# mochell/PiCLES

Measured on AMD Instinct MI355X. Metric: particle_steps_per_sec, higher is better.
Workload: dtype f64

## Files before the change

### include/picles_hip.h

```cpp
#ifndef PICLES_HIP_H
#define PICLES_HIP_H

#include <stdint.h>
#include <stddef.h>

#ifdef __cplusplus
extern "C" {
#endif

#define PICLES_ABI_VERSION 8

typedef struct picles_grid {
    int32_t Nx, Ny;
    double  dx, dy;
    int32_t periodic_x;
    int32_t periodic_y;
    const int8_t *mask;
    int32_t j_begin, j_end;
} picles_grid;

typedef struct picles_phys {
    double r_g, C_alpha, C_phi, C_e, g;
    double gamma, q;
    double c_beta, c_D, c_e, c_alpha;
    int32_t propagation, input, dissipation, peak_shift, direction;
    int32_t _pad0;
    double  dir_deadband;
} picles_phys;

typedef struct picles_ode {
    double  abstol, reltol;
    double  dt0;
    double  dtmin;
    int32_t force_dtmin;
    int32_t solver;
    int64_t maxiters;
    double  log_energy_minimum, log_energy_maximum, wind_min_squared;
    double  timestep;
} picles_ode;

typedef struct picles_model {
    int32_t periodic_boundary;
    int32_t init_type;
    double  default_particle[3];
    double  minimal_state[2];
} picles_model;

#define PICLES_STEP_ZERO_FIRST   1
#define PICLES_STEP_MOVIE        2
#define PICLES_STEP_ATOMIC       4

#define PICLES_ST_STEPPED        1
#define PICLES_ST_MAXITERS       2
#define PICLES_ST_RESEED_NAN     4
#define PICLES_ST_RESEED_INF     8
#define PICLES_ST_CLAMPED       16
#define PICLES_ST_SWITCHED_ON   32
#define PICLES_ST_DTMIN         64
#define PICLES_ST_NONFINITE    128

typedef struct picles_counters {
    uint64_t rhs_evals;
    uint64_t steps_accepted;
    uint64_t steps_rejected;
    uint64_t reseeds;
    uint64_t clamps;
    uint64_t maxiters_hits;
    uint64_t particles_advanced;
    uint64_t halo_overflow;
    int32_t  max_reach;
    int32_t  max_reach_seen;
    uint64_t dropped_nonfinite;
    uint64_t wave_attempt_slots;
} picles_counters;

typedef struct picles_timing {
    double advance_ms, scatter_ms, remesh_ms, other_ms;
    uint64_t advance_launches, scatter_launches, remesh_launches;
} picles_timing;

typedef struct picles_ctx picles_ctx;

int32_t picles_create(const picles_grid *g, const picles_phys *p, const picles_ode *o,
                      const picles_model *m, int32_t device_id, int32_t halo_rows,
                      picles_ctx **out);
int32_t picles_destroy(picles_ctx *ctx);
const char *picles_last_error(const picles_ctx *ctx);
int32_t picles_abi_version(void);

int32_t picles_set_winds(picles_ctx *ctx, const double *u0, const double *v0, double t0,
                         const double *u1, const double *v1, double t1);
int32_t picles_set_winds3(picles_ctx *ctx, const double *u0, const double *v0, double t0,
                          const double *um, const double *vm,
                          const double *u1, const double *v1, double t1);
int32_t picles_set_winds_knot(picles_ctx *ctx, const double *u0, const double *v0, double t0,
                              const double *uk, const double *vk, double tk,
                              const double *u1, const double *v1, double t1);
#define PICLES_MAX_KNOTS 8
int32_t picles_set_winds_polyline(picles_ctx *ctx, int32_t nlev, const double *const *u, const double *const *v, const double *times);

int32_t picles_set_metric(picles_ctx *ctx, const double *m11, const double *m22, const double *pc);

int32_t picles_set_wind_grid(picles_ctx *ctx, int32_t nx, int32_t ny, int32_t nt,
                             double x0, double dx, double y0, double dy, double t0, double dt,
                             const double *u, const double *v, double mesh_x0, double mesh_y0);
#define PICLES_LATTICE_LINEAR  0
#define PICLES_LATTICE_SMOOTH3 1
int32_t picles_set_wind_grid_mode(picles_ctx *ctx, int32_t mode);
int32_t picles_lattice_knots(double lat_t0, double lat_dt, double t, double dt, double *tk);
int32_t picles_lattice_knot_times(double lat_t0, double lat_dt, double t, double dt, double *tks, int32_t cap);
int32_t picles_get_winds(picles_ctx *ctx, double *u0, double *v0, double *u1, double *v1);
int32_t picles_get_winds_mid(picles_ctx *ctx, double *um, double *vm);

int32_t picles_seed(picles_ctx *ctx, double t0);

int32_t picles_time_step(picles_ctx *ctx, double dt, int32_t flags);
int32_t picles_run_steps(picles_ctx *ctx, double dt, int32_t n_steps);
int32_t picles_advance(picles_ctx *ctx, double dt, int32_t flags);
int32_t picles_remesh(picles_ctx *ctx, double dt);
int32_t picles_tick(picles_ctx *ctx, double dt);
int32_t picles_zero_state(picles_ctx *ctx);
double  picles_clock(const picles_ctx *ctx);

int32_t picles_get_state(picles_ctx *ctx, double *state);
int32_t picles_set_state(picles_ctx *ctx, const double *state);
int32_t picles_get_movie_state(picles_ctx *ctx, double *state);

int32_t picles_store_init(picles_ctx *ctx, int32_t n_slots);
int32_t picles_store_push(picles_ctx *ctx);
int32_t picles_store_pop(picles_ctx *ctx, double *state, double *time);
int32_t picles_store_pending(const picles_ctx *ctx);

#define PICLES_DIAG_HS    1
#define PICLES_DIAG_TP    2
#define PICLES_DIAG_CG_X  4
#define PICLES_DIAG_CG_Y  8
#define PICLES_DIAG_E    16
#define PICLES_DIAG_MX   32
#define PICLES_DIAG_MY   64
#define PICLES_DIAG_ALL 127
#define PICLES_DIAG_TILE 256
int32_t picles_diag_init(picles_ctx *ctx, int32_t cx, int32_t cy, int32_t field_mask, int32_t n_slots);
int32_t picles_diag_shape(const picles_ctx *ctx, int32_t *nxc, int32_t *nyc_loc, int32_t *n_fields, int32_t *n_partials, size_t *bytes);
int32_t picles_diag_push(picles_ctx *ctx);
int32_t picles_diag_pop(picles_ctx *ctx, void *fields, double *partials, double *time);
int32_t picles_diag_pending(const picles_ctx *ctx);

#define PICLES_PROBE_E_FULL -30
int32_t picles_probe_init(picles_ctx *ctx, int32_t n, const int32_t *ij, int32_t every, int32_t first, int32_t capacity);
int32_t picles_probe_sample(picles_ctx *ctx, void *stream);
int32_t picles_probe_pop(picles_ctx *ctx, int32_t max_samples, double *values, double *times, int64_t *steps, int32_t *n_out);
int32_t picles_probe_pending(const picles_ctx *ctx);
int32_t picles_probe_shape(const picles_ctx *ctx, int32_t *n, int32_t *every, int32_t *capacity);
int32_t picles_probe_free(picles_ctx *ctx);

#define PICLES_STAT_PEAK   1
#define PICLES_STAT_MEAN   2
#define PICLES_STAT_EXCEED 4
#define PICLES_STAT_ALL    7
int32_t picles_stat_init(picles_ctx *ctx, int32_t group_mask, int32_t n_thresholds, const double *thresholds, int32_t every, int32_t first);
int32_t picles_stat_shape(const picles_ctx *ctx, int32_t *group_mask, int32_t *n_thresholds, double *thresholds, int32_t *every, int32_t *n_planes, size_t *bytes);
int32_t picles_stat_update(picles_ctx *ctx, void *stream);
int32_t picles_stat_get(picles_ctx *ctx, int32_t group_mask, void *planes, int64_t *n_samples, double *t_first, double *t_last);
int32_t picles_stat_set(picles_ctx *ctx, int32_t group_mask, const void *planes, int64_t n_samples, double t_first, double t_last);
int32_t picles_stat_reset(picles_ctx *ctx);
int32_t picles_stat_free(picles_ctx *ctx);

int32_t picles_get_particles(picles_ctx *ctx, double *z, uint8_t *on, uint8_t *boundary,
                             int32_t *status);
int32_t picles_set_particles(picles_ctx *ctx, const double *z, const uint8_t *on);

int32_t picles_get_counters(picles_ctx *ctx, picles_counters *c);
int32_t picles_reset_counters(picles_ctx *ctx);
int32_t picles_enable_timing(picles_ctx *ctx, int32_t on);
int32_t picles_get_timing(picles_ctx *ctx, picles_timing *t);
int32_t picles_get_timing_samples(picles_ctx *ctx, int32_t kind, double *out_ms, int32_t cap);
int32_t picles_get_dispatch_order(picles_ctx *ctx, int32_t *out, int32_t cap);
int32_t picles_sync(picles_ctx *ctx);

#define PICLES_ROWS_ALL      0
#define PICLES_ROWS_EDGE     1
#define PICLES_ROWS_INTERIOR 2
int32_t picles_begin_step(picles_ctx *ctx, double dt, int32_t flags);
int32_t picles_advance_rows(picles_ctx *ctx, int32_t which, void *stream);
int32_t picles_scatter_remesh(picles_ctx *ctx, void *stream);
int32_t picles_begin_fused_step(picles_ctx *ctx, double dt);
int32_t picles_step_rows(picles_ctx *ctx, int32_t which, void *stream);
int32_t picles_end_fused_step(picles_ctx *ctx);
int32_t picles_halo_send_dev(picles_ctx *ctx, int32_t side, void **ptr, size_t *bytes);
int32_t picles_halo_recv_dev(picles_ctx *ctx, int32_t side, void **ptr, size_t *bytes);
int32_t picles_halo_rows(const picles_ctx *ctx);
int32_t picles_set_halo_rows(picles_ctx *ctx, int32_t halo_rows);
int32_t picles_set_slab_mode(picles_ctx *ctx, int32_t on);

#define PICLES_SLAB_ID_BYTES 128
int32_t picles_slab_unique_id(void *id128);
int32_t picles_slab_comm_init(picles_ctx *ctx, const void *id128, int32_t rank, int32_t world);
int32_t picles_slab_run_steps(picles_ctx *ctx, double dt, int32_t n_steps, int32_t flags);
int32_t picles_slab_exchange(picles_ctx *ctx);
int32_t picles_slab_streams(picles_ctx *ctx, void **edge_stream, void **interior_stream);
int32_t picles_slab_comm_destroy(picles_ctx *ctx);
typedef struct picles_slab_phases {
    uint64_t steps;
    uint64_t exchange_hidden;
    double   edge_ms;
    double   exchange_ms;
    double   interior_ms;
    double   slack_ms;
    double   span_ms;
} picles_slab_phases;
int32_t picles_slab_get_phases(picles_ctx *ctx, picles_slab_phases *out);

#define PICLES_CKPT_E_SHORT    -20
#define PICLES_CKPT_E_MAGIC    -21
#define PICLES_CKPT_E_VERSION  -22
#define PICLES_CKPT_E_CONFIG   -23
#define PICLES_CKPT_E_CHECKSUM -24
#define PICLES_CKPT_E_BUSY     -25
int32_t picles_checkpoint_size(picles_ctx *ctx, size_t *bytes);
int32_t picles_checkpoint_begin(picles_ctx *ctx);
int32_t picles_checkpoint_end(picles_ctx *ctx, void *buf, size_t bytes);
int32_t picles_checkpoint_load(picles_ctx *ctx, const void *buf, size_t bytes);

int32_t picles_scatter_particles(picles_ctx *ctx, int64_t n, const int32_t *ij,
                                 const double *xy, const double *charge);

#ifdef __cplusplus
}
#endif
#endif
```

### picles_amd/_capi.py

```python
from __future__ import annotations

import ctypes as C
import os
from pathlib import Path

HERE = Path(__file__).resolve().parent
LIB_PATH = HERE / "csrc" / "libpicles_hip.so"

c_double_p = C.POINTER(C.c_double)
c_int8_p = C.POINTER(C.c_int8)
c_uint8_p = C.POINTER(C.c_uint8)
c_int32_p = C.POINTER(C.c_int32)


class PiclesGrid(C.Structure):
    _fields_ = [
        ("Nx", C.c_int32), ("Ny", C.c_int32),
        ("dx", C.c_double), ("dy", C.c_double),
        ("periodic_x", C.c_int32), ("periodic_y", C.c_int32),
        ("mask", c_int8_p),
        ("j_begin", C.c_int32), ("j_end", C.c_int32),
    ]


class PiclesPhys(C.Structure):
    _fields_ = [
        ("r_g", C.c_double), ("C_alpha", C.c_double), ("C_phi", C.c_double),
        ("C_e", C.c_double), ("g", C.c_double),
        ("gamma", C.c_double), ("q", C.c_double),
        ("c_beta", C.c_double), ("c_D", C.c_double), ("c_e", C.c_double), ("c_alpha", C.c_double),
        ("propagation", C.c_int32), ("input", C.c_int32), ("dissipation", C.c_int32),
        ("peak_shift", C.c_int32), ("direction", C.c_int32), ("_pad0", C.c_int32),
        ("dir_deadband", C.c_double),
    ]


class PiclesOde(C.Structure):
    _fields_ = [
        ("abstol", C.c_double), ("reltol", C.c_double),
        ("dt0", C.c_double), ("dtmin", C.c_double),
        ("force_dtmin", C.c_int32), ("solver", C.c_int32),
        ("maxiters", C.c_int64),
        ("log_energy_minimum", C.c_double), ("log_energy_maximum", C.c_double),
        ("wind_min_squared", C.c_double), ("timestep", C.c_double),
    ]


class PiclesModel(C.Structure):
    _fields_ = [
        ("periodic_boundary", C.c_int32), ("init_type", C.c_int32),
        ("default_particle", C.c_double * 3),
        ("minimal_state", C.c_double * 2),
    ]


class PiclesCounters(C.Structure):
    _fields_ = [
        ("rhs_evals", C.c_uint64), ("steps_accepted", C.c_uint64), ("steps_rejected", C.c_uint64),
        ("reseeds", C.c_uint64), ("clamps", C.c_uint64), ("maxiters_hits", C.c_uint64),
        ("particles_advanced", C.c_uint64), ("halo_overflow", C.c_uint64),
        ("max_reach", C.c_int32), ("max_reach_seen", C.c_int32),
        ("dropped_nonfinite", C.c_uint64), ("wave_attempt_slots", C.c_uint64),
    ]

    def as_dict(self):
        return {k: getattr(self, k) for k, _ in self._fields_ if not k.startswith("_")}


class PiclesTiming(C.Structure):
    _fields_ = [
        ("advance_ms", C.c_double), ("scatter_ms", C.c_double), ("remesh_ms", C.c_double),
        ("other_ms", C.c_double),
        ("advance_launches", C.c_uint64), ("scatter_launches", C.c_uint64),
        ("remesh_launches", C.c_uint64),
    ]

    def as_dict(self):
        return {k: getattr(self, k) for k, _ in self._fields_}


class PiclesSlabPhases(C.Structure):
    _fields_ = [
        ("steps", C.c_uint64), ("exchange_hidden", C.c_uint64),
        ("edge_ms", C.c_double), ("exchange_ms", C.c_double), ("interior_ms", C.c_double),
        ("slack_ms", C.c_double), ("span_ms", C.c_double),
    ]

    def as_dict(self):
        return {k: getattr(self, k) for k, _ in self._fields_}


LATTICE_LINEAR, LATTICE_SMOOTH3 = 0, 1
STEP_ZERO_FIRST = 1
STEP_MOVIE = 2
STEP_ATOMIC = 4
ABI_VERSION = 8
SLAB_ID_BYTES = 128
PROBE_E_FULL = -30

STAT_PEAK, STAT_MEAN, STAT_EXCEED, STAT_ALL = 1, 2, 4, 7

ROWS_ALL, ROWS_EDGE, ROWS_INTERIOR = 0, 1, 2

CKPT_E_SHORT, CKPT_E_MAGIC, CKPT_E_VERSION, CKPT_E_CONFIG, CKPT_E_CHECKSUM, CKPT_E_BUSY = -20, -21, -22, -23, -24, -25
CKPT_MAGIC = 0x31544b4353454c43
CKPT_HEADER_BYTES = 256
CKPT_SEGMENTS = ("state", "z", "qold", "dtn", "asw", "status", "on", "pflags", "counters", "reach_maps")

DIAG_FIELDS = ("hs", "tp", "cg_x", "cg_y", "e", "m_x", "m_y")
DIAG_BITS = {name: 1 << k for k, name in enumerate(DIAG_FIELDS)}
DIAG_TILE = 256
DIAG_PARTIAL = ("sum_e", "sum_mx", "sum_my", "n_wet", "max_e", "max_mx", "max_my")

ST_STEPPED, ST_MAXITERS, ST_RESEED_NAN, ST_RESEED_INF = 1, 2, 4, 8
ST_CLAMPED, ST_SWITCHED_ON, ST_DTMIN, ST_NONFINITE = 16, 32, 64, 128

_VP = C.c_void_p
SYMBOLS = {
    "picles_create": (C.c_int32, [C.POINTER(PiclesGrid), C.POINTER(PiclesPhys), C.POINTER(PiclesOde),
                                  C.POINTER(PiclesModel), C.c_int32, C.c_int32, C.POINTER(_VP)]),
    "picles_destroy": (C.c_int32, [_VP]),
    "picles_last_error": (C.c_char_p, [_VP]),
    "picles_abi_version": (C.c_int32, []),
    "picles_set_winds": (C.c_int32, [_VP, c_double_p, c_double_p, C.c_double, c_double_p, c_double_p, C.c_double]),
    "picles_set_winds3": (C.c_int32, [_VP, c_double_p, c_double_p, C.c_double, c_double_p, c_double_p, c_double_p, c_double_p, C.c_double]),
    "picles_set_winds_knot": (C.c_int32, [_VP, c_double_p, c_double_p, C.c_double, c_double_p, c_double_p, C.c_double,
                                          c_double_p, c_double_p, C.c_double]),
    "picles_set_winds_polyline": (C.c_int32, [_VP, C.c_int32, C.POINTER(c_double_p), C.POINTER(c_double_p), c_double_p]),
    "picles_get_winds_mid": (C.c_int32, [_VP, c_double_p, c_double_p]),
    "picles_set_metric": (C.c_int32, [_VP, c_double_p, c_double_p, c_double_p]),
    "picles_set_wind_grid": (C.c_int32, [_VP, C.c_int32, C.c_int32, C.c_int32, C.c_double, C.c_double, C.c_double,
                                         C.c_double, C.c_double, C.c_double, c_double_p, c_double_p, C.c_double, C.c_double]),
    "picles_set_wind_grid_mode": (C.c_int32, [_VP, C.c_int32]),
    "picles_lattice_knots": (C.c_int32, [C.c_double, C.c_double, C.c_double, C.c_double, c_double_p]),
    "picles_lattice_knot_times": (C.c_int32, [C.c_double, C.c_double, C.c_double, C.c_double, c_double_p, C.c_int32]),
    "picles_get_winds": (C.c_int32, [_VP, c_double_p, c_double_p, c_double_p, c_double_p]),
    "picles_seed": (C.c_int32, [_VP, C.c_double]),
    "picles_time_step": (C.c_int32, [_VP, C.c_double, C.c_int32]),
    "picles_run_steps": (C.c_int32, [_VP, C.c_double, C.c_int32]),
    "picles_advance": (C.c_int32, [_VP, C.c_double, C.c_int32]),
    "picles_remesh": (C.c_int32, [_VP, C.c_double]),
    "picles_tick": (C.c_int32, [_VP, C.c_double]),
    "picles_zero_state": (C.c_int32, [_VP]),
    "picles_clock": (C.c_double, [_VP]),
    "picles_get_state": (C.c_int32, [_VP, c_double_p]),
    "picles_set_state": (C.c_int32, [_VP, c_double_p]),
    "picles_get_movie_state": (C.c_int32, [_VP, c_double_p]),
    "picles_store_init": (C.c_int32, [_VP, C.c_int32]),
    "picles_store_push": (C.c_int32, [_VP]),
    "picles_store_pop": (C.c_int32, [_VP, c_double_p, c_double_p]),
    "picles_store_pending": (C.c_int32, [_VP]),
    "picles_diag_init": (C.c_int32, [_VP, C.c_int32, C.c_int32, C.c_int32, C.c_int32]),
    "picles_diag_shape": (C.c_int32, [_VP, c_int32_p, c_int32_p, c_int32_p, c_int32_p, C.POINTER(C.c_size_t)]),
    "picles_diag_push": (C.c_int32, [_VP]),
    "picles_diag_pop": (C.c_int32, [_VP, _VP, c_double_p, c_double_p]),
    "picles_diag_pending": (C.c_int32, [_VP]),
    "picles_probe_init": (C.c_int32, [_VP, C.c_int32, c_int32_p, C.c_int32, C.c_int32, C.c_int32]),
    "picles_probe_sample": (C.c_int32, [_VP, _VP]),
    "picles_probe_pop": (C.c_int32, [_VP, C.c_int32, c_double_p, c_double_p, C.POINTER(C.c_int64), c_int32_p]),
    "picles_probe_pending": (C.c_int32, [_VP]),
    "picles_probe_shape": (C.c_int32, [_VP, c_int32_p, c_int32_p, c_int32_p]),
    "picles_probe_free": (C.c_int32, [_VP]),
    "picles_stat_init": (C.c_int32, [_VP, C.c_int32, C.c_int32, c_double_p, C.c_int32, C.c_int32]),
    "picles_stat_shape": (C.c_int32, [_VP, c_int32_p, c_int32_p, c_double_p, c_int32_p, c_int32_p, C.POINTER(C.c_size_t)]),
    "picles_stat_update": (C.c_int32, [_VP, _VP]),
    "picles_stat_get": (C.c_int32, [_VP, C.c_int32, _VP, C.POINTER(C.c_int64), c_double_p, c_double_p]),
    "picles_stat_set": (C.c_int32, [_VP, C.c_int32, _VP, C.c_int64, C.c_double, C.c_double]),
    "picles_stat_reset": (C.c_int32, [_VP]),
    "picles_stat_free": (C.c_int32, [_VP]),
    "picles_get_particles": (C.c_int32, [_VP, c_double_p, c_uint8_p, c_uint8_p, c_int32_p]),
    "picles_set_particles": (C.c_int32, [_VP, c_double_p, c_uint8_p]),
    "picles_get_counters": (C.c_int32, [_VP, C.POINTER(PiclesCounters)]),
    "picles_reset_counters": (C.c_int32, [_VP]),
    "picles_enable_timing": (C.c_int32, [_VP, C.c_int32]),
    "picles_get_timing": (C.c_int32, [_VP, C.POINTER(PiclesTiming)]),
    "picles_get_timing_samples": (C.c_int32, [_VP, C.c_int32, c_double_p, C.c_int32]),
    "picles_get_dispatch_order": (C.c_int32, [_VP, C.POINTER(C.c_int32), C.c_int32]),
    "picles_sync": (C.c_int32, [_VP]),
    "picles_begin_step": (C.c_int32, [_VP, C.c_double, C.c_int32]),
    "picles_advance_rows": (C.c_int32, [_VP, C.c_int32, _VP]),
    "picles_scatter_remesh": (C.c_int32, [_VP, _VP]),
    "picles_begin_fused_step": (C.c_int32, [_VP, C.c_double]),
    "picles_step_rows": (C.c_int32, [_VP, C.c_int32, _VP]),
    "picles_end_fused_step": (C.c_int32, [_VP]),
    "picles_halo_send_dev": (C.c_int32, [_VP, C.c_int32, C.POINTER(_VP), C.POINTER(C.c_size_t)]),
    "picles_halo_recv_dev": (C.c_int32, [_VP, C.c_int32, C.POINTER(_VP), C.POINTER(C.c_size_t)]),
    "picles_halo_rows": (C.c_int32, [_VP]),
    "picles_set_halo_rows": (C.c_int32, [_VP, C.c_int32]),
    "picles_set_slab_mode": (C.c_int32, [_VP, C.c_int32]),
    "picles_slab_unique_id": (C.c_int32, [_VP]),
    "picles_slab_comm_init": (C.c_int32, [_VP, _VP, C.c_int32, C.c_int32]),
    "picles_slab_run_steps": (C.c_int32, [_VP, C.c_double, C.c_int32, C.c_int32]),
    "picles_slab_exchange": (C.c_int32, [_VP]),
    "picles_slab_streams": (C.c_int32, [_VP, C.POINTER(_VP), C.POINTER(_VP)]),
    "picles_slab_comm_destroy": (C.c_int32, [_VP]),
    "picles_slab_get_phases": (C.c_int32, [_VP, C.POINTER(PiclesSlabPhases)]),
    "picles_scatter_particles": (C.c_int32, [_VP, C.c_int64, c_int32_p, c_double_p, c_double_p]),
    "picles_checkpoint_size": (C.c_int32, [_VP, C.POINTER(C.c_size_t)]),
    "picles_checkpoint_begin": (C.c_int32, [_VP]),
    "picles_checkpoint_end": (C.c_int32, [_VP, _VP, C.c_size_t]),
    "picles_checkpoint_load": (C.c_int32, [_VP, _VP, C.c_size_t]),
}

_lib = None


class PiclesError(RuntimeError):
    pass


class CheckpointError(PiclesError):

    def __init__(self, code, msg):
        super().__init__(msg)
        self.code = code


def _settle_rocm_runtime():
    import sys
    if "torch" in sys.modules or os.environ.get("PICLES_NO_TORCH_PRELOAD"):
        return
    try:
        import torch
    except Exception:
        pass


def load(path: os.PathLike | None = None) -> C.CDLL:
    global _lib
    if _lib is not None and path is None:
        return _lib
    p = Path(path) if path else Path(os.environ.get("PICLES_HIP_LIB", LIB_PATH))
    if not p.exists():
        raise PiclesError(
            f"{p} not found: build the HIP extension first "
            "(python -c 'import __graft_entry__ as g; g.build()' or make -C picles_amd/csrc)")
    _settle_rocm_runtime()
    lib = C.CDLL(str(p))
    for name, (res, args) in SYMBOLS.items():
        fn = getattr(lib, name)
        fn.restype = res
        fn.argtypes = args
    if lib.picles_abi_version() != ABI_VERSION:
        raise PiclesError(f"{p}: ABI version {lib.picles_abi_version()}, this binding expects {ABI_VERSION} — rebuild the library")
    if path is None:
        _lib = lib
    return lib


def dptr(a):
    if a is None:
        return None
    return a.ctypes.data_as(c_double_p)
```

### picles_amd/csrc/k_step.inc

```
#ifndef K_STEP_NAME
#define K_STEP_NAME k_step
#define K_STEP_WROW false
#include "k_step.inc"
#undef K_STEP_NAME
#undef K_STEP_WROW
#define K_STEP_NAME k_step_waverow
#define K_STEP_WROW true
#include "k_step.inc"
#undef K_STEP_NAME
#undef K_STEP_WROW
#else
template <bool FAST, bool TSIT, bool STATIC, bool METRIC, bool AUTO>
__global__ void __launch_bounds__(256, (FAST && !AUTO) ? 4 : (FAST ? 3 : 2)) K_STEP_NAME(KParams P, GridP G, Arrays A, double t_prev, double DT_prev,
                                                double t_start, double DT, int r0, int n0, int r1, int n1)
{
    constexpr bool WROW = K_STEP_WROW;
    static_assert(!WROW || (FAST && !METRIC), "k_step_waverow: specialised physics, Cartesian");
#ifdef PICLES_PHASE_CLOCK
    const unsigned long long pc0_ = __builtin_readcyclecounter();
    unsigned long long pc1_ = pc0_, pc2_ = pc0_, pc3_ = pc0_;
#endif
#ifdef PICLES_WAVE_LOG
    const unsigned long long wl0_ = __builtin_amdgcn_s_memrealtime();
    unsigned long long wl1_ = 0;
#endif
    dp_device_init(TSIT ? 1 : 0);
    order_sign_init();
    const long long ord_counts = order_counts(A);
    const int ord_entry = order_entry(A);
    const int mr_early = pull_reach_early(A);
    pm_device_init();
    long long t = 0;
    const unsigned int lblock = ordered_block(A, ord_counts, ord_entry);
    WaveRow wr = {0, 0, 0};
    const unsigned int lane = threadIdx.x & 63u;
    bool active;
    if constexpr (WROW) { active = rows_index_waverow(G, r0, n0, lblock, wr); t = wr.t0 + lane; }
    else active = rows_index(G, r0, n0, r1, n1, t, lblock);
    StepStats S = {{0u, 0u, 0u, 0}, 0u, 0u, 0u, 0u, 0u, 0u, 0};
    int rtile = -1;
    if (active) {
        int i, jl;
        if constexpr (WROW) { i = wr.i0 + (int)lane; jl = wr.jl; }
        else { i = (int)(t % G.Nx); jl = (int)(t / G.Nx); }
        double s0 = 0.0, s1 = 0.0, s2 = 0.0;
        if constexpr (WROW) rmap_clear_ahead_waverow(A, wr, lane);
        else rmap_clear_ahead(A, t);
        const Arrays Av = WROW ? arrays_at(A, wr.t0) : A;
        const long long tx = WROW ? (long long)lane : t;
        constexpr bool PREFETCH = AUTO;
        unsigned char pf_pre = 0;
        Wind w_pre = {0.0, 0.0, 0.0, 0.0, 0.0, 0.0};
        double qold_pre = 0.0, uP_pre = 0.0, vP_pre = 0.0;
        int asw_pre = 0;
        if constexpr (PREFETCH) {
            pf_pre = Av.pflags[tx];
            w_pre = load_wind(P, Av, tx);
            if constexpr (WROW) w_pre.xi = (unsigned int)t;
            qold_pre = Av.qold[tx];
            asw_pre = Av.asw[tx];
            if (!STATIC) { uP_pre = Av.uP[tx]; vP_pre = Av.vP[tx]; }
        }
        if constexpr (WROW) pull_waverow(G, A, wr, lane, pull_reach_local_waverow(G, A, wr, lane, pull_reach(G, A, jl, mr_early)), s0, s1, s2);
        else pull_any(G, A, i, jl, pull_reach_local(G, A, i, jl, pull_reach(G, A, jl, mr_early)), s0, s1, s2);
#ifdef PICLES_PHASE_CLOCK
        __asm__ volatile("" : "+v"(s0), "+v"(s1), "+v"(s2));
        pc1_ = __builtin_readcyclecounter();
#endif
#ifdef PICLES_WAVE_LOG
        __asm__ volatile("" : "+v"(s0), "+v"(s1), "+v"(s2));
        wl1_ = __builtin_amdgcn_s_memrealtime();
#endif
        unsigned char pf = PREFETCH ? pf_pre : Av.pflags[tx];
        __shared__ int stash_[WROW ? 1 : 5][256];
        if (pf & PF_STEPPED) {
            Wind w = PREFETCH ? w_pre : load_wind(P, Av, tx);
            if constexpr (WROW) w.xi = (unsigned int)t;
            Vec5 z = {0.0, 0.0, 0.0, 0.0, 0.0};
            double qold = PREFETCH ? qold_pre : Av.qold[tx], dtn = -1.0;
            int br = remesh_regs_lazy(P, pf, s0, s1, s2, DT_prev, z, STATIC ? &Av.u0[tx] : (PREFETCH ? &uP_pre : &Av.uP[tx]),
                                      STATIC ? &Av.v0[tx] : (PREFETCH ? &vP_pre : &Av.vP[tx]));
            int on = (br <= 1);
            int asw = AUTO ? (PREFETCH ? asw_pre : Av.asw[tx]) : 0;
            if (br == 1) { qold = PI_LNQOLDINIT; asw = ASW_FRESH; S.reseeds = 1; }
            unsigned int rs = S.reseeds;
            S.reseeds = 0;
            const int tid_ = threadIdx.x;
            if constexpr (WROW) stash_[0][tid_] = (int)pf | ((int)rs << 8);
            else {
                stash_[0][tid_] = (int)(unsigned int)((unsigned long long)t & 0xffffffffull); stash_[1][tid_] = (int)((unsigned long long)t >> 32);
                stash_[2][tid_] = i; stash_[3][tid_] = jl; stash_[4][tid_] = (int)pf | ((int)rs << 8);
            }
            int status;
            if (METRIC) status = advance_core<FAST, STATIC, true, TSIT, AUTO>(P, w, z, on, qold, dtn, t_start, DT, S, Av.m11[tx], Av.m22[tx], Av.pc[tx], &asw);
            else status = advance_core<FAST, STATIC, false, TSIT, AUTO>(P, w, z, on, qold, dtn, t_start, DT, S, 0.0, 0.0, 0.0, &asw);
#ifdef PICLES_PHASE_CLOCK
            __asm__ volatile("" : "+v"(z.lne));
            pc2_ = __builtin_readcyclecounter();
#endif
            KStepArgsPtr K = kargs_reload();
            const KParams Pb = K->P;
            const GridP Gb = K->G;
            const Arrays Ab = K->A;
            __asm__ volatile("" ::: "memory");
            const int tid2_ = threadIdx.x;
            WaveRow wrb = {0, 0, 0};
            long long tb;
            int ib = 0, jlb = 0, pr_;
            if constexpr (WROW) {
                wrb = waverow_of(Gb, K->r0, lblock);
                tb = wrb.t0 + (threadIdx.x & 63u);
                pr_ = stash_[0][tid2_];
            } else {
                tb = (long long)(((unsigned long long)(unsigned int)stash_[1][tid2_] << 32) | (unsigned int)stash_[0][tid2_]);
                ib = stash_[2][tid2_]; jlb = stash_[3][tid2_]; pr_ = stash_[4][tid2_];
            }
            const unsigned char pfb = (unsigned char)(pr_ & 0xff);
            const Arrays Abv = WROW ? arrays_at(Ab, wrb.t0) : Ab;
            const long long tbx = WROW ? (long long)(threadIdx.x & 63u) : tb;
            status = advance_guards(Pb, [&]() { Wind wg = load_wind(Pb, Abv, tbx); if constexpr (WROW) wg.xi = (unsigned int)tb; return wg; },
                                    z, dtn, K->t_start, K->DT, status, S);
            if (AUTO) Abv.asw[tbx] = asw;
            S.reseeds += (unsigned int)(pr_ >> 8);
            Abv.qold[tbx] = qold;
            Abv.status[tbx] = status;
            if constexpr (WROW) write_record_at(Gb, rec_row_out(Ab, Gb, wrb.jl + Gb.R) + wrb.i0, threadIdx.x & 63u, pfb, on, z, S);
            else write_record(Gb, Ab, ib, jlb, pfb, on, z, S);
            rtile = WROW ? (int)(wrb.t0 >> 6) : (int)(tb >> 6);
        }
    }
    {
        KStepArgsPtr K = kargs_reload();
        const Arrays Ab = K->A;
        flush_stats<WROW>(Ab, S, rtile);
        if (Ab.ord && order_wanted(Ab)) order_file(Ab, lblock, __ballot(S.adv != 0 || S.reseeds != 0) != 0);
#ifdef PICLES_WAVE_LOG
        if ((threadIdx.x & 63) == 0) {
            unsigned int hw_, xcc_;
            __asm__ volatile("s_getreg_b32 %0, hwreg(HW_REG_HW_ID)" : "=s"(hw_));
            __asm__ volatile("s_getreg_b32 %0, hwreg(HW_REG_XCC_ID)" : "=s"(xcc_));
            unsigned long long *wl_ = (unsigned long long *)Ab.movie + 4ull * ((unsigned long long)lblock * 4ull + (threadIdx.x >> 6));
            wl_[0] = wl0_; wl_[1] = wl1_; wl_[2] = __builtin_amdgcn_s_memrealtime();
            wl_[3] = (unsigned long long)hw_ | ((unsigned long long)xcc_ << 32) | ((unsigned long long)blockIdx.x << 40);
        }
#endif
#ifdef PICLES_PHASE_CLOCK
        pc3_ = __builtin_readcyclecounter();
        if ((threadIdx.x & 63) == 0) {
            DevCounters *c = Ab.cnt + ((blockIdx.x * 4u + (threadIdx.x >> 6)) & (NSLOTS - 1));
            if (pc1_ == pc0_) pc1_ = pc3_;
            if (pc2_ < pc1_) pc2_ = pc1_;
            atomicAdd(&c->pad_[0], pc1_ - pc0_); atomicAdd(&c->pad_[1], pc2_ - pc1_); atomicAdd(&c->pad_[2], pc3_ - pc2_); atomicAdd(&c->pad_[3], 1ull);
        }
#endif
    }
}
#endif
```

### picles_amd/csrc/kernels.h

```cpp
#ifndef PICLES_KERNELS_H
#define PICLES_KERNELS_H

#include <hip/hip_runtime.h>
#include <cstdint>
#include <type_traits>

#include "../../include/picles_hip.h"
#include "physics.h"

struct GridP {
    int Nx, Ny;
    int periodic_x, periodic_y;
    int tripolar;
    int j_begin, ny_loc;
    int R;
    int Rp;
    int single_slab;
    int ngroups;
};

#define NSLOTS 1024
struct DevCounters {
    unsigned long long rhs, acc, rej, reseeds, clamps, maxit, adv, overflow;
    unsigned long long nonfinite, wslots, pad_[6];
};

struct Arrays {
    double *state, *movie;
    double *z;
    double *qold, *dtn;
    int *asw;
    unsigned char *on, *pflags;
    int *status;
    double *u0, *v0, *u1, *v1;
    double *um, *vm;
    double *uP, *vP;
    double *m11, *m22, *pc;
    double *rec;
    double *rec_out;
    DevCounters *cnt;
    int mr_idx;
    int ntile;
    int *rmap;
    int ord_on, nblk;
    int *ord;
    long long n;
};
__device__ __forceinline__ int *order_buf(const Arrays &A, int which) { return A.ord + (size_t)which * (size_t)(2 + A.nblk); }

__device__ __forceinline__ int *reach_counters(const Arrays &A) { return (int *)(A.cnt + NSLOTS); }

#define PF_STEPPED 1
#define PF_GROUP2 2
#define PF_BOUNDARY 4

__device__ __forceinline__ unsigned long long wave_sum_u64(unsigned long long v)
{
    const unsigned int lo0 = (unsigned int)__builtin_amdgcn_readfirstlane((int)(unsigned int)v);
    const unsigned int hi0 = (unsigned int)__builtin_amdgcn_readfirstlane((int)(unsigned int)(v >> 32));
    const unsigned long long v0 = ((unsigned long long)hi0 << 32) | lo0;
    if (__all(v == v0)) return v0 * 64ull;
#pragma unroll
    for (int o = 32; o > 0; o >>= 1) v += __shfl_xor(v, o, 64);
    return v;
}
__device__ __forceinline__ int wave_max_i32(int v)
{
#pragma unroll
    for (int o = 32; o > 0; o >>= 1) {
        int t = __shfl_xor(v, o, 64);
        v = (t > v) ? t : v;
    }
    return v;
}

template <bool POLY = false>
__device__ __forceinline__ Wind load_wind(const KParams &P, const Arrays &A, long long t)
{
    Wind w;
    w.u0 = A.u0[t];
    w.v0 = A.v0[t];
    w.bu = 0.0;
    w.bv = 0.0;
    w.xi = (unsigned int)t;
    if (POLY && !P.wind_static && P.wind_nk > 1) {
        const double *pl = P.wind_xb + PICLES_MAX_KNOTS + t;
        w.du = pl[0]; w.dv = pl[P.wind_xn]; w.bu = pl[2 * P.wind_xn]; w.bv = pl[3 * P.wind_xn];
        return w;
    }
    if (P.wind_static) {
        w.du = 0.0;
        w.dv = 0.0;
    } else {
        const double u1 = A.u1[t], v1 = A.v1[t];
        w.du = u1 - w.u0;
        w.dv = v1 - w.v0;
        if (A.um) {
            const double um = A.um[t], vm = A.vm[t];
            if (P.wind_sk > 0.0) {
                w.du = (um - w.u0) * P.wind_isk;
                w.dv = (vm - w.v0) * P.wind_isk;
                w.bu = (u1 - um) * P.wind_i1sk - w.du;
                w.bv = (v1 - vm) * P.wind_i1sk - w.dv;
            } else {
                w.bu = 2.0 * ((w.u0 + u1) - 2.0 * um);
                w.bv = 2.0 * ((w.v0 + v1) - 2.0 * vm);
            }
        }
    }
    return w;
}

__device__ __forceinline__ double *rec_row(const Arrays &A, const GridP &G, int row)
{
    return A.rec + (size_t)row * 6 * G.Nx;
}
__device__ __forceinline__ double *rec_row_out(const Arrays &A, const GridP &G, int row)
{
    return A.rec_out + (size_t)row * 6 * G.Nx;
}

#define REC_BIAS 2048
#define REACH_CAP 64
__device__ __forceinline__ double rec_encode(int grp, int bx, int by)
{
    return (double)(grp + 4 * (bx + REC_BIAS) + 4 * 4096 * (by + REC_BIAS));
}
__device__ __forceinline__ void rec_decode(double code, int &grp, int &bx, int &by)
{
    int ci = (int)code;
    grp = ci & 3;
    bx = ((ci >> 2) & 4095) - REC_BIAS;
    by = (ci >> 14) - REC_BIAS;
}

struct StepStats {
    PStats st;
    unsigned int adv, reseeds, clamps, maxit, overflow, nonfinite;
    int reach;
};

template <bool FAST, bool STATIC, bool METRIC = false, bool TSIT = false, bool AUTO = false, bool TABS = true>
__device__ __forceinline__ int advance_core(const KParams &P, const Wind &w, Vec5 &z, int &on, double &qold,
                                            double &dtn, double t_start, double DT, StepStats &S,
                                            double m11 = 0.0, double m22 = 0.0, double pc = 0.0, int *asw = nullptr)
{
    int status = PICLES_ST_STEPPED;
    if (on) {
        S.adv = 1;
        integrate_dp5<FAST, STATIC, METRIC, TSIT, AUTO, TABS>(P, w, z, qold, dtn, t_start, DT, S.st, m11, m22, pc, asw);
        status |= S.st.status;
    } else {
        double u, v;
        wind_at<(!FAST && !STATIC)>(P, w, t_start + DT, u, v);
        if (u * u + v * v >= P.wind_min_sq) {
            reseed(P, u, v, DT, z);
            dtn = -1.0;
            on = 1;
            status |= PICLES_ST_SWITCHED_ON;
        }
    }
    return status;
}

template <bool POLY = false, class WF>
__device__ __forceinline__ int advance_guards(const KParams &P, WF wind, Vec5 &z, double &dtn, double t_start, double DT,
                                              int status, StepStats &S)
{
    if (pm_isnan(z.lne) || pm_isnan(z.cx) || pm_isnan(z.cy)) {
        double u, v;
        const Wind w = wind();
        wind_at<POLY>(P, w, t_start + DT, u, v);
        reseed(P, u, v, DT, z);
        dtn = -1.0;
        status |= PICLES_ST_RESEED_NAN;
    } else if (pm_isinf(z.lne) || pm_isinf(z.cx) || pm_isinf(z.cy)) {
        double u, v;
        const Wind w = wind();
        wind_at<POLY>(P, w, t_start, u, v);
        reseed(P, u, v, DT, z);
        dtn = -1.0;
        status |= PICLES_ST_RESEED_INF;
    } else if (z.lne > P.lne_max) {
        z.lne = P.lne_max;
        dtn = -1.0;
        status |= PICLES_ST_CLAMPED;
    }
    if (status & (PICLES_ST_RESEED_NAN | PICLES_ST_RESEED_INF | PICLES_ST_SWITCHED_ON)) S.reseeds = 1;
    if (status & PICLES_ST_CLAMPED) S.clamps = 1;
    if (status & PICLES_ST_MAXITERS) S.maxit = 1;
    return status;
}

struct KStepArgs {
    KParams P;
    GridP G;
    Arrays A;
    double t_prev, DT_prev, t_start, DT;
    int r0, n0, r1, n1;
};
static_assert(__builtin_offsetof(KStepArgs, G) == sizeof(KParams) && __builtin_offsetof(KStepArgs, A) % 8 == 0 &&
              __builtin_offsetof(KStepArgs, t_prev) == __builtin_offsetof(KStepArgs, A) + sizeof(Arrays) &&
              __builtin_offsetof(KStepArgs, r0) == __builtin_offsetof(KStepArgs, DT) + 8,
              "KStepArgs must mirror the kernarg layout of k_step");
typedef const KStepArgs *KStepArgsPtr;
__device__ __forceinline__ KStepArgsPtr kargs_reload(void)
{
    auto p = __builtin_amdgcn_kernarg_segment_ptr();
    __asm__ volatile("" : "+s"(p));
    return (KStepArgsPtr)p;
}

template <class IDX>
__device__ __forceinline__ void write_record_at(const GridP &G, double *rr, IDX i, unsigned char pf, int on, const Vec5 &z, StepStats &S)
{
    auto at = [&](int plane) -> double & {
        if constexpr (std::is_unsigned<IDX>::value) return (rr + (size_t)plane * (size_t)G.Nx)[i];
        else return rr[plane * G.Nx + i];
    };
    double code = 0.0;
    if (on && !(pm_isfinite(z.x) && pm_isfinite(z.y))) {
        S.nonfinite = 1;
    } else if (on && !(pm_fabs(z.x) < 2047.0 && pm_fabs(z.y) < 2047.0)) {
        S.overflow = 1;
    } else if (on) {
        double e, mx, my;
        particle_to_charge(z.lne, z.cx, z.cy, e, mx, my);
        int bx, by;
        double wx, wy;
        index_weight(z.x, bx, wx);
        index_weight(z.y, by, wy);
        int r = (bx < 0) ? -bx : bx + 1;
        int ry = (by < 0) ? -by : by + 1;
        S.reach = (r > ry) ? r : ry;
        if (S.reach <= ((G.Rp > 0) ? G.Rp : REACH_CAP)) {
            at(0) = e; at(1) = mx; at(2) = my; at(3) = wx; at(4) = wy;
            code = rec_encode((pf & PF_GROUP2) ? 2 : 1, bx, by);
        }
        else { S.overflow = 1; S.reach = 0; }
    }
    at(5) = code;
}
__device__ __forceinline__ void write_record(const GridP &G, const Arrays &A, int i, int jl, unsigned char pf, int on,
                                             const Vec5 &z, StepStats &S)
{
    write_record_at(G, rec_row_out(A, G, jl + G.R), i, pf, on, z, S);
}

template <bool WROW = false>
__device__ __forceinline__ void flush_stats(const Arrays &A, const StepStats &S, int rtile = -1)
{
    unsigned long long s_rhs = wave_sum_u64(S.st.rhs);
    unsigned long long s_ar = wave_sum_u64(((unsigned long long)S.st.acc << 32) | S.st.rej);
    unsigned long long b_adv = __ballot(S.adv != 0), b_res1 = __ballot(S.reseeds == 1), b_res2 = __ballot(S.reseeds >= 2);
    unsigned long long b_cl = __ballot(S.clamps != 0), b_mx = __ballot(S.maxit != 0), b_ov = __ballot(S.overflow != 0);
    unsigned long long b_nf = __ballot(S.nonfinite != 0);
    const int att_ = (int)(S.st.acc + S.st.rej);
    int m_att = __builtin_amdgcn_readfirstlane(att_);
    while (__ballot(att_ > m_att)) m_att++;
    int m_reach = 0;
    if (__ballot(S.reach > 0)) {
        m_reach = 1;
        while (__ballot(S.reach > m_reach)) m_reach++;
    }
    if (m_reach > 0) {
        int *const rm = A.rmap + (size_t)((A.mr_idx >> 4) & 15) * (size_t)A.ntile;
        if constexpr (WROW) {
            const int lead = __ffsll((long long)__ballot(S.reach > 0)) - 1;
            const int tile0 = __builtin_amdgcn_readlane(rtile, lead);
            if ((int)(threadIdx.x & 63) == lead) atomicMax(rm + tile0, m_reach);
        }
        int mine = (!WROW && S.reach > 0) ? rtile : -1;
        unsigned long long todo = WROW ? 0ull : __ballot(mine >= 0);
        while (todo) {
            const int lead = __ffsll((long long)todo) - 1;
            const int tile0 = __builtin_amdgcn_readlane(mine, lead);
            const bool in = (mine == tile0);
            int r0 = 1;
            while (__ballot(in && S.reach > r0)) r0++;
            if ((int)(threadIdx.x & 63) == lead) atomicMax(rm + tile0, r0);
            if (in) mine = -1;
            todo = __ballot(mine >= 0);
        }
    }
    if ((threadIdx.x & 63) == 0) {
        DevCounters *c = A.cnt + ((blockIdx.x * 4u + (threadIdx.x >> 6)) & (NSLOTS - 1));
        unsigned long long s_acc = s_ar >> 32, s_rej = s_ar & 0xffffffffULL;
        unsigned long long s_res = (unsigned long long)__popcll(b_res1) + 2ull * __popcll(b_res2);
        if (s_rhs) atomicAdd(&c->rhs, s_rhs);
        if (s_acc) atomicAdd(&c->acc, s_acc);
        if (s_rej) atomicAdd(&c->rej, s_rej);
        if (b_adv) atomicAdd(&c->adv, (unsigned long long)__popcll(b_adv));
        if (s_res) atomicAdd(&c->reseeds, s_res);
        if (b_cl) atomicAdd(&c->clamps, (unsigned long long)__popcll(b_cl));
        if (b_mx) atomicAdd(&c->maxit, (unsigned long long)__popcll(b_mx));
        if (b_ov) atomicAdd(&c->overflow, (unsigned long long)__popcll(b_ov));
        if (b_nf) atomicAdd(&c->nonfinite, (unsigned long long)__popcll(b_nf));
        if (m_att) atomicAdd(&c->wslots, 64ull * (unsigned long long)m_att);
        int *const mr = reach_counters(A), *const mr_out = mr + ((A.mr_idx >> 4) & 15);
        if (m_reach > 0 && m_reach > __hip_atomic_load(mr_out, __ATOMIC_RELAXED, __HIP_MEMORY_SCOPE_AGENT)) {
            atomicMax(mr_out, m_reach);
            atomicMax(mr + 5, m_reach);
        }
        if (blockIdx.x == 0 && threadIdx.x == 0) {
            mr[(A.mr_idx >> 8) & 15] = 0;
            mr[8 + ((A.mr_idx >> 8) & 15)] = 0;
        }
        if (!b_adv && !s_res && mr[8 + ((A.mr_idx >> 4) & 15)] == 0) mr[8 + ((A.mr_idx >> 4) & 15)] = 1;
    }
}

__device__ __forceinline__ unsigned int xcd_block(void)
{
    const unsigned int n = gridDim.x, b = blockIdx.x;
    const unsigned int per = (n + 7u) / 8u;
    unsigned int l = (b % 8u) * per + b / 8u;
    return (n % 8u == 0u) ? l : b;
}

#define PICLES_BLOCK 256
__device__ __forceinline__ long long order_counts(const Arrays &A)
{
    return A.ord_on ? *(const long long *)order_buf(A, A.mr_idx & 15) : 0ll;
}
__device__ __forceinline__ int order_entry(const Arrays &A)
{
    return (A.ord_on && (int)blockIdx.x < A.nblk) ? order_buf(A, A.mr_idx & 15)[2 + blockIdx.x] : 0;
}
__device__ __forceinline__ unsigned int ordered_block(const Arrays &A, long long counts, int entry)
{
    if (A.ord_on) {
        const int busy = (int)(counts & 0xffffffffll), calm = (int)(counts >> 32);
        if (busy + calm == A.nblk && (int)gridDim.x == A.nblk && 8 * calm >= A.nblk) return (unsigned int)entry;
    }
    return xcd_block();
}
__device__ __forceinline__ int *order_sign(void)
{
    __shared__ int sign_;
    return &sign_;
}
__device__ __forceinline__ void order_sign_init(void) { if (threadIdx.x == 0) *order_sign() = 0; }
__device__ __forceinline__ bool order_wanted(const Arrays &A) { return reach_counters(A)[8 + (A.mr_idx & 15)] != 0; }
__device__ __forceinline__ void order_file(const Arrays &A, unsigned int lblock, bool wave_busy)
{
    if ((threadIdx.x & 63) != 0) return;
    const int v = atomicAdd(order_sign(), 1 + (wave_busy ? 256 : 0));
    if ((v & 255) != (int)(PICLES_BLOCK / 64) - 1) return;
    const bool busy = wave_busy || (v >> 8) != 0;
    int *const wb = order_buf(A, (A.mr_idx >> 4) & 15);
    const int pos = busy ? atomicAdd(wb, 1) : A.nblk - 1 - atomicAdd(wb + 1, 1);
    if (pos >= 0 && pos < A.nblk) wb[2 + pos] = (int)lblock;
    if (blockIdx.x == 0) { int *const cb = order_buf(A, (A.mr_idx >> 8) & 15); cb[0] = 0; cb[1] = 0; }
}

__device__ __forceinline__ bool rows_index(const GridP &G, int r0, int n0, int r1, int n1, long long &t, unsigned int lblock)
{
    if (n1 == 0 && (G.Nx & 63) == 0 && (n0 & 3) == 0) {
        const unsigned int nbx = (unsigned int)G.Nx >> 6;
        const unsigned int by = lblock / nbx, bx = lblock - by * nbx;
        if (by >= ((unsigned int)n0 >> 2)) return false;
        t = ((long long)r0 + 4ll * by + (threadIdx.x >> 6)) * G.Nx + (64ll * bx + (threadIdx.x & 63));
        return true;
    }
    long long tid = (long long)lblock * PICLES_BLOCK + threadIdx.x;
    long long na = (long long)n0 * G.Nx, nb = (long long)n1 * G.Nx;
    if (tid >= na + nb) return false;
    t = (tid < na) ? (long long)r0 * G.Nx + tid : (long long)r1 * G.Nx + (tid - na);
    return true;
}

__device__ __forceinline__ int remesh_regs(const KParams &P, const Wind &w, unsigned char pf, double e, double mx,
                                           double my, double clock, double DT, Vec5 &z)
{
    double u, v;
    wind_at<true>(P, w, clock, u, v);
    bool bnd = (pf & PF_BOUNDARY) != 0;
    if (!bnd && (e >= P.min_e) && (mx * mx + my * my >= P.min_m2)) {
        charge_to_particle(e, mx, my, z);
        return 0;
    }
    if (u * u + v * v >= P.wind_min_sq) {
        reseed(P, u, v, DT, z);
        return 1;
    }
    return 2;
}

__device__ __forceinline__ int remesh_regs_lazy(const KParams &P, unsigned char pf, double e, double mx, double my,
                                                double DT, Vec5 &z, const double *pu, const double *pv)
{
    bool bnd = (pf & PF_BOUNDARY) != 0;
    if (!bnd && (e >= P.min_e) && (mx * mx + my * my >= P.min_m2)) {
        charge_to_particle(e, mx, my, z);
        return 0;
    }
    double u = *pu, v = *pv;
    if (u * u + v * v >= P.wind_min_sq) {
        reseed(P, u, v, DT, z);
        return 1;
    }
    return 2;
}

// ... 124 lines not shown
        for (int k = 0; k < 4; k++) {
            if (on[k]) {
                const double w = (hx[k] ? wx[k] : 1.0 - wx[k]) * (hy[k] ? wy[k] : 1.0 - wy[k]);
                s0 += w * e[k];
                s1 += w * mx[k];
                s2 += w * my[k];
            }
        }
    }
}
template <int RT>
__device__ __forceinline__ void pull_node(const GridP &G, const Arrays &A, int i, int jl, int Rdyn,
                                          double &s0, double &s1, double &s2)
{
    const int R = RT ? RT : Rdyn, W = 2 * R + 1;
    const int RO = G.R;
    const int j = jl + G.j_begin, Nx = G.Nx;
    const double *__restrict__ rec = A.rec;
    const unsigned int pl = (unsigned int)Nx, rowlen = 6u * pl;
    bool interior = (i - R >= 0) && (i + R < Nx) && (j - R >= 0) && (j + R < G.Ny);
    if (interior) {
        const unsigned int base = (unsigned int)(jl + RO) * rowlen + (unsigned int)i;
        for (int grp = 1; grp <= G.ngroups; grp++) {
            if constexpr (RT == 1 || RT == 2) {
                pull_window_2p<RT>(rec, base, pl, rowlen, grp, s0, s1, s2);
            } else {
#pragma unroll 1
                for (int dj = -R; dj <= R; dj++) {
                    const unsigned int rb = base + (unsigned int)(dj * (int)rowlen);
                    if constexpr (RT != 0) {
#pragma unroll
                        for (int di = -RT; di <= RT; di++)
                            pull_candidate(rec, rb + (unsigned int)di, pl, di, dj, grp, true, s0, s1, s2);
                    } else {
                        for (int di = -R; di <= R; di++)
                            pull_candidate(rec, rb + (unsigned int)di, pl, di, dj, grp, true, s0, s1, s2);
                    }
                }
            }
        }
        return;
    }
    int shx = 0, shy = 0;
    if (G.periodic_x) { if (i - R < 0) shx = R - i; else if (i + R >= Nx) shx = Nx - i + R; }
    if (G.periodic_y) { if (j - R < 0) shy = R - j; else if (j + R >= G.Ny) shy = G.Ny - j + R; }
    for (int grp = 1; grp <= G.ngroups; grp++) {
#pragma unroll 1
        for (int sj = 0; sj < W; sj++) {
            int qj = sj + shy; if (qj >= W) qj -= W;
            int dj = qj - R;
            int jj = j + dj;
            bool rowok = G.periodic_y || (jj >= 0 && jj < G.Ny);
            int row;
            if (G.single_slab) {
                int jw = jj; if (jw < 0) jw += G.Ny; else if (jw >= G.Ny) jw -= G.Ny;
                row = jw + RO;
            } else {
                row = jl + dj + RO;
            }
            if (!rowok) continue;
#pragma unroll 1
            for (int si = 0; si < W; si++) {
                int qi = si + shx; if (qi >= W) qi -= W;
                int di = qi - R;
                int ii = i + di;
                if (ii < 0 || ii >= Nx) {
                    if (!G.periodic_x) continue;
                    ii += (ii < 0) ? Nx : -Nx;
                }
                pull_candidate(rec, (unsigned int)row * rowlen + (unsigned int)ii, pl, di, dj, grp, true, s0, s1, s2);
            }
        }
    }
}

__device__ __forceinline__ int floor_mod(int a, int b) { int r = a % b; return (r < 0) ? r + b : r; }

__device__ __forceinline__ void pull_node_tripolar(const GridP &G, const Arrays &A, int i, int jl, int R,
                                                   double &s0, double &s1, double &s2)
{
    const int RO = G.R, Nx = G.Nx, Ny = G.Ny, j = jl + G.j_begin, W = 2 * R + 1;
    const double *__restrict__ rec = A.rec;
    const unsigned int pl = (unsigned int)Nx, rowlen = 6u * pl;
    const int cB = floor_mod(Nx - 2 - i, Nx);
    const bool narrow = (2 * W <= Nx);
    const int a0 = floor_mod(i - R, Nx), b0 = floor_mod(cB - R, Nx);
    for (int grp = 1; grp <= G.ngroups; grp++) {
        for (int js = max(0, j - R); js < Ny; js++) {
            const unsigned int rbase = (unsigned int)(js - G.j_begin + RO) * rowlen;
            int ka = 0, kb = 0, is_full = 0;
            while (narrow ? (ka < W || kb < W) : (is_full < Nx)) {
                int is;
                if (narrow) {
                    const int wa = a0 + W - Nx, wb = b0 + W - Nx;
                    int ea = (ka < W) ? ((wa > 0) ? ((ka < wa) ? ka : a0 + (ka - wa)) : a0 + ka) : 0x7fffffff;
                    int eb = (kb < W) ? ((wb > 0) ? ((kb < wb) ? kb : b0 + (kb - wb)) : b0 + kb) : 0x7fffffff;
                    is = min(ea, eb);
                    if (ea == is) ka++;
                    if (eb == is) kb++;
                } else {
                    is = is_full++;
                }
                const int ci0 = (int)rec[rbase + 5u * pl + (unsigned int)is];
                if (ci0 == 0 || (ci0 & 3) != grp) continue;
                const int bx = ((ci0 >> 2) & 4095) - REC_BIAS, by = (ci0 >> 14) - REC_BIAS;
                const double wxh = rec[rbase + 3u * pl + (unsigned int)is], wyh = rec[rbase + 4u * pl + (unsigned int)is];
#pragma unroll
                for (int k = 0; k < 4; k++) {
                    const int ax = k & 1, ay = k >> 1;
                    int ci = is + bx + ax, cj = js + by + ay;
                    if (cj < 0) continue;
                    if (cj >= Ny) { ci = Nx - 1 - floor_mod(ci + 1, Nx); cj = 2 * Ny - 1 - cj; }
                    else ci = floor_mod(ci, Nx);
                    if (ci != i || cj != j) continue;
                    const double w = (ax ? wxh : 1.0 - wxh) * (ay ? wyh : 1.0 - wyh);
                    s0 += w * rec[rbase + (unsigned int)is];
                    s1 += w * rec[rbase + pl + (unsigned int)is];
                    s2 += w * rec[rbase + 2u * pl + (unsigned int)is];
                }
            }
        }
    }
}

__device__ __forceinline__ void pull_any(const GridP &G, const Arrays &A, int i, int jl, int R,
                                         double &s0, double &s1, double &s2)
{
    const int W = 2 * R + 1;
    if (R == 0) return;
    if (G.tripolar && jl + G.j_begin >= G.Ny - R) pull_node_tripolar(G, A, i, jl, R, s0, s1, s2);
    else if ((G.periodic_x && W > G.Nx) || (G.periodic_y && W > G.Ny)) pull_node_aliased(G, A, i, jl, R, s0, s1, s2);
    else if (R == 1) pull_node<1>(G, A, i, jl, 1, s0, s1, s2);
    else if (R == 2) pull_node<2>(G, A, i, jl, 2, s0, s1, s2);
    else if (R == 3) pull_node<3>(G, A, i, jl, 3, s0, s1, s2);
    else if (R == 4) pull_node<4>(G, A, i, jl, 4, s0, s1, s2);
    else pull_node<0>(G, A, i, jl, R, s0, s1, s2);
}

__device__ __forceinline__ int pull_reach_early(const Arrays &A) { return reach_counters(A)[A.mr_idx & 15]; }
__device__ __forceinline__ int pull_reach(const GridP &G, const Arrays &A, int jl, int m)
{
    if (G.Rp > 0 && (jl < G.R || jl >= G.ny_loc - G.R)) return G.Rp;
    if (m < 1) m = 1;
    return (G.Rp > 0 && m > G.Rp) ? G.Rp : m;
}
__device__ __forceinline__ int pull_reach(const GridP &G, const Arrays &A, int jl) { return pull_reach(G, A, jl, pull_reach_early(A)); }


__device__ __forceinline__ void rmap_clear_ahead(const Arrays &A, long long t)
{
    if ((t & 63) == 0) A.rmap[(size_t)((A.mr_idx >> 8) & 15) * (size_t)A.ntile + (size_t)(t >> 6)] = 0;
}

__device__ __forceinline__ int pull_reach_local(const GridP &G, const Arrays &A, int i, int jl, int Rg)
{
    int R = Rg;
    const int j = jl + G.j_begin;
    const bool edge_row = G.Rp > 0 && (jl < G.R || jl >= G.ny_loc - G.R);
    if (Rg >= 2 && Rg <= 31 && !edge_row && i - Rg >= 0 && i + Rg < G.Nx && jl - Rg >= 0 && jl + Rg < G.ny_loc &&
        j - Rg >= 0 && j + Rg < G.Ny) {
        const int *const rm = A.rmap + (size_t)(A.mr_idx & 15) * (size_t)A.ntile;
        int m = 0;
        long long t0 = (long long)(jl - Rg) * G.Nx + (i - Rg);
        for (int dj = -Rg; dj <= Rg; dj++, t0 += G.Nx) {
            const int a = rm[t0 >> 6], b = rm[(t0 + 2 * Rg) >> 6];
            m = max(m, max(a, b));
        }
        R = min(m, Rg);
    }
    if (Rg < 2) return Rg;
    int m = 0;
    while (__ballot(R > m)) m++;
    return m;
}

struct WaveRow {
    int jl, i0;
    long long t0;
};
__device__ __forceinline__ WaveRow waverow_of(const GridP &G, int r0, unsigned int lblock)
{
    const unsigned int nbx = (unsigned int)G.Nx >> 6;
    const unsigned int by = lblock / nbx, bx = lblock - by * nbx;
    WaveRow w;
    unsigned int tid = threadIdx.x;
    __asm__ volatile("" : "+v"(tid));
    w.jl = r0 + 4 * (int)by + __builtin_amdgcn_readfirstlane((int)(tid >> 6));
    w.i0 = (int)(64u * bx);
    w.t0 = (long long)w.jl * G.Nx + w.i0;
    return w;
}
__device__ __forceinline__ bool rows_index_waverow(const GridP &G, int r0, int n0, unsigned int lblock, WaveRow &w)
{
    const unsigned int nbx = (unsigned int)G.Nx >> 6;
    if (lblock / nbx >= ((unsigned int)n0 >> 2)) return false;
    w = waverow_of(G, r0, lblock);
    return true;
}
__device__ __forceinline__ Arrays arrays_at(const Arrays &A, long long t0)
{
    Arrays B = A;
    B.qold += t0; B.asw += t0; B.pflags += t0; B.status += t0;
    B.u0 += t0; B.v0 += t0; B.u1 += t0; B.v1 += t0; B.uP += t0; B.vP += t0;
    B.um = A.um ? A.um + t0 : nullptr; B.vm += t0;
    return B;
}
__device__ __forceinline__ void rmap_clear_ahead_waverow(const Arrays &A, const WaveRow &w, unsigned int lane)
{
    if (lane == 0u) A.rmap[(size_t)((A.mr_idx >> 8) & 15) * (size_t)A.ntile + (size_t)(w.t0 >> 6)] = 0;
}

__device__ __forceinline__ int pull_reach_local_waverow(const GridP &G, const Arrays &A, const WaveRow &w, unsigned int lane, int Rg)
{
    if (Rg < 2) return Rg;
    const int jl = w.jl, j = jl + G.j_begin;
    const bool edge_row = G.Rp > 0 && (jl < G.R || jl >= G.ny_loc - G.R);
    if (Rg <= 31 && !edge_row && w.i0 - Rg >= 0 && w.i0 + 63 + Rg < G.Nx && jl - Rg >= 0 && jl + Rg < G.ny_loc && j - Rg >= 0 && j + Rg < G.Ny) {
        const int *const rm = A.rmap + (size_t)(A.mr_idx & 15) * (size_t)A.ntile;
        const long long nbx = G.Nx >> 6;
        long long tile = ((long long)(jl - Rg) * G.Nx + w.i0) >> 6;
        int m = 0;
        for (int dj = -Rg; dj <= Rg; dj++, tile += nbx) m = max(m, max(rm[tile - 1], max(rm[tile], rm[tile + 1])));
        return __builtin_amdgcn_readfirstlane(min(m, Rg));
    }
    return pull_reach_local(G, A, w.i0 + (int)lane, jl, Rg);
}

template <int R>
__device__ __forceinline__ void pull_walk_lanes(const double *__restrict__ rec, unsigned int base, unsigned int pl, unsigned int rowlen,
                                                unsigned int m, unsigned int ax, unsigned int ay, double &s0, double &s1, double &s2)
{
    constexpr int W = 2 * R + 1;
    while (__ballot(m != 0u)) {
        double e[4], mx[4], my[4], wx[4], wy[4];
        bool on[4], hx[4], hy[4];
#pragma unroll
        for (int k = 0; k < 4; k++) {
            on[k] = (m != 0u);
            const int c = on[k] ? __builtin_ctz(m) : 0;
            m &= m - 1u;
            hx[k] = (ax >> c) & 1u; hy[k] = (ay >> c) & 1u;
            const unsigned int off = base + (unsigned int)((c / W - R) * (int)rowlen + (c % W - R));
            e[k] = mx[k] = my[k] = wx[k] = wy[k] = 0.0;
            if (on[k]) {
                wx[k] = rec[off + 3u * pl]; wy[k] = rec[off + 4u * pl];
                e[k] = rec[off]; mx[k] = rec[off + pl]; my[k] = rec[off + 2u * pl];
            }
        }
#pragma unroll
        for (int k = 0; k < 4; k++) {
            if (on[k]) {
                const double w = (hx[k] ? wx[k] : 1.0 - wx[k]) * (hy[k] ? wy[k] : 1.0 - wy[k]);
                s0 += w * e[k];
                s1 += w * mx[k];
                s2 += w * my[k];
            }
        }
    }
}

template <int R>
__device__ __forceinline__ void pull_window_waverow(const double *__restrict__ rec, const double *__restrict__ rec0, unsigned int lane,
                                                    unsigned int base, unsigned int pl, unsigned int rowlen, int grp,
                                                    double &s0, double &s1, double &s2)
{
    constexpr int W = 2 * R + 1, NC = W * W;
    static_assert(NC <= 25, "corner bits of all candidates in two words");
    const double *const codes = rec0 + 5u * (size_t)pl;
    unsigned int vo[5];
#pragma unroll
    for (int k = 0; k < 5; k++) vo[k] = 8u * ((unsigned int)k * pl + lane);
    int d[NC];
    unsigned int m0 = 0u, some = 0u, px = 0u, py = 0u;
#pragma unroll
    for (int c = 0; c < NC; c++) {
        const int di = c % W - R, dj = c / W - R;
        d[c] = (int)(codes + ((long long)dj * (long long)rowlen + di))[lane] - (grp + 4 * (REC_BIAS - 1 - di) + 4 * 4096 * (REC_BIAS - 1 - dj));
        const unsigned int n = (unsigned int)__builtin_popcountll(__ballot((d[c] & ~(4 | 16384)) == 0));
        m0 |= (n >> 6) << c;
        some |= n & 63u;
        px |= ((unsigned int)d[c] & 4u) << c;
        py |= (((unsigned int)d[c] >> 14) & 1u) << c;
    }
    if constexpr (R >= 2) {
        if (some != 0u) { pull_window_2p<R>(rec, base, pl, rowlen, grp, s0, s1, s2); return; }
    } else if (some != 0u) {
        unsigned int m = 0u, ax = 0u, ay = 0u;
#pragma unroll
        for (int c = 0; c < NC; c++) {
            m |= ((d[c] & ~(4 | 16384)) == 0 ? 1u : 0u) << c;
            ax |= ((d[c] & 4) ? 0u : 1u) << c;
            ay |= ((d[c] & 16384) ? 0u : 1u) << c;
        }
        pull_walk_lanes<R>(rec, base, pl, rowlen, m, ax, ay, s0, s1, s2);
        return;
    }
    unsigned int mu = m0;
    while (mu != 0u) {
        double e[4], mx[4], my[4], wx[4], wy[4];
        bool on[4], hx[4], hy[4];
#pragma unroll
        for (int k = 0; k < 4; k++) {
            on[k] = (mu != 0u);
            const int c = on[k] ? __builtin_ctz(mu) : 0;
            mu &= mu - 1u;
            hx[k] = !((px >> (c + 2)) & 1u); hy[k] = !((py >> c) & 1u);
            const double *const p = rec0 + ((long long)(c / W - R) * (long long)rowlen + (c % W - R));
            e[k] = mx[k] = my[k] = wx[k] = wy[k] = 0.0;
            if (on[k]) {
                const char *const pb = (const char *)p;
                wx[k] = *(const double *)(pb + vo[3]); wy[k] = *(const double *)(pb + vo[4]);
                e[k] = *(const double *)(pb + vo[0]); mx[k] = *(const double *)(pb + vo[1]); my[k] = *(const double *)(pb + vo[2]);
            }
        }
#pragma unroll
        for (int k = 0; k < 4; k++) {
            if (on[k]) {
                const double w = (hx[k] ? wx[k] : 1.0 - wx[k]) * (hy[k] ? wy[k] : 1.0 - wy[k]);
                s0 += w * e[k];
                s1 += w * mx[k];
                s2 += w * my[k];
            }
        }
    }
}

__device__ __forceinline__ void pull_waverow(const GridP &G, const Arrays &A, const WaveRow &w, unsigned int lane, int R,
                                             double &s0, double &s1, double &s2)
{
    const int j = w.jl + G.j_begin;
    if ((R == 1 || R == 2) && w.i0 - R >= 0 && w.i0 + 63 + R < G.Nx && j - R >= 0 && j + R < G.Ny) {
        const unsigned int pl = (unsigned int)G.Nx, rowlen = 6u * pl;
        const double *const rec0 = A.rec + ((size_t)(w.jl + G.R) * (size_t)rowlen + (size_t)w.i0);
        const unsigned int base = (unsigned int)(w.jl + G.R) * rowlen + ((unsigned int)w.i0 + lane);
        for (int grp = 1; grp <= G.ngroups; grp++) {
            if (R == 1) pull_window_waverow<1>(A.rec, rec0, lane, base, pl, rowlen, grp, s0, s1, s2);
            else pull_window_waverow<2>(A.rec, rec0, lane, base, pl, rowlen, grp, s0, s1, s2);
        }
        return;
    }
    pull_any(G, A, w.i0 + (int)lane, w.jl, R, s0, s1, s2);
}

struct StepLaunch {
    dim3 grid, block;
    hipStream_t stream;
    const KParams *P;
    const GridP *G;
    const Arrays *A;
    double t_prev, DT_prev, t_start, DT;
    int r0, n0, r1, n1;
    bool waverow;
};
static inline bool waverow_geometry(int Nx, int n0, int n1) { return n1 == 0 && (Nx & 63) == 0 && (n0 & 3) == 0; }
static inline bool waverow_flavour(bool fast, bool metric) { return fast && !metric; }
void launch_k_step_explicit(const StepLaunch &L, bool fast, int solver, bool wind_static, bool metric);
void launch_k_step_auto(const StepLaunch &L, bool wind_static, bool metric);
void launch_k_advance(const StepLaunch &L, bool fast, int solver, bool wind_static, bool metric);

#endif
```

### picles_amd/csrc/picles_hip.hip

```cpp
#include <hip/hip_runtime.h>
#include <hipcub/hipcub.hpp>

#include <algorithm>
#include <cstdint>
#include <cstdlib>
#include <cstdio>
#include <cstring>
#include <cmath>
#include <mutex>
#include <string>
#include <vector>

#include "../../include/picles_hip.h"
#include "physics.h"

#define PX_EXPORT extern "C" __attribute__((visibility("default")))

#include "kernels.h"
#include "k_diag.h"
#include "k_probe.h"
#include "k_stat.h"

__global__ void __launch_bounds__(256) k_seed(KParams P, GridP G, Arrays A, const signed char *mask, double seed_T)
{
// ... 202 lines not shown
                }
            }
        }
    }
    __syncthreads();
    for (int k = threadIdx.x; k < PT_LY * PT_LX; k += blockDim.x) {
        int li = k % PT_LX, lj = k / PT_LX;
        double a0 = tile[0][lj][li], a1 = tile[1][lj][li], a2 = tile[2][lj][li];
        if (a0 == 0.0 && a1 == 0.0 && a2 == 0.0) continue;
        global_add3(G, A, i0 + li - PT_AP, j0 + lj - PT_AP, a0, a1, a2);
    }
}

__global__ void k_tile_count(GridP G, int ntx, const int *pij, long long np, int *count, int *tile_of)
{
    long long k = (long long)blockIdx.x * blockDim.x + threadIdx.x;
    if (k >= np) return;
    int ib = pij[k], jb = pij[np + k] - G.j_begin;
    int tile = -1;
    if (ib >= 0 && ib < G.Nx && jb >= 0 && jb < G.ny_loc) {
        tile = (jb / PT_TY) * ntx + ib / PT_TX;
        atomicAdd(&count[tile], 1);
    }
    tile_of[k] = tile;
}
__global__ void k_tile_fill(long long np, const int *tile_of, const int *seg_start, int *cursor, int *perm)
{
    long long k = (long long)blockIdx.x * blockDim.x + threadIdx.x;
    if (k >= np) return;
    int tile = tile_of[k];
    if (tile < 0) return;
    int pos = atomicAdd(&cursor[tile], 1);
    perm[seg_start[tile] + pos] = (int)k;
}

struct WindGrid {
    int nx, ny, nt;
    double x0, inv_dx, y0, inv_dy, t0, inv_dt;
    double mesh_x0, mesh_y0, mesh_dx, mesh_dy;
    const double *u, *v;
};

__device__ __forceinline__ void lattice_coord(double c, int n, int &i0, double &f)
{
    double per = (double)(n - 1);
    double w = (c < 0.0 || c > per) ? c - __builtin_floor(c / per) * per : c;
    double fl = __builtin_floor(w);
    i0 = (int)fl;
    if (i0 > n - 2) i0 = n - 2;
    if (i0 < 0) i0 = 0;
    f = w - (double)i0;
}

struct WindSampleOut { double t[2]; double *u[2], *v[2]; };
template <int NT>
__global__ void __launch_bounds__(256) k_wind_sample(GridP G, WindGrid Wg, WindSampleOut O, long long n)
{
    long long k = (long long)blockIdx.x * blockDim.x + threadIdx.x;
    if (k >= n) return;
    int i = (int)(k % G.Nx), j = (int)(k / G.Nx) + G.j_begin;
    double x = Wg.mesh_x0 + (double)i * Wg.mesh_dx, y = Wg.mesh_y0 + (double)j * Wg.mesh_dy;
    int ix, iy;
    double fx, fy;
    lattice_coord((x - Wg.x0) * Wg.inv_dx, Wg.nx, ix, fx);
    lattice_coord((y - Wg.y0) * Wg.inv_dy, Wg.ny, iy, fy);
    size_t sx = 1, sy = (size_t)Wg.nx, st = (size_t)Wg.nx * Wg.ny;
    const double *F[2] = {Wg.u, Wg.v};
#pragma unroll
    for (int q = 0; q < NT; q++) {
        int it;
        double ft;
        lattice_coord((O.t[q] - Wg.t0) * Wg.inv_dt, Wg.nt, it, ft);
        size_t b = ix * sx + iy * sy + it * st;
        double out[2];
#pragma unroll
        for (int c = 0; c < 2; c++) {
            const double *f = F[c];
            double c00 = f[b] + (f[b + sx] - f[b]) * fx;
            double c10 = f[b + sy] + (f[b + sy + sx] - f[b + sy]) * fx;
            double c01 = f[b + st] + (f[b + st + sx] - f[b + st]) * fx;
            double c11 = f[b + st + sy] + (f[b + st + sy + sx] - f[b + st + sy]) * fx;
            double c0 = c00 + (c10 - c00) * fy;
            double c1 = c01 + (c11 - c01) * fy;
            out[c] = c0 + (c1 - c0) * ft;
        }
        O.u[q][k] = out[0];
        O.v[q][k] = out[1];
    }
}

struct WindPolyForm { int nk; double sk[PICLES_MAX_KNOTS]; double ilen[PICLES_MAX_KNOTS + 1]; };
__global__ void __launch_bounds__(256) k_wind_poly(WindPolyForm F, const double *u0, const double *v0, const double *u1, const double *v1,
                                                   const double *lv, double *xb, long long n)
{
    long long t = (long long)blockIdx.x * blockDim.x + threadIdx.x;
    if (t < PICLES_MAX_KNOTS) xb[t] = (t < F.nk) ? F.sk[t] : 2.0;
    if (t >= n) return;
    double *pl = xb + PICLES_MAX_KNOTS;
    for (int c = 0; c < 2; c++) {
        double prev = c ? v0[t] : u0[t], slp = 0.0;
        for (int j = 0; j <= F.nk; j++) {
            const double next = (j < F.nk) ? lv[(size_t)(2 * j + c) * n + t] : (c ? v1[t] : u1[t]);
            const double sl = (next - prev) * F.ilen[j];
            pl[(size_t)(2 * j + c) * n + t] = j ? sl - slp : sl;
            slp = sl;
            prev = next;
        }
    }
}

static thread_local std::string g_create_error;

static const uint64_t FP_SEED = 0xcbf29ce484222325ull;
static uint64_t fp_bytes(uint64_t h, const void *p, size_t bytes)
{
    const unsigned char *b = (const unsigned char *)p;
    size_t k = 0;
    for (; k + 8 <= bytes; k += 8) {
        uint64_t w;
        memcpy(&w, b + k, 8);
        h = (h ^ w) * 0x100000001b3ull;
        h ^= h >> 29;
    }
    uint64_t w = (uint64_t)(bytes - k) << 56;
    if (k < bytes) { uint64_t t = 0; memcpy(&t, b + k, bytes - k); w ^= t; }
    h = (h ^ w) * 0x100000001b3ull;
    return h ^ (h >> 29);
}
template <class T> static uint64_t fp_val(uint64_t h, T v) { return fp_bytes(h, &v, sizeof v); }

struct picles_ctx {
    picles_grid g;
    picles_phys ph;
    picles_ode od;
    picles_model md;
    KParams P;
    GridP G;
    Arrays A;
    int device;
    hipStream_t stream;
    hipEvent_t ev_edge;
    hipEvent_t ev_ctx = nullptr;
    bool edge_pending = false;
    bool step_fresh = false;
    struct SlabRing *ring = nullptr;
    double *rec_buf[2] = {nullptr, nullptr};
    int *mr_buf[5] = {nullptr, nullptr, nullptr, nullptr, nullptr};
    int mr_w = 0;
    struct Pipe *pipe = nullptr;
    int pipe_nb = 0;
    int cur = 0;
    bool fuse_steps = true;
    int waverow_mode = 1;
    bool pending = false;
    double pend_t = 0.0, pend_dt = 0.0;
    signed char *d_mask = nullptr;
    std::vector<signed char> h_mask;
    double clock = 0.0;
    double step_dt = 0.0;
    int step_flags = 0;
    bool state_zero = false;
    bool seeded = false;
    bool timing = false;
    int timing_mode = 0;
    bool in_region = false;
    int region_launches = 0;
    struct Ev { hipEvent_t a, b; int kind; };
    std::vector<Ev> ev_used, ev_free;
    picles_timing tim{};
    std::vector<float> tim_samples[3];
    std::string err;
    int store_slots = 0, store_head = 0, store_count = 0;
    std::vector<double *> store_dev, store_host;
    std::vector<hipEvent_t> store_ready, store_done;
    std::vector<double> store_time;
    hipStream_t store_stream = nullptr;
    int diag_slots = 0, diag_head = 0, diag_count = 0;
    DiagP diag{};
    int diag_nfields = 0, diag_npart = 0;
    size_t diag_field_bytes = 0, diag_part_off = 0, diag_slot_bytes = 0;
    std::vector<unsigned char *> diag_dev, diag_host;
    std::vector<hipEvent_t> diag_ready, diag_done;
    std::vector<double> diag_time;
    int probe_n = 0, probe_every = 1, probe_first = 1, probe_cap = 0, probe_head = 0, probe_count = 0;
    long long probe_steps = 0;
    int *probe_nodes = nullptr;
    double *probe_dev = nullptr, *probe_host = nullptr;
    std::vector<hipEvent_t> probe_ready, probe_done;
    std::vector<double> probe_time;
    std::vector<long long> probe_step;
    bool stat_on = false;
    StatP stat{};
    int stat_every = 1, stat_first = 1;
    long long stat_steps = 0;
    long long stat_samples = 0;
    double stat_t_first = 0.0, stat_t_last = 0.0;
    unsigned char *stat_dev = nullptr;
    size_t stat_bytes = 0;
    hipEvent_t stat_ev = nullptr;
    hipStream_t stat_stream = nullptr;
    bool stat_ev_live = false;
    bool wind_grid_on = false;
    WindGrid wg{};
    double *d_wgu = nullptr, *d_wgv = nullptr;
    double wind_t1 = 0.0;
    bool wind_t1_valid = false;
    int wind_grid_mode = PICLES_LATTICE_LINEAR;
    double wg_t0 = 0.0, wg_dt = 0.0;
    bool ord_valid = false;
    int ord_nblk = 0;
    double *um_buf = nullptr, *vm_buf = nullptr;
    double *lv_buf = nullptr, *xb_buf = nullptr;
    int poly_cap = 0;
    bool ext_streams = false;
    bool ring_orders = false;
    unsigned char *ck_dev = nullptr, *ck_host = nullptr;
    size_t ck_cap = 0;
    hipEvent_t ck_ready = nullptr, ck_done = nullptr;
    bool ck_inflight = false;
    unsigned char ck_hdr[256];
    int halo0 = 0;
    uint64_t fp_metric = 0, fp_lattice = 0;
    int *d_count = nullptr, *d_start = nullptr, *d_cursor = nullptr;
    void *d_scan_tmp = nullptr;
    size_t scan_tmp_bytes = 0;
};

#define HIPCHK(ctx, call)                                                                      \
    do {                                                                                       \
        hipError_t e_ = (call);                                                                \
        if (e_ != hipSuccess) {                                                                \
            (ctx)->err = std::string(#call) + ": " + hipGetErrorString(e_);                    \
            return -10;                                                                        \
        }                                                                                      \
    } while (0)

static bool stream_idle(hipStream_t s)
{
    hipError_t e = hipStreamQuery(s);
    if (e != hipSuccess) (void)hipGetLastError();
    return e == hipSuccess;
}

static int fail(picles_ctx *c, int code, const std::string &m)
{
    c->err = m;
    return code;
}

static void timing_begin(picles_ctx *c, hipStream_t s, int kind)
{
    if (!c->timing) return;
    if (c->in_region) { if (kind == 0) c->region_launches++; return; }
    picles_ctx::Ev e;
    if (!c->ev_free.empty()) { e = c->ev_free.back(); c->ev_free.pop_back(); }
    else { hipEventCreate(&e.a); hipEventCreate(&e.b); }
    e.kind = kind;
    hipEventRecord(e.a, s);
    c->ev_used.push_back(e);
}
static void timing_end(picles_ctx *c, hipStream_t s)
{
    if (!c->timing || c->in_region) return;
    hipEventRecord(c->ev_used.back().b, s);
}
static void timing_collect(picles_ctx *c)
{
    for (auto &e : c->ev_used) {
        hipEventSynchronize(e.b);
        float ms = 0.f;
        hipEventElapsedTime(&ms, e.a, e.b);
        if (e.kind >= 0 && e.kind < 3 && c->tim_samples[e.kind].size() < (1u << 20)) c->tim_samples[e.kind].push_back(ms);
        switch (e.kind) {
        case 3: c->tim.advance_ms += ms; break;
        case 0: c->tim.advance_ms += ms; c->tim.advance_launches++; break;
        case 1: c->tim.scatter_ms += ms; c->tim.scatter_launches++; break;
        case 2: c->tim.remesh_ms += ms; c->tim.remesh_launches++; break;
        default: c->tim.other_ms += ms;
        }
        c->ev_free.push_back(e);
    }
    c->ev_used.clear();
}

static size_t rec_bytes(const picles_ctx *c) { return (size_t)(c->G.ny_loc + 2 * c->G.R) * 6 * c->G.Nx * sizeof(double); }

static Arrays arrays_for(picles_ctx *c, int read_buf, int write_buf)
{
    Arrays A = c->A;
    A.rec = c->rec_buf[read_buf];
    A.rec_out = c->rec_buf[write_buf];
    A.mr_idx = (read_buf == write_buf ? c->mr_w : (c->mr_w + 4) % 5) | (c->mr_w << 4) | (((c->mr_w + 2) % 5) << 8);
    return A;
}

static int launch_scatter(picles_ctx *c, hipStream_t s, bool remesh);

static int probe_room(picles_ctx *c, long long n_steps, const char *who);
static int probe_take(picles_ctx *c, hipStream_t s);
static bool probe_due(const picles_ctx *c, long long s);
static void probe_release(picles_ctx *c);
static int stat_update(picles_ctx *c, hipStream_t s);
static void stat_release(picles_ctx *c);
static inline bool stat_due(const picles_ctx *c, long long s)
{
    return s >= c->stat_first && (s - c->stat_first) % c->stat_every == 0;
}

static int flush(picles_ctx *c)
{
    if (!c->pending) return 0;
    HIPCHK(c, hipDeviceSynchronize());
    c->pending = false;
    double clock_save = c->clock, dt_save = c->step_dt;
    int flags_save = c->step_flags;
    c->clock = c->pend_t;
    c->step_dt = c->pend_dt;
    c->step_flags = PICLES_STEP_ZERO_FIRST;
    int rc = launch_scatter(c, c->stream, true);
    c->clock = clock_save; c->step_dt = dt_save; c->step_flags = flags_save;
    return rc;
}

PX_EXPORT int32_t picles_abi_version(void) { return PICLES_ABI_VERSION; }

PX_EXPORT const char *picles_last_error(const picles_ctx *ctx)
{
    return ctx ? ctx->err.c_str() : g_create_error.c_str();
}

PX_EXPORT int32_t picles_destroy(picles_ctx *c);
PX_EXPORT int32_t picles_slab_comm_destroy(picles_ctx *c);

PX_EXPORT int32_t picles_create(const picles_grid *g, const picles_phys *p, const picles_ode *o,
                                const picles_model *m, int32_t device_id, int32_t halo_rows, picles_ctx **out)
{
    if (!g || !p || !o || !m || !out) { g_create_error = "null argument"; return -1; }
    *out = nullptr;
    if (g->Nx < 2 || g->Ny < 2) { g_create_error = "grid must be at least 2x2"; return -2; }
    if (g->j_begin < 0 || g->j_end > g->Ny || g->j_end <= g->j_begin) { g_create_error = "bad slab rows [j_begin,j_end)"; return -2; }
    if (o->solver < 0 || o->solver > 2) { g_create_error = "solver must be 0 (DP5), 1 (Tsit5) or 2 (AutoTsit5(Rosenbrock23()))"; return -3; }
    if (halo_rows < 1) halo_rows = 1;
    if (halo_rows > 1024) { g_create_error = "halo_rows must be <= 1024"; return -2; }
    if (!(o->abstol > 0.0) || !(o->reltol >= 0.0) || !(o->maxiters > 0) || !(o->dtmin >= 0.0)) {
        g_create_error = "ODE settings: abstol > 0, reltol >= 0, maxiters > 0, dtmin >= 0 required";
        return -3;
    }
    int ndev = 0;
    hipError_t e = hipGetDeviceCount(&ndev);
    if (e != hipSuccess || ndev <= 0) {
        g_create_error = "no HIP device available (this library has no CPU path)";
        return -4;
    }
    if (device_id < 0 || device_id >= ndev) { g_create_error = "device_id out of range"; return -4; }
    if ((e = hipSetDevice(device_id)) != hipSuccess) { g_create_error = hipGetErrorString(e); return -4; }

    picles_ctx *c = new picles_ctx();
    if (const char *wr = getenv("PICLES_WAVEROW")) c->waverow_mode = !strcmp(wr, "0") ? 0 : (!strcmp(wr, "require") ? 2 : 1);
    memset(&c->A, 0, sizeof(c->A));
    c->stream = nullptr;
    c->ev_edge = nullptr;
    c->g = *g; c->ph = *p; c->od = *o; c->md = *m;
    c->device = device_id;
    KParams &P = c->P;
    P.r_g = p->r_g; P.inv_rg = 1.0 / p->r_g; P.C_alpha = p->C_alpha; P.C_phi = p->C_phi; P.C_e = p->C_e;
    double q = p->q;
    P.p = (-1.0 - 10.0 * q) / 2.0;
    P.n = 2.0 * q / (P.p + 4.0 * q);
    P.neg2p = -2.0 * P.p;
    double e_T = std::sqrt(p->c_e * pm_pow(p->c_alpha, -P.p / q) / pm_pow(p->gamma * p->c_beta * p->c_D, 1.0 / P.n));
    P.inv_eT = 1.0 / e_T;
    P.inv_eT4 = (P.inv_eT * P.inv_eT) * (P.inv_eT * P.inv_eT);
    P.half_inv_rg = 0.5 * P.inv_rg;
    P.two_inv_rg2 = 2.0 * (P.inv_rg * P.inv_rg);
    {
        const double k1 = 0.25 * PK_G0, k2 = k1 * k1, K = k2 * k2;
        P.KeT4 = K * P.inv_eT4;
        P.KrCa = (K * P.r_g) * P.C_alpha;
        P.Cdir = P.C_phi * P.two_inv_rg2;
        P.rg2 = P.r_g * P.r_g;
        const double rg4 = P.rg2 * P.rg2, rg8 = rg4 * rg4;
        P.Cw = (0.5 * PK_G0) * P.r_g;
        P.Chrh = -0.25 * P.r_g;
        P.ymax = 10.0 / P.r_g;
        P.sgmax = 1e8 / P.rg2;
        P.KeT4y = P.KeT4 * rg8;
        P.KrCay = P.KrCa * rg8;
        P.Cs = (0.5 * P.C_phi) * P.rg2;
        P.Cdir2 = 2.0 * P.C_phi;
        P.g4rg2 = k1 * P.rg2;
        P.qU2r_max = 249999.0 / (P.ymax * P.ymax);
    }
    P.inv_dx = 1.0 / g->dx; P.inv_dy = 1.0 / g->dy;
    P.deadband2 = p->dir_deadband * p->dir_deadband;
    P.propagation = p->propagation; P.input = p->input; P.dissipation = p->dissipation;
    P.peak_shift = p->peak_shift; P.direction = p->direction; P.n_is_2 = (P.n == 2.0);
    P.p_is_075 = (P.p == 0.75);
    P.fast_phys = P.propagation && P.input && P.dissipation && P.peak_shift && P.direction && P.n_is_2 && P.p_is_075 && P.deadband2 == 0.0;
    P.abstol = o->abstol; P.reltol = o->reltol; P.dt0 = o->dt0; P.dtmin = o->dtmin;
    P.inv_abstol = 1.0 / o->abstol;
    P.maxiters = o->maxiters; P.force_dtmin = o->force_dtmin;
    P.solver = o->solver;
    P.lne_max = o->log_energy_maximum; P.wind_min_sq = o->wind_min_squared;
    P.init_type = m->init_type;
    P.def_lne = m->default_particle[0]; P.def_cx = m->default_particle[1]; P.def_cy = m->default_particle[2];
    P.min_e = m->minimal_state[0]; P.min_m2 = m->minimal_state[1];
    P.wind_static = 1; P.tw0 = 0.0; P.inv_dtw = 0.0; P.wind_sk = P.wind_isk = P.wind_i1sk = 0.0;

    GridP &G = c->G;
    G.Nx = g->Nx; G.Ny = g->Ny; G.periodic_x = (g->periodic_x != 0); G.periodic_y = (g->periodic_y == 1);
    G.tripolar = (g->periodic_y == 2);
    if (g->periodic_y < 0 || g->periodic_y > 2 || (G.tripolar && !G.periodic_x)) {
        g_create_error = "periodic_y must be 0, 1 or 2 (tripolar north, which needs a periodic x axis)";
        delete c;
        return -2;
    }
    G.j_begin = g->j_begin; G.ny_loc = g->j_end - g->j_begin;
    G.single_slab = (g->j_begin == 0 && g->j_end == g->Ny);
    G.R = halo_rows;
    c->halo0 = halo_rows;
    G.Rp = G.single_slab ? 0 : halo_rows;
    G.ngroups = 1;

    long long n = (long long)G.Nx * G.ny_loc;
    c->h_mask.resize(n);
    for (int jl = 0; jl < G.ny_loc; jl++)
        for (int i = 0; i < G.Nx; i++) {
            int j = jl + G.j_begin;
            signed char mk;
            if (g->mask) mk = g->mask[(long long)j * G.Nx + i];
            else {
                bool ring = (!g->periodic_x && (i == 0 || i == G.Nx - 1)) || (!g->periodic_y && (j == 0 || j == G.Ny - 1));
                mk = ring ? 3 : 1;
            }
            c->h_mask[(long long)jl * G.Nx + i] = mk;
        }
    std::vector<unsigned char> pf(n, 0);
    bool any3 = false;
    if (g->mask) { for (long long k = 0; k < (long long)G.Nx * G.Ny; k++) if (g->mask[k] == 3) { any3 = true; break; } }
    else any3 = (!g->periodic_x || !g->periodic_y);
    for (long long k = 0; k < n; k++) {
        signed char mk = c->h_mask[k];
        unsigned char f = 0;
        if (mk == 1) f |= PF_STEPPED;
        if (mk == 3 && m->periodic_boundary) f |= PF_STEPPED | PF_GROUP2;
        bool bnd = m->periodic_boundary ? (mk == 2) : (mk >= 2);
        if (bnd) f |= PF_BOUNDARY;
        pf[k] = f;
    }
    if (any3 && m->periodic_boundary) G.ngroups = 2;
    if ((long long)(G.ny_loc + 2 * G.R) * 6 * G.Nx >= (1LL << 31)) {
        g_create_error = "slab too large for 32-bit record offsets ((ny_loc + 2 halo_rows) * 6 * Nx must be < 2^31): use more slabs";
        delete c;
        return -2;
    }
    if (!G.single_slab && ((G.periodic_y && G.Ny <= 2 * G.R) || G.ny_loc < G.R)) {
        g_create_error = "slab: periodic y axis not longer than 2*halo_rows, or fewer own rows than halo_rows";
        delete c;
        return -2;
    }

#define CK(call) do { hipError_t e2 = (call); if (e2 != hipSuccess) { g_create_error = std::string(#call) + ": " + hipGetErrorString(e2); picles_destroy(c); return -10; } } while (0)
    CK(hipStreamCreateWithFlags(&c->stream, hipStreamNonBlocking));
    CK(hipEventCreateWithFlags(&c->ev_edge, hipEventDisableTiming));
    CK(hipEventCreateWithFlags(&c->ev_ctx, hipEventDisableTiming));
    Arrays &A = c->A;
    memset(&A, 0, sizeof(A));
    A.n = n;
    CK(hipMalloc(&A.state, 3 * n * 8)); CK(hipMalloc(&A.movie, 3 * n * 8));
    CK(hipMalloc(&A.z, 5 * n * 8));
    CK(hipMalloc(&A.qold, n * 8)); CK(hipMalloc(&A.dtn, n * 8)); CK(hipMalloc(&A.asw, n * 4)); CK(hipMemset(A.asw, 0, n * 4));
    CK(hipMalloc(&A.on, n)); CK(hipMalloc(&A.pflags, n)); CK(hipMalloc(&A.status, n * 4));
    CK(hipMalloc(&A.u0, n * 8)); CK(hipMalloc(&A.v0, n * 8)); CK(hipMalloc(&A.u1, n * 8)); CK(hipMalloc(&A.v1, n * 8));
    CK(hipMalloc(&A.cnt, NSLOTS * sizeof(DevCounters) + 16 * sizeof(int)));
    for (int k = 0; k < 5; k++) c->mr_buf[k] = (int *)(A.cnt + NSLOTS) + k;
    CK(hipMemset(c->mr_buf[0], 0, 16 * sizeof(int)));
    for (int k = 0; k < 2; k++) {
        CK(hipMalloc(&c->rec_buf[k], rec_bytes(c)));
        CK(hipMemset(c->rec_buf[k], 0, rec_bytes(c)));
    }
    A.nblk = (int)((n + 255) / 256);
    A.ord_on = 0;
    A.ord = nullptr;
    CK(hipMalloc(&A.ord, (size_t)5 * (2 + A.nblk) * sizeof(int)));
    CK(hipMemset(A.ord, 0, (size_t)5 * (2 + A.nblk) * sizeof(int)));
    A.ntile = (int)((n + 63) / 64);
    CK(hipMalloc(&A.rmap, (size_t)5 * A.ntile * sizeof(int)));
    CK(hipMemset(A.rmap, 0, (size_t)5 * A.ntile * sizeof(int)));
    CK(hipMalloc(&c->d_mask, n));
    CK(hipMemset(A.state, 0, 3 * n * 8)); CK(hipMemset(A.movie, 0, 3 * n * 8)); CK(hipMemset(A.z, 0, 5 * n * 8));
    CK(hipMemset(A.qold, 0, n * 8)); CK(hipMemset(A.dtn, 0, n * 8)); CK(hipMemset(A.on, 0, n)); CK(hipMemset(A.status, 0, n * 4));
    CK(hipMemset(A.u0, 0, n * 8)); CK(hipMemset(A.v0, 0, n * 8)); CK(hipMemset(A.u1, 0, n * 8)); CK(hipMemset(A.v1, 0, n * 8));
    CK(hipMemset(A.cnt, 0, NSLOTS * sizeof(DevCounters)));
    CK(hipMemcpy(A.pflags, pf.data(), n, hipMemcpyHostToDevice));
    CK(hipMemcpy(c->d_mask, c->h_mask.data(), n, hipMemcpyHostToDevice));
#undef CK
    c->state_zero = true;
    *out = c;
    return 0;
}

PX_EXPORT int32_t picles_destroy(picles_ctx *c)
{
    if (!c) return 0;
    hipSetDevice(c->device);
    if (c->ring) picles_slab_comm_destroy(c);
    if (c->stream) hipStreamSynchronize(c->stream);
    if (c->store_stream) hipStreamSynchronize(c->store_stream);
    Arrays &A = c->A;
    hipFree(A.state); hipFree(A.movie); hipFree(A.z); hipFree(A.qold); hipFree(A.dtn); hipFree(A.asw); hipFree(A.on);
    hipFree(A.pflags); hipFree(A.status); hipFree(A.u0); hipFree(A.v0); hipFree(A.u1); hipFree(A.v1);
    if (A.uP) { hipFree(A.uP); hipFree(A.vP); }
    if (c->um_buf) { hipFree(c->um_buf); hipFree(c->vm_buf); }
    if (c->lv_buf) { hipFree(c->lv_buf); hipFree(c->xb_buf); }
    hipFree(A.cnt); hipFree(A.rmap); hipFree(c->d_mask);
    if (A.ord) hipFree(A.ord);
    if (A.m11) { hipFree(A.m11); hipFree(A.m22); hipFree(A.pc); }
    for (int k = 0; k < 2; k++) hipFree(c->rec_buf[k]);

    for (auto p : c->store_dev) hipFree(p);
    for (auto p : c->store_host) hipHostFree(p);
    for (auto e : c->store_ready) hipEventDestroy(e);
    for (auto e : c->store_done) hipEventDestroy(e);
    for (auto p : c->diag_dev) hipFree(p);
    for (auto p : c->diag_host) hipHostFree(p);
    for (auto e : c->diag_ready) hipEventDestroy(e);
    for (auto e : c->diag_done) hipEventDestroy(e);
    probe_release(c);
    if (c->stat_on) hipDeviceSynchronize();
    stat_release(c);
    if (c->ck_dev) hipFree(c->ck_dev);
    if (c->ck_host) hipHostFree(c->ck_host);
    if (c->ck_ready) hipEventDestroy(c->ck_ready);
    if (c->ck_done) hipEventDestroy(c->ck_done);
    if (c->store_stream) hipStreamDestroy(c->store_stream);
    if (c->d_wgu) hipFree(c->d_wgu);
    if (c->d_wgv) hipFree(c->d_wgv);
    if (c->d_count) hipFree(c->d_count);
    if (c->d_start) hipFree(c->d_start);
    if (c->d_cursor) hipFree(c->d_cursor);
    if (c->d_scan_tmp) hipFree(c->d_scan_tmp);
    for (auto &e : c->ev_used) { hipEventDestroy(e.a); hipEventDestroy(e.b); }
    for (auto &e : c->ev_free) { hipEventDestroy(e.a); hipEventDestroy(e.b); }
    if (c->ev_edge) hipEventDestroy(c->ev_edge);
    if (c->ev_ctx) hipEventDestroy(c->ev_ctx);
    if (c->stream) hipStreamDestroy(c->stream);
    delete c;
    return 0;
}

PX_EXPORT int32_t picles_sync(picles_ctx *c)
{
    if (!c) return -1;
    HIPCHK(c, hipSetDevice(c->device));
    { int rc = flush(c); if (rc) return rc; }
    HIPCHK(c, hipDeviceSynchronize());
    return 0;
}

PX_EXPORT double picles_clock(const picles_ctx *c) { return c ? c->clock : 0.0; }

static inline unsigned nblocks(long long n, int b) { return (unsigned)((n + b - 1) / b); }

static void wind_window_form(picles_ctx *c, double t0, double t1, bool knot, double tk)
{
    KParams &P = c->P;
    P.tw0 = t0;
    P.inv_dtw = 1.0 / (t1 - t0);
    if (knot) {
        P.wind_sk = (tk - t0) * P.inv_dtw;
        P.wind_isk = 1.0 / P.wind_sk;
        P.wind_i1sk = 1.0 / (1.0 - P.wind_sk);
    } else {
        P.wind_sk = P.wind_isk = P.wind_i1sk = 0.0;
    }
    P.wind_nk = knot ? 1 : 0;
}

static int wind_poly_buffers(picles_ctx *c, int nk)
{
    if (nk <= c->poly_cap) return 0;
    if (c->lv_buf) { hipFree(c->lv_buf); hipFree(c->xb_buf); c->lv_buf = c->xb_buf = nullptr; c->poly_cap = 0; }
    const size_t n = (size_t)c->A.n;
    HIPCHK(c, hipMalloc(&c->lv_buf, (size_t)2 * nk * n * 8));
    HIPCHK(c, hipMalloc(&c->xb_buf, ((size_t)PICLES_MAX_KNOTS + (size_t)2 * (nk + 1) * n) * 8));
    c->poly_cap = nk;
    return 0;
}
static int wind_window_poly(picles_ctx *c, double t0, double t1, int nk, const double *tk, hipStream_t s)
{
    KParams &P = c->P;
    Arrays &A = c->A;
    wind_window_form(c, t0, t1, true, tk[0]);
    WindPolyForm F;
    F.nk = nk;
    double sprev = 0.0;
    for (int k = 0; k < PICLES_MAX_KNOTS; k++) F.sk[k] = 2.0;
    for (int k = 0; k <= nk; k++) {
        const double sn = (k < nk) ? (tk[k] - t0) * P.inv_dtw : 1.0;
        if (k < nk) F.sk[k] = sn;
        F.ilen[k] = 1.0 / (sn - sprev);
        sprev = sn;
    }
    for (int k = nk + 1; k <= PICLES_MAX_KNOTS; k++) F.ilen[k] = 0.0;
    hipLaunchKernelGGL(k_wind_poly, dim3(nblocks(A.n, 256)), dim3(256), 0, s, F, A.u0, A.v0, A.u1, A.v1, c->lv_buf, c->xb_buf, A.n);
    HIPCHK(c, hipGetLastError());
    A.um = c->lv_buf; A.vm = c->lv_buf + A.n;
    P.wind_nk = nk;
    P.wind_xb = c->xb_buf;
    P.wind_xn = A.n;
    return 0;
}

static int set_wind_levels(picles_ctx *c, const double *u0, const double *v0, double t0,
                           const double *um, const double *vm, bool knot, double tk,
                           const double *u1, const double *v1, double t1)
{
    if (!c || !u0 || !v0) return -1;
    HIPCHK(c, hipSetDevice(c->device));
    { int rc = flush(c); if (rc) return rc; }
    HIPCHK(c, hipDeviceSynchronize());
    c->wind_grid_on = false;
    Arrays &A = c->A;
    size_t b = (size_t)A.n * 8;
    HIPCHK(c, hipMemcpyAsync(A.u0, u0, b, hipMemcpyHostToDevice, c->stream));
    HIPCHK(c, hipMemcpyAsync(A.v0, v0, b, hipMemcpyHostToDevice, c->stream));
    const bool two = u1 && v1 && t1 != t0;
    const bool three = two && um && vm;
    if (two) {
        HIPCHK(c, hipMemcpyAsync(A.u1, u1, b, hipMemcpyHostToDevice, c->stream));
        HIPCHK(c, hipMemcpyAsync(A.v1, v1, b, hipMemcpyHostToDevice, c->stream));
        c->P.wind_static = 0;
        wind_window_form(c, t0, t1, three && knot, tk);
    } else {
        c->P.wind_static = 1;
        c->P.tw0 = t0;
        c->P.inv_dtw = 0.0;
        c->P.wind_sk = c->P.wind_isk = c->P.wind_i1sk = 0.0;
        c->P.wind_nk = 0;
    }
    if (three) {
// ... 128 lines not shown
    const double eps = 1e-9;
    const double c0 = (t - lat_t0) / lat_dt, c1 = (t + dt - lat_t0) / lat_dt;
    const double k0 = __builtin_floor(c0 + eps) + 1.0;
    if (!(k0 < c1 - eps)) return 0;
    if (tk) *tk = lat_t0 + k0 * lat_dt;
    return (k0 + 1.0 < c1 - eps) ? 2 : 1;
}

PX_EXPORT int32_t picles_lattice_knot_times(double lat_t0, double lat_dt, double t, double dt, double *tks, int32_t cap)
{
    const double eps = 1e-9;
    const double c0 = (t - lat_t0) / lat_dt, c1 = (t + dt - lat_t0) / lat_dt;
    int n = 0;
    for (double k = __builtin_floor(c0 + eps) + 1.0; k < c1 - eps; k += 1.0) {
        if (tks && n < cap) tks[n] = lat_t0 + k * lat_dt;
        if (++n == 0x7fffffff) break;
    }
    return n;
}

struct WindowPlan { bool three; bool knot; double tm; int nk; double tk[PICLES_MAX_KNOTS]; };
static int wind_window_plan(picles_ctx *c, double t, double dt, WindowPlan &W)
{
    W = WindowPlan{};
    if (c->wind_grid_mode == PICLES_LATTICE_SMOOTH3) {
        W.three = true;
        W.tm = t + 0.5 * dt;
        return 0;
    }
    const int nk = picles_lattice_knot_times(c->wg_t0, c->wg_dt, t, dt, W.tk, PICLES_MAX_KNOTS);
    if (nk > PICLES_MAX_KNOTS) {
        char buf[360];
        snprintf(buf, sizeof buf, "the model step [%.17g, %.17g] contains %d time knots of the wind lattice (spacing %.17g s); a window carries at most %d: "
                 "take shorter model steps, or picles_set_wind_grid_mode(PICLES_LATTICE_SMOOTH3) if the lattice tabulates a smooth closure",
                 t, t + dt, nk, c->wg_dt, PICLES_MAX_KNOTS);
        return fail(c, -7, buf);
    }
    if (nk >= 1) { W.three = true; W.knot = true; W.tm = W.tk[0]; }
    W.nk = nk;
    return 0;
}

static int wind_window_sample(picles_ctx *c, const WindowPlan &W, double t, double dt, bool with0, hipStream_t s)
{
    Arrays &A = c->A;
    dim3 grid(nblocks(A.n, 256)), block(256);
    if (W.three && W.nk < 2 && !c->um_buf) {
        HIPCHK(c, hipMalloc(&c->um_buf, (size_t)A.n * 8));
        HIPCHK(c, hipMalloc(&c->vm_buf, (size_t)A.n * 8));
    }
    if (with0) {
        WindSampleOut O = {{t, 0.0}, {A.u0, nullptr}, {A.v0, nullptr}};
        hipLaunchKernelGGL(k_wind_sample<1>, grid, block, 0, s, c->G, c->wg, O, A.n);
    }
    if (W.nk >= 2) {
        { int rc = wind_poly_buffers(c, W.nk); if (rc) return rc; }
        const size_t n = (size_t)A.n;
        for (int k = 0; k < W.nk; k += 2) {
            const bool two = k + 1 < W.nk;
            WindSampleOut O = {{W.tk[k], two ? W.tk[k + 1] : t + dt},
                               {c->lv_buf + (size_t)(2 * k) * n, two ? c->lv_buf + (size_t)(2 * k + 2) * n : A.u1},
                               {c->lv_buf + (size_t)(2 * k + 1) * n, two ? c->lv_buf + (size_t)(2 * k + 3) * n : A.v1}};
            hipLaunchKernelGGL(k_wind_sample<2>, grid, block, 0, s, c->G, c->wg, O, A.n);
        }
        if (W.nk % 2 == 0) {
            WindSampleOut O = {{t + dt, 0.0}, {A.u1, nullptr}, {A.v1, nullptr}};
            hipLaunchKernelGGL(k_wind_sample<1>, grid, block, 0, s, c->G, c->wg, O, A.n);
        }
        HIPCHK(c, hipGetLastError());
        c->wind_t1 = t + dt;
        c->wind_t1_valid = true;
        c->P.wind_static = 0;
        return wind_window_poly(c, t, t + dt, W.nk, W.tk, s);
    }
    if (W.three) {
        WindSampleOut O = {{W.tm, t + dt}, {c->um_buf, A.u1}, {c->vm_buf, A.v1}};
        hipLaunchKernelGGL(k_wind_sample<2>, grid, block, 0, s, c->G, c->wg, O, A.n);
        A.um = c->um_buf; A.vm = c->vm_buf;
    } else {
        WindSampleOut O = {{t + dt, 0.0}, {A.u1, nullptr}, {A.v1, nullptr}};
        hipLaunchKernelGGL(k_wind_sample<1>, grid, block, 0, s, c->G, c->wg, O, A.n);
        A.um = A.vm = nullptr;
    }
    HIPCHK(c, hipGetLastError());
    c->wind_t1 = t + dt;
    c->wind_t1_valid = true;
    c->P.wind_static = 0;
    wind_window_form(c, t, t + dt, W.knot, W.tm);
    return 0;
}

static int wind_grid_prepare(picles_ctx *c, double t, double dt, hipStream_t s)
{
    Arrays &A = c->A;
    WindowPlan W;
    { int rc = wind_window_plan(c, t, dt, W); if (rc) return rc; }
    const bool reuse = c->wind_t1_valid && c->wind_t1 == t;
    if (reuse) {
        std::swap(A.u0, A.u1);
        std::swap(A.v0, A.v1);
    }
    return wind_window_sample(c, W, t, dt, !reuse, s);
}

PX_EXPORT int32_t picles_get_winds(picles_ctx *c, double *u0, double *v0, double *u1, double *v1)
{
    if (!c) return -1;
    HIPCHK(c, hipSetDevice(c->device));
    HIPCHK(c, hipDeviceSynchronize());
    size_t b = (size_t)c->A.n * 8;
    if (u0) HIPCHK(c, hipMemcpy(u0, c->A.u0, b, hipMemcpyDeviceToHost));
    if (v0) HIPCHK(c, hipMemcpy(v0, c->A.v0, b, hipMemcpyDeviceToHost));
    if (u1) HIPCHK(c, hipMemcpy(u1, c->A.u1, b, hipMemcpyDeviceToHost));
    if (v1) HIPCHK(c, hipMemcpy(v1, c->A.v1, b, hipMemcpyDeviceToHost));
    return 0;
}

PX_EXPORT int32_t picles_get_winds_mid(picles_ctx *c, double *um, double *vm)
{
    if (!c) return -1;
    if (!c->A.um) return 1;
    HIPCHK(c, hipSetDevice(c->device));
    HIPCHK(c, hipDeviceSynchronize());
    size_t b = (size_t)c->A.n * 8;
    if (um) HIPCHK(c, hipMemcpy(um, c->A.um, b, hipMemcpyDeviceToHost));
    if (vm) HIPCHK(c, hipMemcpy(vm, c->A.vm, b, hipMemcpyDeviceToHost));
    return 0;
}

PX_EXPORT int32_t picles_seed(picles_ctx *c, double t0)
{
    if (!c) return -1;
    HIPCHK(c, hipSetDevice(c->device));
    if (c->ext_streams) HIPCHK(c, hipDeviceSynchronize());
    c->clock = t0;
    if (c->wind_grid_on) {
        c->wind_t1_valid = false;
        const WindowPlan two = WindowPlan{};
        int rc = wind_window_sample(c, two, 0.0, c->od.timestep, true, c->stream);
        if (rc) return rc;
    }
    c->pending = false;
    c->ord_valid = false;
    c->cur = 0;
    c->mr_w = 0;
    for (int k = 0; k < 2; k++) {
        HIPCHK(c, hipMemsetAsync(c->rec_buf[k], 0, rec_bytes(c), c->stream));
        HIPCHK(c, hipMemsetAsync(c->mr_buf[k], 0, sizeof(int), c->stream));
        if (k == 0) for (int q = 2; q < 5; q++) HIPCHK(c, hipMemsetAsync(c->mr_buf[q], 0, sizeof(int), c->stream));
    }
    HIPCHK(c, hipMemsetAsync(c->A.cnt, 0, NSLOTS * sizeof(DevCounters), c->stream));
    HIPCHK(c, hipMemsetAsync(c->mr_buf[0] + 5, 0, 11 * sizeof(int), c->stream));
    HIPCHK(c, hipMemsetAsync(c->A.rmap, 0, (size_t)5 * c->A.ntile * sizeof(int), c->stream));
    hipLaunchKernelGGL(k_seed, dim3(nblocks(c->A.n, 256)), dim3(256), 0, c->stream, c->P, c->G, arrays_for(c, 0, 0), c->d_mask, c->od.timestep);
    HIPCHK(c, hipGetLastError());
    c->state_zero = false;
    c->seeded = true;
    return 0;
}

PX_EXPORT int32_t picles_zero_state(picles_ctx *c)
{
    if (!c) return -1;
    HIPCHK(c, hipSetDevice(c->device));
    { int rc = flush(c); if (rc) return rc; }
    if (c->ext_streams) HIPCHK(c, hipDeviceSynchronize());
    HIPCHK(c, hipMemsetAsync(c->A.state, 0, 3 * c->A.n * 8, c->stream));
    c->state_zero = true;
    return 0;
}

PX_EXPORT int32_t picles_tick(picles_ctx *c, double dt)
{
    if (!c) return -1;
    c->clock += dt;
    return 0;
}

PX_EXPORT int32_t picles_begin_step(picles_ctx *c, double dt, int32_t flags)
{
    if (!c) return -1;
    if (!(dt > 0.0)) return fail(c, -2, "dt must be positive");
    { int rc = flush(c); if (rc) return rc; }
    if (c->wind_grid_on) {
        HIPCHK(c, hipSetDevice(c->device));
        if (c->ext_streams && !c->ring_orders) HIPCHK(c, hipDeviceSynchronize());
        int rc = wind_grid_prepare(c, c->clock, dt, c->stream);
        if (rc) return rc;
    }
    c->step_dt = dt;
    c->step_flags = flags;
    c->edge_pending = false;
    c->cur ^= 1;
    c->mr_w = (c->mr_w + 1) % 5;
    c->step_fresh = true;
    return 0;
}

static bool physics_fast(const KParams &P)
{
    return P.propagation && P.input && P.dissipation && P.peak_shift && P.direction && P.n_is_2 && P.p_is_075 && P.deadband2 == 0.0;
}

static bool rows_of(const GridP &G, int which, int &r0, int &n0, int &r1, int &n1)
{
    int R = G.R;
    r0 = n0 = r1 = n1 = 0;
    bool small = G.ny_loc <= 2 * R;
    if (which == PICLES_ROWS_ALL) { n0 = G.ny_loc; }
    else if (which == PICLES_ROWS_EDGE) {
        if (small) n0 = G.ny_loc;
        else { n0 = R; r1 = G.ny_loc - R; n1 = R; }
    } else if (which == PICLES_ROWS_INTERIOR) {
        if (!small) { r0 = R; n0 = G.ny_loc - 2 * R; }
    } else return false;
    return true;
}
static int select_rows(picles_ctx *c, int which, int &r0, int &n0, int &r1, int &n1)
{
    return rows_of(c->G, which, r0, n0, r1, n1) ? 0 : fail(c, -2, "bad row selector");
}

static int step_prologue(picles_ctx *c, hipStream_t s)
{
    if (s != c->stream && !stream_idle(c->stream)) {
        HIPCHK(c, hipEventRecord(c->ev_ctx, c->stream));
        HIPCHK(c, hipStreamWaitEvent(s, c->ev_ctx, 0));
    }
    return 0;
}

PX_EXPORT int32_t picles_advance_rows(picles_ctx *c, int32_t which, void *stream)
{
    if (!c) return -1;
    HIPCHK(c, hipSetDevice(c->device));
    hipStream_t s = stream ? (hipStream_t)stream : c->stream;
    if (stream) c->ext_streams = true;
    int r0, n0, r1, n1;
    int rc = select_rows(c, which, r0, n0, r1, n1);
    if (rc) return rc;
    long long nt = (long long)(n0 + n1) * c->G.Nx;
    if (nt == 0) return 0;
    if ((rc = step_prologue(c, s))) return rc;
    c->ord_valid = false;
    timing_begin(c, s, 0);
    {
        const KParams &P = c->P;
        bool fast = physics_fast(P);
        if (!P.wind_static && P.wind_nk > 1) fast = false;
        Arrays A = arrays_for(c, c->cur, c->cur);
        StepLaunch L = {dim3(nblocks(nt, 256)), dim3(256), s, &c->P, &c->G, &A, 0.0, 0.0, c->clock, c->step_dt, r0, n0, r1, n1};
        launch_k_advance(L, fast, P.solver, P.wind_static != 0, c->A.pc != nullptr);
    }
    timing_end(c, s);
    HIPCHK(c, hipGetLastError());
    if (which == PICLES_ROWS_EDGE && s != c->stream) {
        HIPCHK(c, hipEventRecord(c->ev_edge, s));
        c->edge_pending = true;
    }
    return 0;
}

static bool step_fusable(const picles_ctx *c, int flags, double dt)
{
    if (flags != PICLES_STEP_ZERO_FIRST || !c->fuse_steps) return false;
    const KParams &P = c->P;
    if (c->wind_grid_on ? (c->wind_grid_mode != PICLES_LATTICE_SMOOTH3 && picles_lattice_knot_times(c->wg_t0, c->wg_dt, c->clock, dt, nullptr, 0) >= 2)
                        : (!P.wind_static && P.wind_nk > 1)) return false;
    const bool fast = physics_fast(P);
    if (c->wind_grid_on) return fast;
    if (c->A.pc) return fast && P.wind_static != 0;
    if (P.solver == 2) return fast && P.wind_static != 0;
    return P.wind_static != 0;
}

static bool step_rows_waverow(const picles_ctx *c, int which)
{
    int r0, n0, r1, n1;
    if (!rows_of(c->G, which, r0, n0, r1, n1)) return false;
    if (n0 + n1 == 0) return true;
    return waverow_flavour(physics_fast(c->P), c->A.pc != nullptr) && waverow_geometry(c->G.Nx, n0, n1);
}

static bool waverow_measured(const KParams &P) { return P.solver == 0 && P.wind_static != 0; }

static int launch_step_rows(picles_ctx *c, int which, hipStream_t s)
{
    int r0, n0, r1, n1;
    int rc = select_rows(c, which, r0, n0, r1, n1);
    if (rc) return rc;
    long long nt = (long long)(n0 + n1) * c->G.Nx;
    if (nt == 0) return 0;
    if ((rc = step_prologue(c, s))) return rc;
    const KParams &P = c->P;
    Arrays A = arrays_for(c, c->cur ^ 1, c->cur);
    bool fast = physics_fast(P);
    const bool orders = c->A.ord && (c->G.single_slab ? which == PICLES_ROWS_ALL : which == PICLES_ROWS_INTERIOR);
    if (orders) {
        A.nblk = (int)nblocks(nt, 256);
        const bool follows = c->ord_valid && c->ord_nblk == A.nblk;
        if (!follows) HIPCHK(c, hipMemsetAsync(c->A.ord, 0, (size_t)5 * (2 + c->A.nblk) * sizeof(int), s));
        A.ord_on = follows ? 1 : 0;
        c->ord_valid = true;
        c->ord_nblk = A.nblk;
    } else {
        A.ord = nullptr;
        if (c->G.single_slab || which != PICLES_ROWS_EDGE) c->ord_valid = false;
    }
    timing_begin(c, s, 0);
    {
        StepLaunch L = {dim3(nblocks(nt, 256)), dim3(256), s, &c->P, &c->G, &A, c->pend_t, c->pend_dt, c->clock, c->step_dt, r0, n0, r1, n1,
                        (c->waverow_mode == 2 || (c->waverow_mode == 1 && waverow_measured(P))) && step_rows_waverow(c, which)};
        if (fast && P.solver == 2) launch_k_step_auto(L, P.wind_static != 0, c->A.pc != nullptr);
        else launch_k_step_explicit(L, fast, P.solver, P.wind_static != 0, c->A.pc != nullptr);
    }
    timing_end(c, s);
    HIPCHK(c, hipGetLastError());
    return 0;
}

PX_EXPORT int32_t picles_begin_fused_step(picles_ctx *c, double dt)
{
    if (!c) return -1;
    if (!(dt > 0.0)) return fail(c, -2, "dt must be positive");
    if (!step_fusable(c, PICLES_STEP_ZERO_FIRST, dt)) return 1;
    if (c->waverow_mode == 2 && !(c->G.single_slab ? step_rows_waverow(c, PICLES_ROWS_ALL)
                                                   : step_rows_waverow(c, PICLES_ROWS_EDGE) && step_rows_waverow(c, PICLES_ROWS_INTERIOR)))
        return fail(c, -5, "PICLES_WAVEROW=require: a fused launch of this step does not qualify for k_step_waverow (one row range, "
                           "Nx a multiple of 64, rows a multiple of 4, specialised physics without the per-node metric)");
    HIPCHK(c, hipSetDevice(c->device));
    if (c->wind_grid_on) {
        Arrays &A = c->A;
        if (c->pending && !(c->wind_t1_valid && c->wind_t1 == c->clock && c->P.tw0 == c->pend_t && !c->P.wind_static))
            return 1;
        if (c->ext_streams && !c->ring_orders) HIPCHK(c, hipDeviceSynchronize());
        if (c->pending) {
            WindowPlan W;
            { int rc = wind_window_plan(c, c->clock, dt, W); if (rc) return rc; }
            if (!A.uP) {
                HIPCHK(c, hipMalloc(&A.uP, (size_t)A.n * 8));
                HIPCHK(c, hipMalloc(&A.vP, (size_t)A.n * 8));
            }
            double *tu = A.uP, *tv = A.vP;
            A.uP = A.u0; A.vP = A.v0;
            A.u0 = A.u1; A.v0 = A.v1;
            A.u1 = tu; A.v1 = tv;
            int rc = wind_window_sample(c, W, c->clock, dt, false, c->stream);
            if (rc) return rc;
        } else {
            int rc = wind_grid_prepare(c, c->clock, dt, c->stream);
            if (rc) return rc;
        }
        if (c->ext_streams && !c->ring_orders) HIPCHK(c, hipStreamSynchronize(c->stream));
    }
    c->step_dt = dt;
    c->step_flags = PICLES_STEP_ZERO_FIRST;
    c->edge_pending = false;
    c->cur ^= 1;
    c->mr_w = (c->mr_w + 1) % 5;
    c->step_fresh = true;
    return 0;
}

PX_EXPORT int32_t picles_step_rows(picles_ctx *c, int32_t which, void *stream)
{
    if (!c) return -1;
    HIPCHK(c, hipSetDevice(c->device));
    hipStream_t s = stream ? (hipStream_t)stream : c->stream;
    if (stream) c->ext_streams = true;
    if (!c->pending) return picles_advance_rows(c, which, stream);
    return launch_step_rows(c, which, s);
}

PX_EXPORT int32_t picles_end_fused_step(picles_ctx *c)
{
    if (!c) return -1;
    c->pending = true;
    c->pend_t = c->clock;
    c->pend_dt = c->step_dt;
    c->state_zero = false;
    c->edge_pending = false;
    c->clock += c->step_dt;
    c->probe_steps++;
    c->stat_steps++;
    return 0;
}

static int launch_scatter(picles_ctx *c, hipStream_t s, bool remesh)
{
    Arrays A = arrays_for(c, c->cur, c->cur);
    int flags = c->step_flags;
    bool movie = (flags & PICLES_STEP_MOVIE) != 0;
    bool zero_first = (flags & PICLES_STEP_ZERO_FIRST) != 0;
    int accum = (zero_first || c->state_zero) ? 0 : 1;
    if (flags & PICLES_STEP_ATOMIC) {
        if (!c->G.single_slab) return fail(c, -5, "PICLES_STEP_ATOMIC is single-slab only");
        if (c->G.tripolar) return fail(c, -5, "PICLES_STEP_ATOMIC does not implement the tripolar fold: use the deterministic pull");
        if (!accum) HIPCHK(c, hipMemsetAsync(c->A.state, 0, 3 * c->A.n * 8, s));
        int ntx = (c->G.Nx + PT_TX - 1) / PT_TX, nty = (c->G.ny_loc + PT_TY - 1) / PT_TY;
        timing_begin(c, s, 1);
        hipLaunchKernelGGL(k_push_tiles<true>, dim3(ntx * nty), dim3(256), 0, s, c->G, A, ntx,
                           (const int *)nullptr, (const int *)nullptr, (const int *)nullptr,
                           (const double *)nullptr, (const double *)nullptr, 0LL);
        timing_end(c, s);
        HIPCHK(c, hipGetLastError());
        if (movie) HIPCHK(c, hipMemcpyAsync(c->A.movie, c->A.state, 3 * c->A.n * 8, hipMemcpyDeviceToDevice, s));
        if (remesh) {
            timing_begin(c, s, 2);
            hipLaunchKernelGGL(k_remesh, dim3(nblocks(c->A.n, 256)), dim3(256), 0, s, c->P, c->G, A, c->clock, c->step_dt);
            timing_end(c, s);
            HIPCHK(c, hipGetLastError());
        }
        if (movie && remesh) HIPCHK(c, hipMemsetAsync(c->A.state, 0, 3 * c->A.n * 8, s));
        c->state_zero = movie && remesh;
        return 0;
    }
    timing_begin(c, s, 1);
    if (remesh)
        hipLaunchKernelGGL(k_scatter<true>, dim3(nblocks(c->A.n, 256)), dim3(256), 0, s, c->P, c->G, A, accum, movie ? 1 : 0, c->clock, c->step_dt);
    else
        hipLaunchKernelGGL(k_scatter<false>, dim3(nblocks(c->A.n, 256)), dim3(256), 0, s, c->P, c->G, A, accum, 0, c->clock, c->step_dt);
    timing_end(c, s);
    HIPCHK(c, hipGetLastError());
    c->state_zero = movie && remesh;
    return 0;
}

PX_EXPORT int32_t picles_scatter_remesh(picles_ctx *c, void *stream)
{
    if (!c) return -1;
    HIPCHK(c, hipSetDevice(c->device));
    hipStream_t s = stream ? (hipStream_t)stream : c->stream;
    if (c->edge_pending) { HIPCHK(c, hipStreamWaitEvent(s, c->ev_edge, 0)); c->edge_pending = false; }
    if (s != c->stream && !stream_idle(c->stream)) {
        HIPCHK(c, hipEventRecord(c->ev_ctx, c->stream));
        HIPCHK(c, hipStreamWaitEvent(s, c->ev_ctx, 0));
    }
    int rc = launch_scatter(c, s, true);
    if (rc) return rc;
    c->clock += c->step_dt;
    c->probe_steps++;
    c->stat_steps++;
    return 0;
}

static int time_step_phases(picles_ctx *c, double dt, int32_t flags)
{
    if (step_fusable(c, flags, dt)) {
        int rc0 = picles_begin_fused_step(c, dt);
        if (rc0) return rc0 < 0 ? rc0 : fail(c, -6, "internal: fusable step refused");
        if ((rc0 = picles_step_rows(c, PICLES_ROWS_ALL, nullptr))) return rc0;
        return picles_end_fused_step(c);
    }
    int rc = picles_begin_step(c, dt, flags);
    if (rc) return rc;
    rc = picles_advance_rows(c, PICLES_ROWS_ALL, nullptr);
    if (rc) return rc;
    return picles_scatter_remesh(c, nullptr);
}

PX_EXPORT int32_t picles_time_step(picles_ctx *c, double dt, int32_t flags)
{
    if (!c) return -1;
    if (!c->G.single_slab) return fail(c, -5, "picles_time_step needs the whole grid; slabs use begin_step/advance_rows/scatter_remesh");
    if (!(dt > 0.0)) return fail(c, -2, "dt must be positive");
    { int rc = probe_room(c, 1, "picles_time_step"); if (rc) return rc; }
    int rc = time_step_phases(c, dt, flags);
    if (rc) return rc;
    if (c->probe_n && probe_due(c, c->probe_steps)) { if ((rc = probe_take(c, c->stream))) return rc; }
    if (c->stat_on && stat_due(c, c->stat_steps)) return stat_update(c, c->stream);
    return 0;
}

PX_EXPORT int32_t picles_run_steps(picles_ctx *c, double dt, int32_t n_steps)
{
    if (!c || n_steps < 0) return -1;
    if (c->G.single_slab && dt > 0.0) { int rc = probe_room(c, n_steps, "picles_run_steps"); if (rc) return rc; }
    const bool region = c->timing && c->timing_mode == 2 && n_steps > 0;
    if (region) {
        HIPCHK(c, hipSetDevice(c->device));
        timing_begin(c, c->stream, 3);
        c->in_region = true;
        c->region_launches = 0;
    }
    int rc = 0;
    for (int k = 0; k < n_steps && rc == 0; k++) rc = picles_time_step(c, dt, PICLES_STEP_ZERO_FIRST);
    if (region) {
        c->in_region = false;
        timing_end(c, c->stream);
        c->tim.advance_launches += (uint64_t)c->region_launches;
    }
    return rc;
}

PX_EXPORT int32_t picles_advance(picles_ctx *c, double dt, int32_t flags)
{
    if (!c) return -1;
    if (!c->G.single_slab) return fail(c, -5, "picles_advance needs the whole grid");
    int rc = picles_begin_step(c, dt, flags & ~(PICLES_STEP_MOVIE));
    if (rc) return rc;
    rc = picles_advance_rows(c, PICLES_ROWS_ALL, nullptr);
    if (rc) return rc;
    return launch_scatter(c, c->stream, false);
}

PX_EXPORT int32_t picles_remesh(picles_ctx *c, double dt)
{
    if (!c) return -1;
    HIPCHK(c, hipSetDevice(c->device));
    { int rc = flush(c); if (rc) return rc; }
    timing_begin(c, c->stream, 2);
    hipLaunchKernelGGL(k_remesh, dim3(nblocks(c->A.n, 256)), dim3(256), 0, c->stream, c->P, c->G, arrays_for(c, c->cur, c->cur), c->clock, dt);
    timing_end(c, c->stream);
    HIPCHK(c, hipGetLastError());
    return 0;
}

static int d2h(picles_ctx *c, void *dst, const void *src, size_t bytes)
{
    HIPCHK(c, hipSetDevice(c->device));
    { int rc = flush(c); if (rc) return rc; }
    HIPCHK(c, hipDeviceSynchronize());
    HIPCHK(c, hipMemcpy(dst, src, bytes, hipMemcpyDeviceToHost));
    return 0;
}
static int h2d(picles_ctx *c, void *dst, const void *src, size_t bytes)
{
    HIPCHK(c, hipSetDevice(c->device));
    { int rc = flush(c); if (rc) return rc; }
    HIPCHK(c, hipDeviceSynchronize());
    HIPCHK(c, hipMemcpyAsync(dst, src, bytes, hipMemcpyHostToDevice, c->stream));
    HIPCHK(c, hipStreamSynchronize(c->stream));
    return 0;
}

PX_EXPORT int32_t picles_get_state(picles_ctx *c, double *s) { return (c && s) ? d2h(c, s, c->A.state, 3 * c->A.n * 8) : -1; }
PX_EXPORT int32_t picles_get_movie_state(picles_ctx *c, double *s) { return (c && s) ? d2h(c, s, c->A.movie, 3 * c->A.n * 8) : -1; }
PX_EXPORT int32_t picles_set_state(picles_ctx *c, const double *s)
{
    if (!c || !s) return -1;
    c->state_zero = false;
    return h2d(c, c->A.state, s, 3 * c->A.n * 8);
}

PX_EXPORT int32_t picles_get_particles(picles_ctx *c, double *z, uint8_t *on, uint8_t *boundary, int32_t *status)
{
    if (!c) return -1;
    int rc = 0;
    if (z && (rc = d2h(c, z, c->A.z, 5 * c->A.n * 8))) return rc;
    if (on && (rc = d2h(c, on, c->A.on, c->A.n))) return rc;
    if (status && (rc = d2h(c, status, c->A.status, c->A.n * 4))) return rc;
    if (boundary) {
        std::vector<unsigned char> pf(c->A.n);
        if ((rc = d2h(c, pf.data(), c->A.pflags, c->A.n))) return rc;
        for (long long k = 0; k < c->A.n; k++) boundary[k] = (pf[k] & PF_BOUNDARY) ? 1 : 0;
    }
    return 0;
}

PX_EXPORT int32_t picles_set_particles(picles_ctx *c, const double *z, const uint8_t *on)
{
    if (!c) return -1;
    int rc = 0;
    if (z && (rc = h2d(c, c->A.z, z, 5 * c->A.n * 8))) return rc;
    if (on && (rc = h2d(c, c->A.on, on, c->A.n))) return rc;
    std::vector<double> neg(c->A.n, -1.0);
    return h2d(c, c->A.dtn, neg.data(), c->A.n * 8);
}

PX_EXPORT int32_t picles_get_counters(picles_ctx *c, picles_counters *out)
{
    if (!c || !out) return -1;
    std::vector<DevCounters> d(NSLOTS);
    int rc = d2h(c, d.data(), c->A.cnt, NSLOTS * sizeof(DevCounters));
    if (rc) return rc;
    int mr = 0, mrt = 0;
    if ((rc = d2h(c, &mr, c->mr_buf[c->mr_w], sizeof(int)))) return rc;
    if ((rc = d2h(c, &mrt, c->mr_buf[0] + 5, sizeof(int)))) return rc;
    memset(out, 0, sizeof(*out));
    for (const DevCounters &k : d) {
        out->rhs_evals += k.rhs; out->steps_accepted += k.acc; out->steps_rejected += k.rej;
        out->reseeds += k.reseeds; out->clamps += k.clamps; out->maxiters_hits += k.maxit;
        out->particles_advanced += k.adv; out->halo_overflow += k.overflow;
        out->dropped_nonfinite += k.nonfinite;
        out->wave_attempt_slots += k.wslots;
    }
#ifdef PICLES_PHASE_CLOCK
    {
        unsigned long long p0 = 0, p1 = 0, p2 = 0, nw = 0;
        for (const DevCounters &k : d) { p0 += k.pad_[0]; p1 += k.pad_[1]; p2 += k.pad_[2]; nw += k.pad_[3]; }
        if (nw) fprintf(stderr, "PHASE_CLOCK waves %llu: prologue+pull %.0f, RK+guards %.0f, record+stats %.0f cycles per wave (lane 0's view)\n",
                        nw, (double)p0 / nw, (double)p1 / nw, (double)p2 / nw);
    }
#endif
    out->max_reach = mr;
    out->max_reach_seen = mrt;
    return 0;
}

PX_EXPORT int32_t picles_get_dispatch_order(picles_ctx *c, int32_t *out, int32_t cap)
{
    if (!c) return -1;
    if (cap < 0 || (cap > 0 && !out)) return fail(c, -2, "picles_get_dispatch_order: bad buffer");
    if (!c->A.ord || !c->ord_valid) return 0;
    const int n = c->ord_nblk;
    std::vector<int> h((size_t)2 + n);
    int rc = d2h(c, h.data(), c->A.ord + (size_t)((c->mr_w + 4) % 5) * (size_t)(2 + n), h.size() * sizeof(int));
    if (rc) return rc;
    if (h[0] + h[1] != n) return 0;
    const int m = cap < 2 + n ? cap : 2 + n;
    for (int k = 0; k < m; k++) out[k] = h[k];
    return n;
}

PX_EXPORT int32_t picles_reset_counters(picles_ctx *c)
{
    if (!c) return -1;
    HIPCHK(c, hipSetDevice(c->device));
    HIPCHK(c, hipDeviceSynchronize());
    HIPCHK(c, hipMemsetAsync(c->A.cnt, 0, NSLOTS * sizeof(DevCounters), c->stream));
    HIPCHK(c, hipMemsetAsync(c->mr_buf[0] + 5, 0, sizeof(int), c->stream));
    return 0;
}

PX_EXPORT int32_t picles_enable_timing(picles_ctx *c, int32_t on)
{
    if (!c) return -1;
    timing_collect(c);
    c->timing = on != 0;
    c->timing_mode = (on == 2) ? 2 : (on ? 1 : 0);
    if (on) { memset(&c->tim, 0, sizeof(c->tim)); for (auto &v : c->tim_samples) v.clear(); }
    return 0;
}

PX_EXPORT int32_t picles_get_timing(picles_ctx *c, picles_timing *t)
{
    if (!c || !t) return -1;
    HIPCHK(c, hipSetDevice(c->device));
    { int rc = flush(c); if (rc) return rc; }
    timing_collect(c);
    *t = c->tim;
    return 0;
}

PX_EXPORT int32_t picles_get_timing_samples(picles_ctx *c, int32_t kind, double *out_ms, int32_t cap)
{
    if (!c || kind < 0 || kind > 2 || cap < 0 || (cap > 0 && !out_ms)) return -1;
    HIPCHK(c, hipSetDevice(c->device));
    { int rc = flush(c); if (rc) return rc; }
    timing_collect(c);
    const std::vector<float> &v = c->tim_samples[kind];
    int n = (int)std::min<size_t>(v.size(), (size_t)cap);
    for (int k = 0; k < n; k++) out_ms[k] = v[k];
    return (int32_t)v.size();
}

PX_EXPORT int32_t picles_store_init(picles_ctx *c, int32_t n_slots)
{
    if (!c || n_slots < 1) return -1;
    HIPCHK(c, hipSetDevice(c->device));
    HIPCHK(c, hipDeviceSynchronize());
    if (c->store_slots) return fail(c, -2, "store already initialised");
    size_t b = 3 * (size_t)c->A.n * 8;
    if (!c->store_stream) HIPCHK(c, hipStreamCreateWithFlags(&c->store_stream, hipStreamNonBlocking));
    for (int k = 0; k < n_slots; k++) {
        double *d = nullptr, *h = nullptr;
        hipEvent_t e1, e2;
        HIPCHK(c, hipMalloc(&d, b));
        HIPCHK(c, hipHostMalloc(&h, b, hipHostMallocDefault));
        HIPCHK(c, hipEventCreateWithFlags(&e1, hipEventDisableTiming));
        HIPCHK(c, hipEventCreateWithFlags(&e2, hipEventDisableTiming));
        c->store_dev.push_back(d); c->store_host.push_back(h);
        c->store_ready.push_back(e1); c->store_done.push_back(e2);
    }
    c->store_time.assign(n_slots, 0.0);
    c->store_slots = n_slots; c->store_head = 0; c->store_count = 0;
    return 0;
}

PX_EXPORT int32_t picles_store_pending(const picles_ctx *c) { return c ? c->store_count : -1; }

PX_EXPORT int32_t picles_store_push(picles_ctx *c)
{
    if (!c) return -1;
    if (!c->store_slots) return fail(c, -2, "picles_store_init first");
    if (c->store_count == c->store_slots) return fail(c, -3, "snapshot ring full: pop first");
    HIPCHK(c, hipSetDevice(c->device));
    { int rc = flush(c); if (rc) return rc; }
    if (c->ext_streams) HIPCHK(c, hipDeviceSynchronize());
    int slot = (c->store_head + c->store_count) % c->store_slots;
    size_t b = 3 * (size_t)c->A.n * 8;
    HIPCHK(c, hipMemcpyAsync(c->store_dev[slot], c->A.state, b, hipMemcpyDeviceToDevice, c->stream));
    HIPCHK(c, hipEventRecord(c->store_ready[slot], c->stream));
    HIPCHK(c, hipStreamWaitEvent(c->store_stream, c->store_ready[slot], 0));
    HIPCHK(c, hipMemcpyAsync(c->store_host[slot], c->store_dev[slot], b, hipMemcpyDeviceToHost, c->store_stream));
    HIPCHK(c, hipEventRecord(c->store_done[slot], c->store_stream));
    c->store_time[slot] = c->clock;
    c->store_count++;
    return 0;
}

PX_EXPORT int32_t picles_store_pop(picles_ctx *c, double *state, double *time)
{
    if (!c || !state) return -1;
    if (!c->store_count) return fail(c, -3, "no snapshot pending");
    HIPCHK(c, hipSetDevice(c->device));
    int slot = c->store_head;
    HIPCHK(c, hipEventSynchronize(c->store_done[slot]));
    memcpy(state, c->store_host[slot], 3 * (size_t)c->A.n * 8);
    if (time) *time = c->store_time[slot];
    c->store_head = (c->store_head + 1) % c->store_slots;
    c->store_count--;
    return 0;
}

PX_EXPORT int32_t picles_diag_init(picles_ctx *c, int32_t cx, int32_t cy, int32_t field_mask, int32_t n_slots)
{
    if (!c) return -1;
    if (cx < 1 || cx > 16 || cy < 1 || cy > 16) return fail(c, -2, "picles_diag_init: coarsening factors must be 1 ... 16");
    if (field_mask <= 0 || (field_mask & ~PICLES_DIAG_ALL)) return fail(c, -2, "picles_diag_init: empty or unknown field mask");
    if (n_slots < 1) return fail(c, -2, "picles_diag_init: n_slots must be >= 1");
    if (c->diag_slots) return fail(c, -2, "picles_diag_init: diagnostics already initialised");
    if (c->G.j_begin % cy != 0) return fail(c, -2, "picles_diag_init: the slab's j_begin must be a multiple of cy (coarse cells are global)");
    HIPCHK(c, hipSetDevice(c->device));
    DiagP D{};
    D.Nx = c->G.Nx; D.ny_loc = c->G.ny_loc; D.cx = cx; D.cy = cy;
    D.Nxc = (c->G.Nx + cx - 1) / cx; D.nyc_loc = (c->G.ny_loc + cy - 1) / cy;
    D.tiles_per_row = (D.Nxc + DIAG_TILE - 1) / DIAG_TILE;
    D.mask = (unsigned)field_mask; D.g = c->ph.g; D.r_g = c->ph.r_g; D.plane = c->A.n;
    const int nf = __builtin_popcount((unsigned)field_mask), np = D.nyc_loc * D.tiles_per_row;
    const size_t fb = (size_t)4 * D.Nxc * D.nyc_loc * nf, po = (fb + 15) & ~(size_t)15, sb = po + (size_t)np * 7 * 8;
    if (!c->store_stream) HIPCHK(c, hipStreamCreateWithFlags(&c->store_stream, hipStreamNonBlocking));
    for (int k = 0; k < n_slots; k++) {
        unsigned char *d = nullptr, *h = nullptr;
        hipEvent_t e1, e2;
        HIPCHK(c, hipMalloc(&d, sb));
        c->diag_dev.push_back(d);
        HIPCHK(c, hipHostMalloc(&h, sb, hipHostMallocDefault));
        c->diag_host.push_back(h);
        HIPCHK(c, hipEventCreateWithFlags(&e1, hipEventDisableTiming));
        c->diag_ready.push_back(e1);
        HIPCHK(c, hipEventCreateWithFlags(&e2, hipEventDisableTiming));
        c->diag_done.push_back(e2);
    }
    c->diag = D; c->diag_nfields = nf; c->diag_npart = np;
    c->diag_field_bytes = fb; c->diag_part_off = po; c->diag_slot_bytes = sb;
    c->diag_time.assign(n_slots, 0.0);
    c->diag_slots = n_slots; c->diag_head = 0; c->diag_count = 0;
    return 0;
// ... 280 lines not shown
                                   int32_t first)
{
    if (!c) return -1;
    if (c->stat_on) return fail(c, -2, "picles_stat_init: a statistics set exists (picles_stat_free first)");
    if (group_mask <= 0 || (group_mask & ~PICLES_STAT_ALL)) return fail(c, -2, "picles_stat_init: empty or unknown group mask");
    if (every < 1 || first < 1) return fail(c, -2, "picles_stat_init: every and first must be >= 1");
    if (group_mask & PICLES_STAT_EXCEED) {
        if (n_thresholds < 1 || n_thresholds > STAT_MAX_THR || !thresholds)
            return fail(c, -2, "picles_stat_init: PICLES_STAT_EXCEED takes 1 ... 4 thresholds");
        for (int k = 0; k < n_thresholds; k++)
            if (!std::isfinite(thresholds[k]) || !(thresholds[k] > 0.0) || (k > 0 && !(thresholds[k] > thresholds[k - 1])))
                return fail(c, -2, "picles_stat_init: thresholds must be finite, positive and strictly ascending");
    } else if (n_thresholds != 0) {
        return fail(c, -2, "picles_stat_init: thresholds given without PICLES_STAT_EXCEED");
    }
    HIPCHK(c, hipSetDevice(c->device));
    StatP S{};
    S.mask = (unsigned)group_mask;
    S.nthr = n_thresholds;
    for (int k = 0; k < n_thresholds; k++) S.thr[k] = thresholds[k];
    const size_t bytes = (size_t)c->A.n * ((size_t)stat_nf64(S) * 8 + (size_t)stat_nu32(S) * 4);
    struct Undo { picles_ctx *c; bool armed; ~Undo() { if (armed) stat_release(c); } } undo{c, true};
    if (!c->store_stream) HIPCHK(c, hipStreamCreateWithFlags(&c->store_stream, hipStreamNonBlocking));
    HIPCHK(c, hipMalloc(&c->stat_dev, bytes));
    HIPCHK(c, hipEventCreateWithFlags(&c->stat_ev, hipEventDisableTiming));
    HIPCHK(c, hipMemsetAsync(c->stat_dev, 0, bytes, c->stream));
    c->stat = S; c->stat_bytes = bytes;
    { int rc = stat_mark(c, c->stream); if (rc) return rc; }
    c->stat_every = every; c->stat_first = first; c->stat_steps = 0;
    c->stat_samples = 0; c->stat_t_first = 0.0; c->stat_t_last = 0.0;
    c->stat_on = true;
    undo.armed = false;
    return 0;
}

PX_EXPORT int32_t picles_stat_shape(const picles_ctx *c, int32_t *group_mask, int32_t *n_thresholds, double *thresholds, int32_t *every,
                                    int32_t *n_planes, size_t *bytes)
{
    if (!c || !c->stat_on) return -1;
    if (group_mask) *group_mask = (int32_t)c->stat.mask;
    if (n_thresholds) *n_thresholds = c->stat.nthr;
    if (thresholds) for (int k = 0; k < c->stat.nthr; k++) thresholds[k] = c->stat.thr[k];
    if (every) *every = c->stat_every;
    if (n_planes) *n_planes = stat_nf64(c->stat) + stat_nu32(c->stat);
    if (bytes) *bytes = c->stat_bytes;
    return 0;
}

PX_EXPORT int32_t picles_stat_update(picles_ctx *c, void *stream)
{
    if (!c) return -1;
    if (!c->stat_on) return fail(c, -2, "picles_stat_init first");
    HIPCHK(c, hipSetDevice(c->device));
    if (stream) c->ext_streams = true;
    return stat_update(c, stream ? (hipStream_t)stream : c->stream);
}

static int stat_mask_ok(picles_ctx *c, int32_t group_mask, const char *who)
{
    if (group_mask < 0 || (group_mask & ~(int32_t)c->stat.mask))
        return fail(c, -2, std::string(who) + ": group mask is no subset of the set's");
    return 0;
}

PX_EXPORT int32_t picles_stat_get(picles_ctx *c, int32_t group_mask, void *planes, int64_t *n_samples, double *t_first, double *t_last)
{
    if (!c) return -1;
    if (!c->stat_on) return fail(c, -2, "picles_stat_init first");
    if (!planes) return fail(c, -2, "picles_stat_get: planes must be given");
    { int rc = stat_mask_ok(c, group_mask, "picles_stat_get"); if (rc) return rc; }
    HIPCHK(c, hipSetDevice(c->device));
    HIPCHK(c, hipStreamWaitEvent(c->store_stream, c->stat_ev, 0));
    size_t off[4], len[4], at = 0;
    const int n = stat_pieces(c, (unsigned)group_mask, off, len);
    for (int k = 0; k < n; k++) {
        HIPCHK(c, hipMemcpyAsync((unsigned char *)planes + at, c->stat_dev + off[k], len[k], hipMemcpyDeviceToHost, c->store_stream));
        at += len[k];
    }
    HIPCHK(c, hipStreamSynchronize(c->store_stream));
    if (n_samples) *n_samples = (int64_t)c->stat_samples;
    if (t_first) *t_first = c->stat_t_first;
    if (t_last) *t_last = c->stat_t_last;
    return 0;
}

PX_EXPORT int32_t picles_stat_set(picles_ctx *c, int32_t group_mask, const void *planes, int64_t n_samples, double t_first, double t_last)
{
    if (!c) return -1;
    if (!c->stat_on) return fail(c, -2, "picles_stat_init first");
    if (!planes) return fail(c, -2, "picles_stat_set: planes must be given");
    if (n_samples < 0) return fail(c, -2, "picles_stat_set: n_samples must be >= 0");
    { int rc = stat_mask_ok(c, group_mask, "picles_stat_set"); if (rc) return rc; }
    HIPCHK(c, hipSetDevice(c->device));
    { int rc = stat_order(c, c->stream); if (rc) return rc; }
    size_t off[4], len[4], at = 0;
    const int n = stat_pieces(c, (unsigned)group_mask, off, len);
    for (int k = 0; k < n; k++) {
        HIPCHK(c, hipMemcpyAsync(c->stat_dev + off[k], (const unsigned char *)planes + at, len[k], hipMemcpyHostToDevice, c->stream));
        at += len[k];
    }
    { int rc = stat_mark(c, c->stream); if (rc) return rc; }
    HIPCHK(c, hipEventSynchronize(c->stat_ev));
    c->stat_samples = (long long)n_samples; c->stat_t_first = t_first; c->stat_t_last = t_last;
    return 0;
}

PX_EXPORT int32_t picles_stat_reset(picles_ctx *c)
{
    if (!c) return -1;
    if (!c->stat_on) return fail(c, -2, "picles_stat_init first");
    HIPCHK(c, hipSetDevice(c->device));
    hipStream_t s = c->stream;
    { int rc = stat_order(c, s); if (rc) return rc; }
    HIPCHK(c, hipMemsetAsync(c->stat_dev, 0, c->stat_bytes, s));
    { int rc = stat_mark(c, s); if (rc) return rc; }
    c->stat_samples = 0; c->stat_t_first = 0.0; c->stat_t_last = 0.0;
    return 0;
}

PX_EXPORT int32_t picles_stat_free(picles_ctx *c)
{
    if (!c) return -1;
    if (!c->stat_on) return 0;
    HIPCHK(c, hipSetDevice(c->device));
    HIPCHK(c, hipDeviceSynchronize());
    stat_release(c);
    return 0;
}

PX_EXPORT int32_t picles_halo_rows(const picles_ctx *c) { return c ? c->G.R : -1; }

PX_EXPORT int32_t picles_set_halo_rows(picles_ctx *c, int32_t r)
{
    if (!c || r < 1 || r > 1024) return -1;
    HIPCHK(c, hipSetDevice(c->device));
    if (!c->G.single_slab && ((c->G.periodic_y && c->G.Ny <= 2 * r) || c->G.ny_loc < r))
        return fail(c, -2, "slab: periodic y axis not longer than 2*halo_rows, or fewer own rows than halo_rows");
    { int rc = flush(c); if (rc) return rc; }
    HIPCHK(c, hipDeviceSynchronize());
    int oldR = c->G.R;
    size_t row_b = (size_t)6 * c->G.Nx * 8;
    c->G.R = r;
    c->G.Rp = c->G.single_slab ? 0 : r;
    for (int k = 0; k < 2; k++) {
        double *old = c->rec_buf[k];
        c->rec_buf[k] = nullptr;
        HIPCHK(c, hipMalloc(&c->rec_buf[k], rec_bytes(c)));
        HIPCHK(c, hipMemsetAsync(c->rec_buf[k], 0, rec_bytes(c), c->stream));
        HIPCHK(c, hipMemcpyAsync((char *)c->rec_buf[k] + (size_t)r * row_b, (char *)old + (size_t)oldR * row_b,
                                 (size_t)c->G.ny_loc * row_b, hipMemcpyDeviceToDevice, c->stream));
        HIPCHK(c, hipStreamSynchronize(c->stream));
        HIPCHK(c, hipFree(old));
    }
    return 0;
}

PX_EXPORT int32_t picles_set_slab_mode(picles_ctx *c, int32_t on)
{
    if (!c) return -1;
    GridP &G = c->G;
    if (!(G.j_begin == 0 && G.ny_loc == G.Ny)) return on ? 0 : fail(c, -2, "a partial slab cannot resolve the y wrap locally");
    if (c->pending || c->seeded) return fail(c, -2, "picles_set_slab_mode: call before picles_seed");
    if (on) {
        if ((G.periodic_y && G.Ny <= 2 * G.R) || G.ny_loc < G.R)
            return fail(c, -2, "slab: periodic y axis not longer than 2*halo_rows, or fewer own rows than halo_rows");
        if (G.tripolar) return fail(c, -5, "slab mode on a whole tripolar grid is not supported");
        G.single_slab = 0;
        G.Rp = G.R;
    } else {
        G.single_slab = 1;
        G.Rp = 0;
    }
    return 0;
}

static int halo_ptr(picles_ctx *c, int side, bool send, void **ptr, size_t *bytes)
{
    if (!c || !ptr || !bytes || side < 0 || side > 1) return -1;
    const GridP &G = c->G;
    if (G.ny_loc < G.R) return fail(c, -2, "slab has fewer rows than halo_rows");
    size_t row_b = (size_t)6 * G.Nx * 8;
    int row;
    if (send) row = (side == 0) ? G.R : G.ny_loc;
    else row = (side == 0) ? 0 : G.ny_loc + G.R;
    *ptr = (char *)c->rec_buf[c->cur] + (size_t)row * row_b;
    *bytes = (size_t)G.R * row_b;
    return 0;
}
PX_EXPORT int32_t picles_halo_send_dev(picles_ctx *c, int32_t side, void **ptr, size_t *bytes) { return halo_ptr(c, side, true, ptr, bytes); }
PX_EXPORT int32_t picles_halo_recv_dev(picles_ctx *c, int32_t side, void **ptr, size_t *bytes) { return halo_ptr(c, side, false, ptr, bytes); }

#include <dlfcn.h>
#include <rccl/rccl.h>

struct RcclApi {
    decltype(&ncclGetUniqueId) GetUniqueId = nullptr;
    decltype(&ncclCommInitRank) CommInitRank = nullptr;
    decltype(&ncclCommDestroy) CommDestroy = nullptr;
    decltype(&ncclGroupStart) GroupStart = nullptr;
    decltype(&ncclGroupEnd) GroupEnd = nullptr;
    decltype(&ncclSend) Send = nullptr;
    decltype(&ncclRecv) Recv = nullptr;
    decltype(&ncclGetErrorString) GetErrorString = nullptr;
    void *handle = nullptr;
};

static RcclApi *rccl_api(std::string &err)
{
    static RcclApi api;
    static bool tried = false;
    static std::mutex mu;
    std::lock_guard<std::mutex> lk(mu);
    if (api.handle) return &api;
    if (tried) { err = "the communication library could not be loaded"; return nullptr; }
    tried = true;
    void *h = nullptr;
    const char *over = getenv("PICLES_CCL_LIB");
    if (over && *over) {
        h = dlopen(over, RTLD_NOW | RTLD_LOCAL);
        if (!h) { err = std::string("dlopen(PICLES_CCL_LIB=") + over + "): " + dlerror(); return nullptr; }
    } else {
        const char *names[] = {"librccl.so.1", "librccl.so", "/opt/rocm/lib/librccl.so.1"};
        for (const char *n : names) if ((h = dlopen(n, RTLD_NOW | RTLD_NOLOAD))) break;
        if (!h) for (const char *n : names) if ((h = dlopen(n, RTLD_NOW | RTLD_GLOBAL))) break;
        if (!h) { err = std::string("dlopen(librccl.so.1): ") + dlerror(); return nullptr; }
    }
#define RSYM(f) do { api.f = (decltype(api.f))dlsym(h, "nccl" #f); if (!api.f) { err = "the communication library lacks nccl" #f; return nullptr; } } while (0)
    RSYM(GetUniqueId); RSYM(CommInitRank); RSYM(CommDestroy); RSYM(GroupStart); RSYM(GroupEnd); RSYM(Send); RSYM(Recv);
    RSYM(GetErrorString);
#undef RSYM
    api.handle = h;
    return &api;
}

struct SlabRing {
    RcclApi *api = nullptr;
    ncclComm_t comm = nullptr;
    int rank = 0, world = 1, prev = -1, next = -1;
    hipStream_t sE = nullptr, sM = nullptr;
    hipEvent_t evE = nullptr, evM = nullptr, evEd = nullptr;
    unsigned long long steps = 0, exchanged_bytes = 0;
    hipStream_t sP = nullptr;
    hipEvent_t evPx = nullptr, evPm = nullptr, evP[2] = {nullptr, nullptr};
    bool evP_live[2] = {false, false};
    struct PhaseEv { hipEvent_t e0, e1, x1, m0, m1; };
    std::vector<PhaseEv> ph_used, ph_free;
};

#define NCCLCHK(c, R, call)                                                                     \
    do {                                                                                        \
        ncclResult_t r_ = (call);                                                               \
        if (r_ != ncclSuccess) {                                                                \
            (c)->err = std::string(#call) + ": " + (R)->api->GetErrorString(r_);                \
            return -11;                                                                         \
        }                                                                                       \
    } while (0)

PX_EXPORT int32_t picles_slab_unique_id(void *id128)
{
    if (!id128) return -1;
    std::string err;
    RcclApi *api = rccl_api(err);
    if (!api) { g_create_error = err; return -11; }
    ncclUniqueId id;
    ncclResult_t r = api->GetUniqueId(&id);
    if (r != ncclSuccess) { g_create_error = std::string("ncclGetUniqueId: ") + api->GetErrorString(r); return -11; }
    static_assert(sizeof(id) == PICLES_SLAB_ID_BYTES, "ncclUniqueId size");
    memcpy(id128, &id, sizeof(id));
    return 0;
}

PX_EXPORT int32_t picles_slab_comm_destroy(picles_ctx *c)
{
    if (!c) return -1;
    SlabRing *R = c->ring;
    if (!R) return 0;
    hipSetDevice(c->device);
    hipDeviceSynchronize();
    if (R->comm) R->api->CommDestroy(R->comm);
    if (R->evE) hipEventDestroy(R->evE);
    if (R->evM) hipEventDestroy(R->evM);
    if (R->evEd) hipEventDestroy(R->evEd);
    for (hipEvent_t e : {R->evPx, R->evPm, R->evP[0], R->evP[1]}) if (e) hipEventDestroy(e);
    if (R->sP) hipStreamDestroy(R->sP);
    for (auto *v : {&R->ph_used, &R->ph_free})
        for (auto &e : *v) { hipEventDestroy(e.e0); hipEventDestroy(e.e1); hipEventDestroy(e.x1); hipEventDestroy(e.m0); hipEventDestroy(e.m1); }
    if (R->sE) hipStreamDestroy(R->sE);
    if (R->sM) hipStreamDestroy(R->sM);
    delete R;
    c->ring = nullptr;
    return 0;
}

PX_EXPORT int32_t picles_slab_comm_init(picles_ctx *c, const void *id128, int32_t rank, int32_t world)
{
    if (!c || !id128) return -1;
    if (world < 1 || rank < 0 || rank >= world) return fail(c, -2, "slab ring: need 0 <= rank < world");
    if (c->ring) return fail(c, -2, "slab ring already initialised");
    if (c->G.single_slab && world > 1) return fail(c, -2, "slab ring of several ranks needs slab contexts (j_begin, j_end)");
    if (c->G.tripolar) return fail(c, -5, "slab ring: the tripolar fold is not wired into the native ring (use picles_amd.parallel)");
    HIPCHK(c, hipSetDevice(c->device));
    std::string err;
    RcclApi *api = rccl_api(err);
    if (!api) return fail(c, -11, err);
    SlabRing *R = new SlabRing();
    R->api = api; R->rank = rank; R->world = world;
    const bool per = c->G.periodic_y;
// ... 347 lines not shown
        const WindGrid &w = c->wg;
        h = fp_val(h, c->wind_grid_mode); h = fp_val(h, w.nx); h = fp_val(h, w.ny); h = fp_val(h, w.nt);
        for (double v : {w.x0, w.inv_dx, w.y0, w.inv_dy, c->wg_t0, c->wg_dt, w.mesh_x0, w.mesh_y0}) h = fp_val(h, v);
        h = fp_val(h, c->fp_lattice);
    }
    return h;
}

static int ckpt_buffers(picles_ctx *c, unsigned long long payload)
{
    const size_t need = (size_t)payload + 16;
    if (!c->store_stream) HIPCHK(c, hipStreamCreateWithFlags(&c->store_stream, hipStreamNonBlocking));
    if (!c->ck_ready) {
        HIPCHK(c, hipEventCreateWithFlags(&c->ck_ready, hipEventDisableTiming));
        HIPCHK(c, hipEventCreateWithFlags(&c->ck_done, hipEventDisableTiming));
    }
    if (c->ck_cap >= need) return 0;
    if (c->ck_dev) { HIPCHK(c, hipFree(c->ck_dev)); c->ck_dev = nullptr; }
    if (c->ck_host) { HIPCHK(c, hipHostFree(c->ck_host)); c->ck_host = nullptr; }
    c->ck_cap = 0;
    HIPCHK(c, hipMalloc(&c->ck_dev, need));
    HIPCHK(c, hipHostMalloc(&c->ck_host, need, hipHostMallocDefault));
    c->ck_cap = need;
    return 0;
}

static void ckpt_launch(picles_ctx *c, int mode, const CkptSegs &S, unsigned long long payload)
{
    unsigned long long maxch = 0;
    for (int k = 0; k < CKPT_NSEG; k++) maxch = std::max(maxch, S.span[k] >> 4);
    const unsigned gx = (unsigned)std::min<unsigned long long>((maxch + 255) / 256, 2048);
    dim3 grid(gx ? gx : 1, CKPT_NSEG), block(256);
    unsigned long long *sums = (unsigned long long *)(c->ck_dev + payload);
    if (mode == 0) hipLaunchKernelGGL(k_ckpt<0>, grid, block, 0, c->stream, S, c->ck_dev, sums);
    else if (mode == 1) hipLaunchKernelGGL(k_ckpt<1>, grid, block, 0, c->stream, S, c->ck_dev, sums);
    else hipLaunchKernelGGL(k_ckpt<2>, grid, block, 0, c->stream, S, c->ck_dev, sums);
}

PX_EXPORT int32_t picles_checkpoint_size(picles_ctx *c, size_t *bytes)
{
    if (!c || !bytes) return -1;
    CkptSegs S;
    *bytes = sizeof(CkptHeader) + (size_t)ckpt_layout(c, S);
    return 0;
}

PX_EXPORT int32_t picles_checkpoint_begin(picles_ctx *c)
{
    if (!c) return -1;
    if (c->ck_inflight) return fail(c, PICLES_CKPT_E_BUSY, "picles_checkpoint_begin: a checkpoint is in flight (picles_checkpoint_end first)");
    if (!c->seeded) return fail(c, -2, "picles_checkpoint_begin: nothing to save (picles_seed or picles_checkpoint_load first)");
    HIPCHK(c, hipSetDevice(c->device));
    { int rc = flush(c); if (rc) return rc; }
    if (c->ext_streams) HIPCHK(c, hipDeviceSynchronize());
    CkptSegs S;
    const unsigned long long payload = ckpt_layout(c, S);
    { int rc = ckpt_buffers(c, payload); if (rc) return rc; }
    unsigned long long *sums = (unsigned long long *)(c->ck_dev + payload);
    HIPCHK(c, hipMemsetAsync(sums, 0, 16, c->stream));
    timing_begin(c, c->stream, 4);
    ckpt_launch(c, 0, S, payload);
    timing_end(c, c->stream);
    HIPCHK(c, hipGetLastError());
    HIPCHK(c, hipEventRecord(c->ck_ready, c->stream));
    HIPCHK(c, hipStreamWaitEvent(c->store_stream, c->ck_ready, 0));
    HIPCHK(c, hipMemcpyAsync(c->ck_host, c->ck_dev, (size_t)payload + 8, hipMemcpyDeviceToHost, c->store_stream));
    HIPCHK(c, hipEventRecord(c->ck_done, c->store_stream));
    CkptHeader h;
    memset(&h, 0, sizeof h);
    h.magic = CKPT_MAGIC; h.format = CKPT_FORMAT; h.abi = PICLES_ABI_VERSION;
    h.header_bytes = sizeof(CkptHeader); h.payload_bytes = payload;
    h.fingerprint = ckpt_fingerprint(c);
    h.clock = c->clock;
    h.halo_rows = c->G.R; h.mr_w = c->mr_w; h.cur = c->cur; h.nseg = CKPT_NSEG;
    h.n = c->A.n;
    for (int k = 0; k < CKPT_NSEG; k++) { h.seg_off[k] = S.off[k]; h.seg_len[k] = S.len[k]; }
    h.step_dt = c->step_dt;
    h.state_zero = c->state_zero ? 1 : 0;
    memcpy(c->ck_hdr, &h, sizeof h);
    c->ck_inflight = true;
    return 0;
}

PX_EXPORT int32_t picles_checkpoint_end(picles_ctx *c, void *buf, size_t bytes)
{
    if (!c) return -1;
    if (!c->ck_inflight) return fail(c, -2, "picles_checkpoint_end: no checkpoint in flight (picles_checkpoint_begin first)");
    CkptHeader h;
    memcpy(&h, c->ck_hdr, sizeof h);
    const size_t total = sizeof h + (size_t)h.payload_bytes;
    if (!buf || bytes < total) {
        char m[160];
        snprintf(m, sizeof m, "picles_checkpoint_end: the blob needs %zu bytes, the buffer has %zu", total, buf ? bytes : (size_t)0);
        return fail(c, PICLES_CKPT_E_SHORT, m);
    }
    HIPCHK(c, hipSetDevice(c->device));
    HIPCHK(c, hipEventSynchronize(c->ck_done));
    memcpy(&h.checksum, c->ck_host + h.payload_bytes, 8);
    memcpy(buf, &h, sizeof h);
    memcpy((unsigned char *)buf + sizeof h, c->ck_host, (size_t)h.payload_bytes);
    c->ck_inflight = false;
    return 0;
}

PX_EXPORT int32_t picles_checkpoint_load(picles_ctx *c, const void *buf, size_t bytes)
{
    if (!c || !buf) return -1;
    if (c->probe_count > 0)
        return fail(c, PICLES_CKPT_E_BUSY, "picles_checkpoint_load: probe samples of this context are pending (picles_probe_pop first)");
    if (c->ck_inflight || c->store_count > 0 || c->diag_count > 0)
        return fail(c, PICLES_CKPT_E_BUSY, "picles_checkpoint_load: a checkpoint or store snapshot of this context is in flight (end / pop it first)");
    CkptHeader h;
    if (bytes < sizeof h) return fail(c, PICLES_CKPT_E_SHORT, "picles_checkpoint_load: buffer shorter than a checkpoint header");
    memcpy(&h, buf, sizeof h);
    if (h.magic != CKPT_MAGIC) return fail(c, PICLES_CKPT_E_MAGIC, "picles_checkpoint_load: not a checkpoint blob (bad magic)");
    if (h.format != CKPT_FORMAT || h.abi != PICLES_ABI_VERSION || h.header_bytes != sizeof h) {
        char m[200];
        snprintf(m, sizeof m, "picles_checkpoint_load: blob format %u / ABI %u, this library reads format %d / ABI %d", h.format, h.abi,
                 CKPT_FORMAT, PICLES_ABI_VERSION);
        return fail(c, PICLES_CKPT_E_VERSION, m);
    }
    if (bytes - sizeof h < h.payload_bytes) {
        char m[200];
        snprintf(m, sizeof m, "picles_checkpoint_load: truncated blob (%zu payload bytes of %llu)", bytes - sizeof h, (unsigned long long)h.payload_bytes);
        return fail(c, PICLES_CKPT_E_SHORT, m);
    }
    CkptSegs S;
    const unsigned long long payload = ckpt_layout(c, S);
    bool same = h.fingerprint == ckpt_fingerprint(c) && h.payload_bytes == payload && h.n == c->A.n && h.nseg == CKPT_NSEG;
    for (int k = 0; same && k < CKPT_NSEG; k++) same = h.seg_off[k] == S.off[k] && h.seg_len[k] == S.len[k];
    if (!same) return fail(c, PICLES_CKPT_E_CONFIG, "picles_checkpoint_load: the blob was written by a model of another configuration "
                                                    "(grid, mask, physics, ODE settings, metric, wind lattice, slab rows or slab mode differ)");
    const GridP &G = c->G;
    const int R = h.halo_rows;
    if (R < 1 || R > 1024 || (!G.single_slab && ((G.periodic_y && G.Ny <= 2 * R) || G.ny_loc < R)) || h.mr_w < 0 || h.mr_w > 4 || (h.cur & ~1))
        return fail(c, PICLES_CKPT_E_CONFIG, "picles_checkpoint_load: the blob's halo rows / counter indices do not fit this context");
    HIPCHK(c, hipSetDevice(c->device));
    { int rc = ckpt_buffers(c, payload); if (rc) return rc; }
    unsigned long long *sums = (unsigned long long *)(c->ck_dev + payload);
    const unsigned long long want[2] = {0ull, (unsigned long long)h.checksum};
    HIPCHK(c, hipMemcpyAsync(c->ck_dev, (const unsigned char *)buf + sizeof h, (size_t)payload, hipMemcpyHostToDevice, c->stream));
    HIPCHK(c, hipMemcpyAsync(sums, want, 16, hipMemcpyHostToDevice, c->stream));
    ckpt_launch(c, 1, S, payload);
    HIPCHK(c, hipGetLastError());
    unsigned long long got = 0;
    HIPCHK(c, hipMemcpyAsync(&got, sums, 8, hipMemcpyDeviceToHost, c->stream));
    HIPCHK(c, hipStreamSynchronize(c->stream));
    if (got != h.checksum) return fail(c, PICLES_CKPT_E_CHECKSUM, "picles_checkpoint_load: payload checksum mismatch (the blob is damaged)");
    HIPCHK(c, hipDeviceSynchronize());
    c->pending = false;
    if (R != G.R) { int rc = picles_set_halo_rows(c, R); if (rc) return rc; }
    ckpt_launch(c, 2, S, payload);
    HIPCHK(c, hipGetLastError());
    HIPCHK(c, hipStreamSynchronize(c->stream));
    c->clock = h.clock;
    c->step_dt = h.step_dt;
    c->pend_t = h.clock; c->pend_dt = h.step_dt;
    c->mr_w = h.mr_w;
    c->cur = h.cur;
    c->state_zero = h.state_zero != 0;
    c->seeded = true;
    c->edge_pending = false;
    c->step_fresh = false;
    c->ord_valid = false;
    c->wind_t1_valid = false;
    return 0;
}
```

### picles_amd/driver.py

```python
from __future__ import annotations

import atexit
import ctypes as C
import weakref

import numpy as np

from . import _capi as K


def _check(lib, h, rc, what):
    if rc != 0:
        msg = lib.picles_last_error(h)
        e = K.PiclesError(f"{what} failed (rc={rc}): {msg.decode() if msg else '?'}")
        e.code = rc
        raise e


def _col(a, n):
    a = np.ascontiguousarray(np.asarray(a, dtype=np.float64).reshape(-1, order="F"))
    if a.size != n:
        raise ValueError(f"expected {n} values, got {a.size}")
    return a

# ... 377 lines not shown
            raise K.PiclesError("picles_diag_shape failed: diag_init first")
        return tuple(x.value for x in a) + (b.value,)

    def diag_push(self):
        self._ck(self.lib.picles_diag_push(self.h), "picles_diag_push")

    def diag_pop(self):
        nxc, nyc, nf, npart, _ = self.diag_shape()
        f = np.empty(nf * nxc * nyc, dtype=np.float32)
        p = np.empty((npart, 7))
        t = C.c_double()
        self._ck(self.lib.picles_diag_pop(self.h, f.ctypes.data, K.dptr(p), C.byref(t)), "picles_diag_pop")
        return f.reshape((nf, nyc, nxc)).transpose(0, 2, 1), p, t.value

    @property
    def diag_pending(self):
        return self.lib.picles_diag_pending(self.h)

    def probe_init(self, nodes, every=1, first=1, capacity=64):
        ij = np.asarray(nodes, dtype=np.int64)
        if ij.ndim != 2 or ij.shape[1] != 2:
            raise ValueError("probe_init: nodes must be an (n, 2) array of (i, j)")
        if ij.size and (np.abs(ij).max() > 2**31 - 1):
            raise ValueError("probe_init: node index out of the int32 range")
        planes = np.ascontiguousarray(ij.T.astype(np.int32))
        self._ck(self.lib.picles_probe_init(self.h, int(ij.shape[0]), planes.ctypes.data_as(K.c_int32_p), int(every), int(first),
                                            int(capacity)), "picles_probe_init")

    def probe_shape(self):
        a = [C.c_int32() for _ in range(3)]
        if self.lib.picles_probe_shape(self.h, *[C.byref(x) for x in a]) != 0:
            raise K.PiclesError("picles_probe_shape failed: probe_init first")
        return tuple(x.value for x in a)

    def probe_sample(self, stream=None):
        self._ck(self.lib.picles_probe_sample(self.h, stream), "picles_probe_sample")

    def probe_pop(self, max_samples=None):
        n, _, cap = self.probe_shape()
        m = cap if max_samples is None else int(max_samples)
        m = max(1, min(m, max(self.probe_pending, 1)))
        v = np.empty((m, 3, n))
        t = np.empty(m)
        s = np.empty(m, dtype=np.int64)
        got = C.c_int32()
        self._ck(self.lib.picles_probe_pop(self.h, m, K.dptr(v), K.dptr(t), s.ctypes.data_as(C.POINTER(C.c_int64)), C.byref(got)),
                 "picles_probe_pop")
        return v[:got.value], t[:got.value], s[:got.value]

    @property
    def probe_pending(self):
        return self.lib.picles_probe_pending(self.h)

    def probe_free(self):
        self._ck(self.lib.picles_probe_free(self.h), "picles_probe_free")

    def stat_init(self, groups=K.STAT_ALL, thresholds=(), every=1, first=1):
        mask = stat_mask(groups)
        thr = np.ascontiguousarray(np.asarray(thresholds, dtype=np.float64).ravel())
        self._ck(self.lib.picles_stat_init(self.h, mask, int(thr.size), K.dptr(thr) if thr.size else None, int(every), int(first)),
                 "picles_stat_init")

    def stat_shape(self):
        m, nt, ev, npl = (C.c_int32() for _ in range(4))
        thr = (C.c_double * 4)()
        b = C.c_size_t()
        if self.lib.picles_stat_shape(self.h, C.byref(m), C.byref(nt), thr, C.byref(ev), C.byref(npl), C.byref(b)) != 0:
            raise K.PiclesError("picles_stat_shape failed: stat_init first")
        return m.value, tuple(thr[k] for k in range(nt.value)), ev.value, npl.value, b.value

    def stat_update(self, stream=None):
        self._ck(self.lib.picles_stat_update(self.h, stream), "picles_stat_update")

    def stat_get(self, groups=None):
        set_mask, thr, _, _, _ = self.stat_shape()
        mask = set_mask if groups is None else stat_mask(groups, allow_empty=True)
        lay = stat_layout(mask, len(thr))
        buf = np.empty(sum(np.dtype(dt).itemsize * k for _, dt, k in lay) * self.N, dtype=np.uint8)
        n, t0, t1 = C.c_int64(), C.c_double(), C.c_double()
        self._ck(self.lib.picles_stat_get(self.h, mask, buf.ctypes.data_as(C.c_void_p), C.byref(n), C.byref(t0), C.byref(t1)),
                 "picles_stat_get")
        out = stat_unpack(buf, lay, self.Nx, self.ny_loc)
        out.update(n_samples=int(n.value), t_first=float(t0.value), t_last=float(t1.value), thresholds=np.asarray(thr), mask=mask)
        return out

    def stat_set(self, acc):
        _, thr, _, _, _ = self.stat_shape()
        mask = int(acc["mask"]) if "mask" in acc else stat_mask_of(acc)
        buf = stat_pack(acc, stat_layout(mask, len(thr)), self.Nx, self.ny_loc)
        self._ck(self.lib.picles_stat_set(self.h, mask, buf.ctypes.data_as(C.c_void_p), int(acc["n_samples"]), float(acc["t_first"]),
                                          float(acc["t_last"])), "picles_stat_set")

    def stat_reset(self):
        self._ck(self.lib.picles_stat_reset(self.h), "picles_stat_reset")

    def stat_free(self):
        self._ck(self.lib.picles_stat_free(self.h), "picles_stat_free")

    def checkpoint_size(self) -> int:
        n = C.c_size_t()
        self._ck(self.lib.picles_checkpoint_size(self.h, C.byref(n)), "picles_checkpoint_size")
        return n.value

    def checkpoint_begin(self):
        self._ck(self.lib.picles_checkpoint_begin(self.h), "picles_checkpoint_begin")

    def checkpoint_end(self) -> np.ndarray:
        buf = np.empty(self.checkpoint_size(), dtype=np.uint8)
        self._ck(self.lib.picles_checkpoint_end(self.h, buf.ctypes.data, buf.size), "picles_checkpoint_end")
        return buf

    def checkpoint_load(self, blob):
        a = np.frombuffer(blob, dtype=np.uint8) if not isinstance(blob, np.ndarray) else np.ascontiguousarray(blob, dtype=np.uint8)
        self.gen += 1
        rc = self.lib.picles_checkpoint_load(self.h, a.ctypes.data if a.size else None, a.size)
        if rc != 0:
            msg = self.lib.picles_last_error(self.h)
            raise K.CheckpointError(rc, f"picles_checkpoint_load failed (rc={rc}): {msg.decode() if msg else '?'}")

    def get_particles(self):
        z = np.empty(5 * self.N)
        on = np.empty(self.N, dtype=np.uint8)
        bnd = np.empty(self.N, dtype=np.uint8)
        st = np.empty(self.N, dtype=np.int32)
        self._ck(self.lib.picles_get_particles(self.h, K.dptr(z), on.ctypes.data_as(K.c_uint8_p),
                                               bnd.ctypes.data_as(K.c_uint8_p), st.ctypes.data_as(K.c_int32_p)),
                 "picles_get_particles")
        sh = (self.Nx, self.ny_loc)
        return (z.reshape(sh + (5,), order="F"), on.reshape(sh, order="F"),
                bnd.reshape(sh, order="F"), st.reshape(sh, order="F"))

    def set_particles(self, z, on):
        self.gen += 1
        z = _col(z, 5 * self.N)
        on = np.ascontiguousarray(np.asarray(on, dtype=np.uint8).reshape(-1, order="F"))
        self._ck(self.lib.picles_set_particles(self.h, K.dptr(z), on.ctypes.data_as(K.c_uint8_p)),
                 "picles_set_particles")

    def scatter_particles(self, ij, xy, charge):
        self.gen += 1
        self.state_gen += 1
        ij = np.ascontiguousarray(np.asarray(ij, dtype=np.int32).T)
        xy = np.ascontiguousarray(np.asarray(xy, dtype=np.float64).T)
        ch = np.ascontiguousarray(np.asarray(charge, dtype=np.float64).T)
        n = ij.shape[1]
        self._ck(self.lib.picles_scatter_particles(self.h, n, ij.ctypes.data_as(K.c_int32_p), K.dptr(xy), K.dptr(ch)),
                 "picles_scatter_particles")

    def get_counters(self):
        c = K.PiclesCounters()
        self._ck(self.lib.picles_get_counters(self.h, C.byref(c)), "picles_get_counters")
        return c.as_dict()

    def reset_counters(self):
        self._ck(self.lib.picles_reset_counters(self.h), "picles_reset_counters")

    def enable_timing(self, on=True):
        self._ck(self.lib.picles_enable_timing(self.h, int(on)), "picles_enable_timing")

    def get_timing_samples(self, kind=0):
        n = self.lib.picles_get_timing_samples(self.h, kind, None, 0)
        if n < 0:
            self._ck(n, "picles_get_timing_samples")
        out = np.empty(max(n, 1))
        n = self.lib.picles_get_timing_samples(self.h, kind, K.dptr(out), n)
        return out[:max(n, 0)]

    def get_dispatch_order(self):
        n = self.lib.picles_get_dispatch_order(self.h, None, 0)
        if n < 0:
            self._ck(n, "picles_get_dispatch_order")
        if n == 0:
            return None
        out = np.empty(2 + n, dtype=np.int32)
        n2 = self.lib.picles_get_dispatch_order(self.h, out.ctypes.data_as(C.POINTER(C.c_int32)), out.size)
        if n2 != n:
            return None
        return int(out[0]), int(out[1]), out[2:].copy()

    def get_timing(self):
        t = K.PiclesTiming()
        self._ck(self.lib.picles_get_timing(self.h, C.byref(t)), "picles_get_timing")
        return t.as_dict()
```

Measured before the change: 7.545 billion.

## Add per-tile class map so uniform-displacement waves use a single bilinear pull

Each wave records into a per-tile class map the shared record code when all 64 lanes have the same deposit class. The next step's wave-row pull checks the neighbourhood of that map. If every tile shares the class, the wave does a fixed 2x2 bilinear gather, or skips the pull entirely when the tiles are empty, instead of the general reach-based gather. This adds class-map reads, ballot and readfirstlane work, memset clears and counter atomics, and doubles the rmap allocation, all to cut the cost of the generic pull loop. It is enabled by default and can be turned off with an environment variable.

```diff
diff --git a/include/picles_hip.h b/include/picles_hip.h
--- a/include/picles_hip.h
+++ b/include/picles_hip.h
@@ -8,7 +8,7 @@
 extern "C" {
 #endif
 
-#define PICLES_ABI_VERSION 8
+#define PICLES_ABI_VERSION 9
 
 typedef struct picles_grid {
     int32_t Nx, Ny;
@@ -176,6 +176,7 @@
 int32_t picles_get_timing(picles_ctx *ctx, picles_timing *t);
 int32_t picles_get_timing_samples(picles_ctx *ctx, int32_t kind, double *out_ms, int32_t cap);
 int32_t picles_get_dispatch_order(picles_ctx *ctx, int32_t *out, int32_t cap);
+int32_t picles_get_pull_class_counts(picles_ctx *ctx, int64_t *out);
 int32_t picles_sync(picles_ctx *ctx);
 
 #define PICLES_ROWS_ALL      0
diff --git a/picles_amd/_capi.py b/picles_amd/_capi.py
--- a/picles_amd/_capi.py
+++ b/picles_amd/_capi.py
@@ -94,7 +94,7 @@
 STEP_ZERO_FIRST = 1
 STEP_MOVIE = 2
 STEP_ATOMIC = 4
-ABI_VERSION = 8
+ABI_VERSION = 9
 SLAB_ID_BYTES = 128
 PROBE_E_FULL = -30
 
@@ -176,6 +176,7 @@
     "picles_get_timing": (C.c_int32, [_VP, C.POINTER(PiclesTiming)]),
     "picles_get_timing_samples": (C.c_int32, [_VP, C.c_int32, c_double_p, C.c_int32]),
     "picles_get_dispatch_order": (C.c_int32, [_VP, C.POINTER(C.c_int32), C.c_int32]),
+    "picles_get_pull_class_counts": (C.c_int32, [_VP, C.POINTER(C.c_int64)]),
     "picles_sync": (C.c_int32, [_VP]),
     "picles_begin_step": (C.c_int32, [_VP, C.c_double, C.c_int32]),
     "picles_advance_rows": (C.c_int32, [_VP, C.c_int32, _VP]),
diff --git a/picles_amd/csrc/k_step.inc b/picles_amd/csrc/k_step.inc
--- a/picles_amd/csrc/k_step.inc
+++ b/picles_amd/csrc/k_step.inc
@@ -38,7 +38,7 @@
     if constexpr (WROW) { active = rows_index_waverow(G, r0, n0, lblock, wr); t = wr.t0 + lane; }
     else active = rows_index(G, r0, n0, r1, n1, t, lblock);
     StepStats S = {{0u, 0u, 0u, 0}, 0u, 0u, 0u, 0u, 0u, 0u, 0};
-    int rtile = -1;
+    int rtile = -1, ccode = -1;
     if (active) {
         int i, jl;
         if constexpr (WROW) { i = wr.i0 + (int)lane; jl = wr.jl; }
@@ -61,7 +61,11 @@
             asw_pre = Av.asw[tx];
             if (!STATIC) { uP_pre = Av.uP[tx]; vP_pre = Av.vP[tx]; }
         }
-        if constexpr (WROW) pull_waverow(G, A, wr, lane, pull_reach_local_waverow(G, A, wr, lane, pull_reach(G, A, jl, mr_early)), s0, s1, s2);
+        if constexpr (WROW) {
+            int cls;
+            const int Rl = pull_reach_local_waverow(G, A, wr, lane, pull_reach(G, A, jl, mr_early), cls);
+            pull_waverow(G, A, wr, lane, Rl, cls, s0, s1, s2);
+        }
         else pull_any(G, A, i, jl, pull_reach_local(G, A, i, jl, pull_reach(G, A, jl, mr_early)), s0, s1, s2);
 #ifdef PICLES_PHASE_CLOCK
         __asm__ volatile("" : "+v"(s0), "+v"(s1), "+v"(s2));
@@ -124,7 +128,7 @@
             S.reseeds += (unsigned int)(pr_ >> 8);
             Abv.qold[tbx] = qold;
             Abv.status[tbx] = status;
-            if constexpr (WROW) write_record_at(Gb, rec_row_out(Ab, Gb, wrb.jl + Gb.R) + wrb.i0, threadIdx.x & 63u, pfb, on, z, S);
+            if constexpr (WROW) write_record_at(Gb, rec_row_out(Ab, Gb, wrb.jl + Gb.R) + wrb.i0, threadIdx.x & 63u, pfb, on, z, S, &ccode);
             else write_record(Gb, Ab, ib, jlb, pfb, on, z, S);
             rtile = WROW ? (int)(wrb.t0 >> 6) : (int)(tb >> 6);
         }
@@ -132,7 +136,7 @@
     {
         KStepArgsPtr K = kargs_reload();
         const Arrays Ab = K->A;
-        flush_stats<WROW>(Ab, S, rtile);
+        flush_stats<WROW>(Ab, S, rtile, ccode);
         if (Ab.ord && order_wanted(Ab)) order_file(Ab, lblock, __ballot(S.adv != 0 || S.reseeds != 0) != 0);
 #ifdef PICLES_WAVE_LOG
         if ((threadIdx.x & 63) == 0) {
diff --git a/picles_amd/csrc/kernels.h b/picles_amd/csrc/kernels.h
--- a/picles_amd/csrc/kernels.h
+++ b/picles_amd/csrc/kernels.h
@@ -22,8 +22,10 @@
 #define NSLOTS 1024
 struct DevCounters {
     unsigned long long rhs, acc, rej, reseeds, clamps, maxit, adv, overflow;
-    unsigned long long nonfinite, wslots, pad_[6];
+    unsigned long long nonfinite, wslots, pad_[4];
+    unsigned long long cls, cls_empty;
 };
+static_assert(sizeof(DevCounters) == 128, "two 64-B lines per slot");
 
 struct Arrays {
     double *state, *movie;
@@ -50,6 +52,10 @@
 
 __device__ __forceinline__ int *reach_counters(const Arrays &A) { return (int *)(A.cnt + NSLOTS); }
 
+#define CMAP_EMPTY (-1)
+#define MR_CLASS_ON 4096
+__device__ __forceinline__ int *class_map(const Arrays &A, int which) { return A.rmap + (size_t)(5 + which) * (size_t)A.ntile; }
+
 #define PF_STEPPED 1
 #define PF_GROUP2 2
 #define PF_BOUNDARY 4
@@ -212,7 +218,8 @@
 }
 
 template <class IDX>
-__device__ __forceinline__ void write_record_at(const GridP &G, double *rr, IDX i, unsigned char pf, int on, const Vec5 &z, StepStats &S)
+__device__ __forceinline__ void write_record_at(const GridP &G, double *rr, IDX i, unsigned char pf, int on, const Vec5 &z, StepStats &S,
+                                                int *code_out = nullptr)
 {
     auto at = [&](int plane) -> double & {
         if constexpr (std::is_unsigned<IDX>::value) return (rr + (size_t)plane * (size_t)G.Nx)[i];
@@ -240,6 +247,7 @@
         else { S.overflow = 1; S.reach = 0; }
     }
     at(5) = code;
+    if (code_out) *code_out = (int)code;
 }
 __device__ __forceinline__ void write_record(const GridP &G, const Arrays &A, int i, int jl, unsigned char pf, int on,
                                              const Vec5 &z, StepStats &S)
@@ -248,8 +256,17 @@
 }
 
 template <bool WROW = false>
-__device__ __forceinline__ void flush_stats(const Arrays &A, const StepStats &S, int rtile = -1)
-{
+__device__ __forceinline__ void flush_stats(const Arrays &A, const StepStats &S, int rtile = -1, int ccode = -1)
+{
+    if constexpr (WROW) {
+        if (A.mr_idx & MR_CLASS_ON) {
+            const int c0 = __builtin_amdgcn_readfirstlane(ccode);
+            if (c0 >= 0 && !__ballot(ccode != c0)) {
+                const int tile0 = __builtin_amdgcn_readfirstlane(rtile);
+                if ((threadIdx.x & 63) == 0) class_map(A, (A.mr_idx >> 4) & 15)[tile0] = c0 ? c0 : CMAP_EMPTY;
+            }
+        }
+    }
     unsigned long long s_rhs = wave_sum_u64(S.st.rhs);
     unsigned long long s_ar = wave_sum_u64(((unsigned long long)S.st.acc << 32) | S.st.rej);
     unsigned long long b_adv = __ballot(S.adv != 0), b_res1 = __ballot(S.reseeds == 1), b_res2 = __ballot(S.reseeds >= 2);
@@ -680,6 +697,7 @@
     if ((t & 63) == 0) A.rmap[(size_t)((A.mr_idx >> 8) & 15) * (size_t)A.ntile + (size_t)(t >> 6)] = 0;
 }
 
+
 __device__ __forceinline__ int pull_reach_local(const GridP &G, const Arrays &A, int i, int jl, int Rg)
 {
     int R = Rg;
@@ -735,22 +753,40 @@
 }
 __device__ __forceinline__ void rmap_clear_ahead_waverow(const Arrays &A, const WaveRow &w, unsigned int lane)
 {
-    if (lane == 0u) A.rmap[(size_t)((A.mr_idx >> 8) & 15) * (size_t)A.ntile + (size_t)(w.t0 >> 6)] = 0;
-}
-
-__device__ __forceinline__ int pull_reach_local_waverow(const GridP &G, const Arrays &A, const WaveRow &w, unsigned int lane, int Rg)
-{
-    if (Rg < 2) return Rg;
+    if (lane == 0u) {
+        A.rmap[(size_t)((A.mr_idx >> 8) & 15) * (size_t)A.ntile + (size_t)(w.t0 >> 6)] = 0;
+        class_map(A, (A.mr_idx >> 8) & 15)[(size_t)(w.t0 >> 6)] = 0;
+    }
+}
+
+__device__ __forceinline__ int pull_reach_local_waverow(const GridP &G, const Arrays &A, const WaveRow &w, unsigned int lane, int Rg, int &cls)
+{
+    cls = 0;
+    const bool klass = (A.mr_idx & MR_CLASS_ON) != 0;
+    if (Rg < 2 && !klass) return Rg;
     const int jl = w.jl, j = jl + G.j_begin;
     const bool edge_row = G.Rp > 0 && (jl < G.R || jl >= G.ny_loc - G.R);
-    if (Rg <= 31 && !edge_row && w.i0 - Rg >= 0 && w.i0 + 63 + Rg < G.Nx && jl - Rg >= 0 && jl + Rg < G.ny_loc && j - Rg >= 0 && j + Rg < G.Ny) {
+    if (Rg >= 1 && Rg <= 31 && !edge_row && w.i0 - Rg >= 0 && w.i0 + 63 + Rg < G.Nx && jl - Rg >= 0 && jl + Rg < G.ny_loc && j - Rg >= 0 && j + Rg < G.Ny) {
         const int *const rm = A.rmap + (size_t)(A.mr_idx & 15) * (size_t)A.ntile;
+        const int *const cm = class_map(A, A.mr_idx & 15);
         const long long nbx = G.Nx >> 6;
         long long tile = ((long long)(jl - Rg) * G.Nx + w.i0) >> 6;
-        int m = 0;
-        for (int dj = -Rg; dj <= Rg; dj++, tile += nbx) m = max(m, max(rm[tile - 1], max(rm[tile], rm[tile + 1])));
-        return __builtin_amdgcn_readfirstlane(min(m, Rg));
-    }
+        int m = 0, diff = 0;
+        const int c0 = klass ? cm[tile] : 0;
+        for (int dj = -Rg; dj <= Rg; dj++, tile += nbx) {
+            if (Rg >= 2) m = max(m, max(rm[tile - 1], max(rm[tile], rm[tile + 1])));
+            if (klass) diff |= (cm[tile - 1] ^ c0) | (cm[tile] ^ c0) | (cm[tile + 1] ^ c0);
+        }
+        if (diff == 0 && c0 > 0) {
+            int grp, bx, by;
+            rec_decode((double)c0, grp, bx, by);
+            const int rx = (bx < 0) ? -bx : bx + 1, ry = (by < 0) ? -by : by + 1;
+            if (max(rx, ry) > Rg) diff = 1;
+        }
+        cls = __builtin_amdgcn_readfirstlane(diff == 0 ? c0 : 0);
+        return Rg >= 2 ? __builtin_amdgcn_readfirstlane(min(m, Rg)) : Rg;
+    }
+    if (Rg < 2) return Rg;
     return pull_reach_local(G, A, w.i0 + (int)lane, jl, Rg);
 }
 
@@ -853,10 +889,49 @@
     }
 }
 
-__device__ __forceinline__ void pull_waverow(const GridP &G, const Arrays &A, const WaveRow &w, unsigned int lane, int R,
+__device__ __forceinline__ void pull_class_waverow(const double *__restrict__ rec0, unsigned int lane, unsigned int pl, unsigned int rowlen,
+                                                   int bx, int by, double &s0, double &s1, double &s2)
+{
+    unsigned int vo[5];
+#pragma unroll
+    for (int k = 0; k < 5; k++) vo[k] = 8u * ((unsigned int)k * pl + lane);
+    double e[4], mx[4], my[4], wx[4], wy[4];
+#pragma unroll
+    for (int k = 0; k < 4; k++) {
+        const int di = -bx - 1 + (k & 1), dj = -by - 1 + (k >> 1);
+        const char *const pb = (const char *)(rec0 + ((long long)dj * (long long)rowlen + di));
+        wx[k] = *(const double *)(pb + vo[3]); wy[k] = *(const double *)(pb + vo[4]);
+        e[k] = *(const double *)(pb + vo[0]); mx[k] = *(const double *)(pb + vo[1]); my[k] = *(const double *)(pb + vo[2]);
+    }
+#pragma unroll
+    for (int k = 0; k < 4; k++) {
+        const bool hx = !(k & 1), hy = !(k >> 1);
+        const double w = (hx ? wx[k] : 1.0 - wx[k]) * (hy ? wy[k] : 1.0 - wy[k]);
+        s0 += w * e[k];
+        s1 += w * mx[k];
+        s2 += w * my[k];
+    }
+}
+
+__device__ __forceinline__ void pull_waverow(const GridP &G, const Arrays &A, const WaveRow &w, unsigned int lane, int R, int cls,
                                              double &s0, double &s1, double &s2)
 {
     const int j = w.jl + G.j_begin;
+    if (cls != 0) {
+        if (lane == 0u) {
+            DevCounters *const c = A.cnt + ((blockIdx.x * 4u + (threadIdx.x >> 6)) & (NSLOTS - 1));
+            atomicAdd(&c->cls, 1ull);
+            if (cls == CMAP_EMPTY) atomicAdd(&c->cls_empty, 1ull);
+        }
+        if (cls == CMAP_EMPTY) return;
+        int cgrp, bx, by;
+        rec_decode((double)cls, cgrp, bx, by);
+        const unsigned int pl = (unsigned int)G.Nx, rowlen = 6u * pl;
+        const double *const rec0 = A.rec + ((size_t)(w.jl + G.R) * (size_t)rowlen + (size_t)w.i0);
+        for (int grp = 1; grp <= G.ngroups; grp++)
+            if (grp == cgrp) pull_class_waverow(rec0, lane, pl, rowlen, bx, by, s0, s1, s2);
+        return;
+    }
     if ((R == 1 || R == 2) && w.i0 - R >= 0 && w.i0 + 63 + R < G.Nx && j - R >= 0 && j + R < G.Ny) {
         const unsigned int pl = (unsigned int)G.Nx, rowlen = 6u * pl;
         const double *const rec0 = A.rec + ((size_t)(w.jl + G.R) * (size_t)rowlen + (size_t)w.i0);
diff --git a/picles_amd/csrc/picles_hip.hip b/picles_amd/csrc/picles_hip.hip
--- a/picles_amd/csrc/picles_hip.hip
+++ b/picles_amd/csrc/picles_hip.hip
@@ -378,6 +378,8 @@
     int cur = 0;
     bool fuse_steps = true;
     int waverow_mode = 1;
+    bool pull_class = true;
+    int cmap_hot = 0;
     bool pending = false;
     double pend_t = 0.0, pend_dt = 0.0;
     signed char *d_mask = nullptr;
@@ -516,8 +518,27 @@
     Arrays A = c->A;
     A.rec = c->rec_buf[read_buf];
     A.rec_out = c->rec_buf[write_buf];
-    A.mr_idx = (read_buf == write_buf ? c->mr_w : (c->mr_w + 4) % 5) | (c->mr_w << 4) | (((c->mr_w + 2) % 5) << 8);
+    A.mr_idx = (read_buf == write_buf ? c->mr_w : (c->mr_w + 4) % 5) | (c->mr_w << 4) | (((c->mr_w + 2) % 5) << 8) | (c->pull_class ? MR_CLASS_ON : 0);
     return A;
+}
+
+static int class_map_zero(picles_ctx *c)
+{
+    c->cmap_hot = 0;
+    HIPCHK(c, hipMemsetAsync(c->A.rmap + (size_t)5 * c->A.ntile, 0, (size_t)5 * c->A.ntile * sizeof(int), c->stream));
+    return 0;
+}
+static int class_map_clear_rows(picles_ctx *c, hipStream_t s, int r0, int n0, int r1, int n1)
+{
+    int *const cm = c->A.rmap + (size_t)(5 + (c->mr_w + 2) % 5) * c->A.ntile;
+    const int rr[2] = {r0, r1}, nn[2] = {n0, n1};
+    for (int k = 0; k < 2; k++) {
+        if (nn[k] <= 0) continue;
+        const long long a = ((long long)rr[k] * c->G.Nx) >> 6, b = ((long long)(rr[k] + nn[k]) * c->G.Nx + 63) >> 6;
+        const long long hi = b < (long long)c->A.ntile ? b : (long long)c->A.ntile;
+        if (hi > a) HIPCHK(c, hipMemsetAsync(cm + a, 0, (size_t)(hi - a) * sizeof(int), s));
+    }
+    return 0;
 }
 
 static int launch_scatter(picles_ctx *c, hipStream_t s, bool remesh);
@@ -583,6 +604,7 @@
 
     picles_ctx *c = new picles_ctx();
     if (const char *wr = getenv("PICLES_WAVEROW")) c->waverow_mode = !strcmp(wr, "0") ? 0 : (!strcmp(wr, "require") ? 2 : 1);
+    if (const char *pc = getenv("PICLES_PULL_CLASS")) c->pull_class = strcmp(pc, "0") != 0;
     memset(&c->A, 0, sizeof(c->A));
     c->stream = nullptr;
     c->ev_edge = nullptr;
@@ -711,8 +733,8 @@
     CK(hipMalloc(&A.ord, (size_t)5 * (2 + A.nblk) * sizeof(int)));
     CK(hipMemset(A.ord, 0, (size_t)5 * (2 + A.nblk) * sizeof(int)));
     A.ntile = (int)((n + 63) / 64);
-    CK(hipMalloc(&A.rmap, (size_t)5 * A.ntile * sizeof(int)));
-    CK(hipMemset(A.rmap, 0, (size_t)5 * A.ntile * sizeof(int)));
+    CK(hipMalloc(&A.rmap, (size_t)10 * A.ntile * sizeof(int)));
+    CK(hipMemset(A.rmap, 0, (size_t)10 * A.ntile * sizeof(int)));
     CK(hipMalloc(&c->d_mask, n));
     CK(hipMemset(A.state, 0, 3 * n * 8)); CK(hipMemset(A.movie, 0, 3 * n * 8)); CK(hipMemset(A.z, 0, 5 * n * 8));
     CK(hipMemset(A.qold, 0, n * 8)); CK(hipMemset(A.dtn, 0, n * 8)); CK(hipMemset(A.on, 0, n)); CK(hipMemset(A.status, 0, n * 4));
@@ -1147,6 +1169,7 @@
     HIPCHK(c, hipMemsetAsync(c->A.cnt, 0, NSLOTS * sizeof(DevCounters), c->stream));
     HIPCHK(c, hipMemsetAsync(c->mr_buf[0] + 5, 0, 11 * sizeof(int), c->stream));
     HIPCHK(c, hipMemsetAsync(c->A.rmap, 0, (size_t)5 * c->A.ntile * sizeof(int), c->stream));
+    { int rc = class_map_zero(c); if (rc) return rc; }
     hipLaunchKernelGGL(k_seed, dim3(nblocks(c->A.n, 256)), dim3(256), 0, c->stream, c->P, c->G, arrays_for(c, 0, 0), c->d_mask, c->od.timestep);
     HIPCHK(c, hipGetLastError());
     c->state_zero = false;
@@ -1188,6 +1211,7 @@
     c->edge_pending = false;
     c->cur ^= 1;
     c->mr_w = (c->mr_w + 1) % 5;
+    if (c->cmap_hot > 0) c->cmap_hot--;
     c->step_fresh = true;
     return 0;
 }
@@ -1238,6 +1262,7 @@
     if (nt == 0) return 0;
     if ((rc = step_prologue(c, s))) return rc;
     c->ord_valid = false;
+    if (c->cmap_hot > 0 && (rc = class_map_clear_rows(c, s, r0, n0, r1, n1))) return rc;
     timing_begin(c, s, 0);
     {
         const KParams &P = c->P;
@@ -1302,10 +1327,12 @@
         A.ord = nullptr;
         if (c->G.single_slab || which != PICLES_ROWS_EDGE) c->ord_valid = false;
     }
+    const bool waverow = (c->waverow_mode == 2 || (c->waverow_mode == 1 && waverow_measured(P))) && step_rows_waverow(c, which);
+    if (waverow && c->pull_class) c->cmap_hot = 4;
+    else if (!waverow && c->cmap_hot > 0 && (rc = class_map_clear_rows(c, s, r0, n0, r1, n1))) return rc;
     timing_begin(c, s, 0);
     {
-        StepLaunch L = {dim3(nblocks(nt, 256)), dim3(256), s, &c->P, &c->G, &A, c->pend_t, c->pend_dt, c->clock, c->step_dt, r0, n0, r1, n1,
-                        (c->waverow_mode == 2 || (c->waverow_mode == 1 && waverow_measured(P))) && step_rows_waverow(c, which)};
+        StepLaunch L = {dim3(nblocks(nt, 256)), dim3(256), s, &c->P, &c->G, &A, c->pend_t, c->pend_dt, c->clock, c->step_dt, r0, n0, r1, n1, waverow};
         if (fast && P.solver == 2) launch_k_step_auto(L, P.wind_static != 0, c->A.pc != nullptr);
         else launch_k_step_explicit(L, fast, P.solver, P.wind_static != 0, c->A.pc != nullptr);
     }
@@ -1353,6 +1380,7 @@
     c->edge_pending = false;
     c->cur ^= 1;
     c->mr_w = (c->mr_w + 1) % 5;
+    if (c->cmap_hot > 0) c->cmap_hot--;
     c->step_fresh = true;
     return 0;
 }
@@ -1557,6 +1585,8 @@
 {
     if (!c) return -1;
     int rc = 0;
+    HIPCHK(c, hipSetDevice(c->device));
+    if ((rc = class_map_zero(c))) return rc;
     if (z && (rc = h2d(c, c->A.z, z, 5 * c->A.n * 8))) return rc;
     if (on && (rc = h2d(c, c->A.on, on, c->A.n))) return rc;
     std::vector<double> neg(c->A.n, -1.0);
@@ -1590,6 +1620,18 @@
 #endif
     out->max_reach = mr;
     out->max_reach_seen = mrt;
+    return 0;
+}
+
+PX_EXPORT int32_t picles_get_pull_class_counts(picles_ctx *c, int64_t *out)
+{
+    if (!c || !out) return -1;
+    std::vector<DevCounters> d(NSLOTS);
+    HIPCHK(c, hipSetDevice(c->device));
+    HIPCHK(c, hipDeviceSynchronize());
+    HIPCHK(c, hipMemcpy(d.data(), c->A.cnt, NSLOTS * sizeof(DevCounters), hipMemcpyDeviceToHost));
+    out[0] = out[1] = 0;
+    for (const DevCounters &k : d) { out[0] += (int64_t)k.cls; out[1] += (int64_t)k.cls_empty; }
     return 0;
 }
 
@@ -2176,7 +2218,7 @@
         HIPCHK(c, hipStreamSynchronize(c->stream));
         HIPCHK(c, hipFree(old));
     }
-    return 0;
+    return class_map_zero(c);
 }
 
 PX_EXPORT int32_t picles_set_slab_mode(picles_ctx *c, int32_t on)
@@ -2830,6 +2872,7 @@
     if (R != G.R) { int rc = picles_set_halo_rows(c, R); if (rc) return rc; }
     ckpt_launch(c, 2, S, payload);
     HIPCHK(c, hipGetLastError());
+    { int rc = class_map_zero(c); if (rc) return rc; }
     HIPCHK(c, hipStreamSynchronize(c->stream));
     c->clock = h.clock;
     c->step_dt = h.step_dt;
diff --git a/picles_amd/driver.py b/picles_amd/driver.py
--- a/picles_amd/driver.py
+++ b/picles_amd/driver.py
@@ -553,6 +553,11 @@
         self._ck(self.lib.picles_get_counters(self.h, C.byref(c)), "picles_get_counters")
         return c.as_dict()
 
+    def get_pull_class_counts(self):
+        out = (C.c_int64 * 2)()
+        self._ck(self.lib.picles_get_pull_class_counts(self.h, out), "picles_get_pull_class_counts")
+        return int(out[0]), int(out[1])
+
     def reset_counters(self):
         self._ck(self.lib.picles_reset_counters(self.h), "picles_reset_counters")
 
```

Measured after the change: 7.957 billion, median of 6. 1.05x the previous value.
